# zengyf131/gswt_renderer

Measured on AMD Instinct MI355X. Metric: frames/sec @1920x1080, 32x32 Wang-tile grid, higher is better.
Workload: dtype f32

## Files before the change

### gswt_renderer_amd/csrc/gswt_api.hip

```cpp
#include "../../include/gswt_hip.h"
#include "gswt_device.h"

#include <dlfcn.h>

#include <algorithm>
#include <cstdarg>
#include <cstdio>
#include <cstring>
#include <string>
#include <unordered_map>
#include <utility>
#include <vector>

using namespace gswt;

namespace {

template <typename T>
struct DevBuf {
    T* p = nullptr;
    size_t cap = 0;
    DevBuf() = default;
    DevBuf(DevBuf&& o) noexcept : p(std::exchange(o.p, nullptr)), cap(std::exchange(o.cap, 0)) {}
    DevBuf& operator=(DevBuf&& o) noexcept { std::swap(p, o.p); std::swap(cap, o.cap); return *this; }
    ~DevBuf() { release(); }
    hipError_t ensure(size_t n)
    {
        if (n <= cap) return hipSuccess;
        size_t ncap = n + n / 4 + 1024;
        T* np = nullptr;
        static const bool log_alloc = getenv("GSWT_LOG_ALLOC") != nullptr;
        if (log_alloc) fprintf(stderr, "gswt alloc: %zu -> %zu bytes%s\n", cap * sizeof(T), ncap * sizeof(T), p ? " (grow: frees the old buffer)" : "");
        hipError_t e = hipMalloc(&np, ncap * sizeof(T));
        if (e != hipSuccess) return e;
        if (p) hipFree(p);
        p = np; cap = ncap;
        return hipSuccess;
    }
    hipError_t ensure_roomy(size_t n) { return n <= cap ? hipSuccess : ensure(2 * n); }
    void release() { if (p) hipFree(p); p = nullptr; cap = 0; }
};

using ListRef = gswt::SceneList;

static inline hipError_t null_stream_done() { return hipStreamSynchronize(nullptr); }

template <typename T>
struct HostBuf {
    T* p = nullptr;
    size_t cap = 0;
    HostBuf() = default;
    HostBuf(HostBuf&& o) noexcept : p(std::exchange(o.p, nullptr)), cap(std::exchange(o.cap, 0)) {}
    HostBuf& operator=(HostBuf&& o) noexcept { std::swap(p, o.p); std::swap(cap, o.cap); return *this; }
    ~HostBuf() { release(); }
    hipError_t ensure(size_t n)
    {
        if (n <= cap) return hipSuccess;
        const size_t ncap = n + n / 4 + 64;
        T* np = nullptr;
        hipError_t e = hipHostMalloc(reinterpret_cast<void**>(&np), ncap * sizeof(T), hipHostMallocDefault);
        if (e != hipSuccess) return e;
        if (p) hipHostFree(p);
        p = np; cap = ncap;
        return hipSuccess;
    }
    void release() { if (p) hipHostFree(p); p = nullptr; cap = 0; }
};

}

#ifndef GSWT_FRAME_SLOTS
#define GSWT_FRAME_SLOTS 5
#endif
constexpr int kFrameSlots = GSWT_FRAME_SLOTS;
constexpr const char* kStreamLayout = "c012p34s";

constexpr int kDrawSets = kFrameSlots + 5;
static_assert(kDrawSets <= kMergeSources, "MergeSources holds one pointer pair per draw set");
static_assert(sizeof(gswt_render_config) == 32 && offsetof(gswt_render_config, out_format) == 28, "gswt_render_config layout");
static_assert(GSWT_OUT_RGBA32F == kOutF32 && GSWT_OUT_RGBA8_UNORM == kOutRGBA8 && GSWT_OUT_BGRA8_UNORM == kOutBGRA8, "output formats");
template <typename T>
struct Ref { T* p = nullptr; };

struct DrawSet {
    HostBuf<uint8_t> h_blob;
    DevBuf<uint8_t> d_blob;
    size_t blob_bytes = 0;
    size_t off_draws = 0, off_xcd = 0, off_groups = 0, off_jobs = 0, off_remap = 0, off_segs = 0, off_blocks = 0, off_cblocks = 0, off_n64 = 0;
    template <typename T> T* hp(size_t off) { return reinterpret_cast<T*>(h_blob.p + off); }
    template <typename T> T* dp(size_t off) { return reinterpret_cast<T*>(d_blob.p + off); }
    hipError_t plan(size_t n_draws, size_t n_groups, size_t n_members, size_t total_entries)
    {
        size_t o = 0;
        auto take = [&o](size_t bytes) { const size_t at = o; o = (o + bytes + 255) & ~(size_t)255; return at; };
        const size_t n_blk = total_entries / 1024 + 2 * n_members + 2;
        off_draws = take((n_draws + 1) * sizeof(DrawDev)); off_xcd = take((n_draws + 1) * 4);
        off_groups = take((n_groups + 1) * sizeof(MergeGroup)); off_jobs = take((n_groups + 1) * sizeof(MergeCopy));
        off_remap = take((n_members + 1) * sizeof(uint2)); off_segs = take((2 * n_members + 1) * sizeof(MergeSeg));
        off_blocks = take(n_blk * sizeof(uint2)); off_cblocks = take(n_blk * sizeof(uint2)); off_n64 = take(64);
        blob_bytes = o;
        hipError_t e = o <= h_blob.cap ? hipSuccess : h_blob.ensure(2 * o);
        if (e != hipSuccess) return e;
        e = d_blob.ensure_roomy(o);
        if (e != hipSuccess) return e;
        draws.p = dp<DrawDev>(off_draws); xcd_first.p = dp<uint32_t>(off_xcd);
        return hipSuccess;
    }
    uint64_t per_xcd[8] = {};
    uint64_t longest = 0;
    Ref<DrawDev> draws;
    DevBuf<uint2> chunk_tab;
    DevBuf<uint2> chunk_tab_xcd;
    DevBuf<uint32_t> merged_list, merged_map;
    Ref<uint32_t> xcd_first;
    struct GroupDesc { uint32_t view, base, len, first, n; uint64_t hash; };
    std::vector<GroupDesc> g_desc;
    std::vector<gswt_merge_member> g_members;
    bool g_valid = false;
    uint32_t src_mask = 0;
    hipEvent_t ev_up = nullptr;
    bool ev_up_pending = false;
    bool built = false;
    size_t n_merged = 0;
    uint32_t n_launch = 0;
    uint32_t n_draws = 0, n_chunks = 0;
    uint64_t n_entries = 0;
    void release()
    {
        chunk_tab.release(); chunk_tab_xcd.release(); merged_list.release(); merged_map.release(); h_blob.release(); d_blob.release();
        draws.p = nullptr; xcd_first.p = nullptr;
        if (ev_up) hipEventDestroy(ev_up);
        ev_up = nullptr;
    }
};

struct FrameArgs {
    gswt_camera_uniforms cam;
    gswt_scene_uniforms su;
    gswt_render_config cfg;
    int width = 0, height = 0;
    const float4* d_bg = nullptr;
    const float* d_bgd = nullptr;
    float4* d_out = nullptr;
    float* d_out_depth = nullptr;
};

enum FrameEvent { kEvStart, kEvProjected, kEvEmitted, kEvSorted, kEvRanges, kEvEnd, kEvCompositeBegin, kEvCompositeEnd, kEvDone, kFrameEvents };

struct FrameSlot {
    hipStream_t stream = nullptr;
    hipEvent_t ev[kFrameEvents] = {};
    hipEvent_t ev_in = nullptr;
    hipEvent_t ev_gather = nullptr;
    bool gather_recorded = false;
    unsigned long long seq = 0;
    unsigned long long* hc = nullptr;
    unsigned long long* hc_dev = nullptr;
    bool pending = false;
    bool collected = false;
    int collected_rc = 0;
    gswt_timings collected_timings = {};
    FrameArgs args;
    int set = 0;
    uint32_t cap = 0;
    int n_tiles = 0;
    int timing_level = 0;
    DevBuf<uint2> rects;
    DevBuf<Rec> recs;
    DevBuf<uint4> live_tab;
    DevBuf<uint32_t> live_cnt;
    DevBuf<uint32_t> live_cid;
    DevBuf<uint32_t> cell_culled;
    DevBuf<uint32_t> block_sums, draw_culled, keys_a, keys_b, vals_a, vals_b, ghist;
    DevBuf<uint2> ranges;
    DevBuf<uint32_t> item_base;
    DevBuf<uint4> item_tab;
    DevBuf<uint32_t> aux_a, aux_b;
    bool strict_vs = false;
    uint32_t depth_passes = 0;
    bool depth_local = false;
    bool full_grid = false;
    uint32_t n_launch_eff = 0;
    DevBuf<float4> partials;
    DevBuf<float> partials_z;
    DevBuf<float4> col_f;
    DevBuf<float> depths;
    GraphRec grec;
    hipGraph_t graph = nullptr;
    hipGraphExec_t graph_exec = nullptr;
    hipGraphNode_t graph_nodes[kGraphMaxNodes] = {};
    GraphNodeRec graph_last[kGraphMaxNodes];
    uint32_t graph_n = 0;
    void release_graph()
    {
        if (graph_exec) hipGraphExecDestroy(graph_exec);
        if (graph) hipGraphDestroy(graph);
        graph_exec = nullptr; graph = nullptr; graph_n = 0;
    }
    void release_buffers()
    {
        rects.release(); recs.release(); cell_culled.release(); live_tab.release(); live_cid.release(); live_cnt.release(); block_sums.release(); draw_culled.release(); keys_a.release();
        keys_b.release(); vals_a.release(); vals_b.release(); ghist.release(); ranges.release(); item_base.release();
        aux_a.release(); aux_b.release(); partials.release(); partials_z.release(); item_tab.release(); col_f.release(); depths.release();
    }
};

struct gswt_ctx {
    int device = 0;
    FrameSlot slots[kFrameSlots];
    unsigned long long frame_seq = 0;
    hipStream_t stream = nullptr;
    bool own_stream = true;
    std::string err;
    DevBuf<uint4> tex;
    size_t n_splats = 0;
    float loc_lo[3] = {}, loc_hi[3] = {}, loc_max_trace = 0.0f;
    DevBuf<uint32_t> static_list;
    DevBuf<float> static_boxes;
    std::vector<ListRef> lists;
    size_t static_n = 0, boxes_n = 0;
    int n_lod = 0, n_tile = 0, n_view = 0;
    bool scene_ready = false;
    DevBuf<float> hmap;
    int hm_w = 0, hm_h = 0;
    float hm_min = 0.f, hm_max = 0.f, hm_du = 0.f, hm_dv = 0.f;
    DevBuf<float4> sky_faces;
    int sky_size = 0, sky_equi = 0;
    DevBuf<float4> proxy_tex;
    int proxy_size = 0, proxy_mips = 0, proxy_grid_dim = 2048;
    uint32_t proxy_mip_off[16] = {};
    DrawSet sets[kDrawSets];
    int cur_set = 0;
    int latest_set = 0;
    int pending_set = -1;
    hipStream_t set_stream = nullptr;
    std::vector<hipStream_t> pad_streams;
    int opt_defer_swap = 0;
    int opt_graph = 0;
    int opt_strict_vs = 1;
    int opt_composite = 0;
    int opt_no_chunk_cull = 0;
    unsigned long long stat_graph_launches = 0, stat_graph_rebuilds = 0, stat_graph_node_updates = 0;
    int pending_frames = 0;
    int merge_target = 0;
    DevBuf<int32_t> raw_depth;
    std::vector<uint32_t> raw_off;
    std::vector<uint32_t> raw_cnt, raw_merge_offset;

    int opt_no_merge_reuse = 0;
    unsigned long long stat_groups_built = 0, stat_groups_reused = 0, stat_groups_reused_deep = 0;
    DevBuf<uint32_t> mg_ws;
    bool draws_ready = false;
    uint32_t pair_cap = 0;
    uint32_t depth_passes = 3;
    uint32_t depth_passes_low_run = 0, depth_passes_low_max = 0;
    int opt_depth_sort = 0;
    int opt_item_order = 0;
    uint32_t live_hint = 0;
    uint32_t depth_max_tile_len = 0;
    unsigned long long stat_depth_local = 0, stat_depth_global = 0;
    int last_slot = 0;
    DevBuf<float4> bg_rgba, out_img;
    DevBuf<float> bg_depth, out_depth_img;
    DevBuf<Varyings> dbg;
    int opt_no_prefilter = 0;
    int opt_debug_varyings = 0;
    int opt_timing = 2;
    int opt_segment = 1536;
    int opt_fixed_pair_cap = 0;
    uint32_t last_n_tiles = 0;
    gswt_timings timings = {};
    void* comm = nullptr;
    int comm_rank = 0, comm_world = 0;
    std::vector<gswt_ctx*> group;
    int group_rank = 0;
    DevBuf<float4> gather_buf;
    hipEvent_t ev_push = nullptr;
    hipEvent_t ev_unshard = nullptr;
    bool unshard_pending = false;
};

namespace {

int fail(gswt_ctx* c, int code, const char* fmt, ...)
{
    char buf[512];
    va_list ap;
    va_start(ap, fmt);
    vsnprintf(buf, sizeof(buf), fmt, ap);
    va_end(ap);
    if (c) c->err = buf;
    return code;
}

hipError_t sync_all(gswt_ctx* c)
{
    hipError_t e = hipStreamSynchronize(c->stream);
    if (c->set_stream) { hipError_t e2 = hipStreamSynchronize(c->set_stream); if (e == hipSuccess) e = e2; }
    for (auto& sl : c->slots)
        if (sl.stream) { hipError_t e2 = hipStreamSynchronize(sl.stream); if (e == hipSuccess) e = e2; }
    return e;
}

#define GSWT_CATCH(NAME)                                                                   \
    catch (const std::bad_alloc&) { return GSWT_ERR_CAPACITY; }                             \
    catch (...) { return GSWT_ERR_HIP; }

#define HIP_TRY(c, expr)                                                                              \
    do {                                                                                              \
        hipError_t _e = (expr);                                                                       \
        if (_e != hipSuccess) return fail((c), GSWT_ERR_HIP, "%s: %s", #expr, hipGetErrorString(_e)); \
    } while (0)

void mat4_mul(const float* a, const float* b, float* out)
{
    for (int c = 0; c < 4; c++)
        for (int r = 0; r < 4; r++) {
            float acc = a[r] * b[4 * c];
            for (int k = 1; k < 4; k++) acc = acc + a[4 * k + r] * b[4 * c + k];
            out[4 * c + r] = acc;
        }
}

}

namespace {

struct Id128 { char b[GSWT_COMM_ID_BYTES]; };
struct RcclApi {
    void* lib = nullptr;
    int (*GetUniqueId)(void*) = nullptr;
    int (*CommInitRank)(void**, int,  Id128, int) = nullptr;
    int (*AllGather)(const void*, void*, size_t, int, void*, hipStream_t) = nullptr;
    int (*CommDestroy)(void*) = nullptr;
    const char* (*GetErrorString)(int) = nullptr;
    bool tried = false;
};
RcclApi g_rccl;

const char* rccl_load()
{
    if (g_rccl.lib) return nullptr;
    if (g_rccl.tried) return "librccl.so could not be loaded";
    g_rccl.tried = true;
    const char* names[] = {"librccl.so", "librccl.so.1", "/opt/rocm/lib/librccl.so.1"};
    for (const char* n : names) {
        g_rccl.lib = dlopen(n, RTLD_NOW | RTLD_GLOBAL);
        if (g_rccl.lib) break;
    }
    if (!g_rccl.lib) return "librccl.so could not be loaded";
    g_rccl.GetUniqueId = reinterpret_cast<int (*)(void*)>(dlsym(g_rccl.lib, "ncclGetUniqueId"));
    g_rccl.CommInitRank = reinterpret_cast<int (*)(void**, int, Id128, int)>(dlsym(g_rccl.lib, "ncclCommInitRank"));
    g_rccl.AllGather = reinterpret_cast<int (*)(const void*, void*, size_t, int, void*, hipStream_t)>(dlsym(g_rccl.lib, "ncclAllGather"));
    g_rccl.CommDestroy = reinterpret_cast<int (*)(void*)>(dlsym(g_rccl.lib, "ncclCommDestroy"));
    g_rccl.GetErrorString = reinterpret_cast<const char* (*)(int)>(dlsym(g_rccl.lib, "ncclGetErrorString"));
    if (!g_rccl.GetUniqueId || !g_rccl.CommInitRank || !g_rccl.AllGather || !g_rccl.CommDestroy) {
        dlclose(g_rccl.lib); g_rccl.lib = nullptr;
        return "librccl.so lacks ncclGetUniqueId / ncclCommInitRank / ncclAllGather / ncclCommDestroy";
    }
    return nullptr;
}

constexpr int kNcclFloat = 7;

struct ShardGeom { int world, mode, out_rows, out_w, fmt; size_t px, bytes; };
ShardGeom shard_geom(const FrameSlot& sl)
{
    ShardGeom g;
    const gswt_render_config& cfg = sl.args.cfg;
    g.world = cfg.shard_count <= 1 ? 1 : cfg.shard_count;
    g.mode = cfg.shard_mode;
    const bool cols = g.world > 1 && g.mode == GSWT_SHARD_COLUMNS;
    g.out_rows = g.world > 1 && !cols ? gswt_shard_rows_padded(sl.args.height, g.world) : sl.args.height;
    g.out_w = cols ? gswt_shard_cols_padded(sl.args.width, g.world) : sl.args.width;
    g.px = (size_t)g.out_rows * g.out_w;
    g.fmt = (int)cfg.out_format;
    g.bytes = g.px * out_pixel_bytes(g.fmt);
    return g;
}

}

static int finish_frame(gswt_ctx* c, FrameSlot& sl);

static hipError_t collect_pending(gswt_ctx* c)
{
    for (auto& sl : c->slots)
        if (sl.pending && !sl.collected) {
            sl.collected_rc = finish_frame(c, sl);
            sl.collected_timings = c->timings;
            sl.collected = true;
        }
    return sync_all(c);
}

static void invalidate_merge_sources(gswt_ctx* c)
{
    for (auto& ds : c->sets) { ds.g_valid = false; ds.g_desc.clear(); ds.g_members.clear(); ds.src_mask = 0; }
}

static void collect_set(gswt_ctx* c, int set, bool host_upload)
{
    for (auto& sl : c->slots)
        if (sl.pending && !sl.collected && sl.set == set) {
            sl.collected_rc = finish_frame(c, sl);
            sl.collected_timings = c->timings;
            sl.collected = true;
        }
    if (!host_upload) return;
    for (int k = 0; k < kDrawSets; k++) {
        DrawSet& o = c->sets[k];
        if (k != set && o.ev_up_pending && ((o.src_mask >> set) & 1u)) { (void)hipEventSynchronize(o.ev_up); o.ev_up_pending = false; }
    }
}

namespace gswt {
int ctx_device(const gswt_ctx* c) { return c->device; }
}

extern "C" {

int gswt_create(int device_id, gswt_ctx** out)
try {
    if (!out) return GSWT_ERR_BAD_ARG;
    *out = nullptr;
    int ndev = 0;
    if (hipGetDeviceCount(&ndev) != hipSuccess || ndev <= 0) return GSWT_ERR_HIP;
    if (device_id < 0 || device_id >= ndev) return GSWT_ERR_BAD_ARG;
    if (hipSetDevice(device_id) != hipSuccess) return GSWT_ERR_HIP;
    gswt_ctx* c = new (std::nothrow) gswt_ctx();
    if (!c) return GSWT_ERR_CAPACITY;
    c->device = device_id;
    const char* layout = getenv("GSWT_STREAM_LAYOUT");
    if (!layout || !*layout) layout = kStreamLayout;
    for (const char* q = layout; *q; q++) {
        hipStream_t* dst = nullptr;
        hipStream_t pad = nullptr;
        if (*q == 'c') dst = &c->stream;
        else if (*q == 's') dst = &c->set_stream;
        else if (*q >= '0' && *q < '0' + kFrameSlots) dst = &c->slots[*q - '0'].stream;
        else if (*q == 'p') dst = &pad;
        else continue;
        if (*dst) continue;
        if ((q[1] == '+' || q[1] == '-')) {
            int lo = 0, hi = 0;
            hipDeviceGetStreamPriorityRange(&lo, &hi);
            if (hipStreamCreateWithPriority(dst, hipStreamNonBlocking, q[1] == '+' ? hi : lo) != hipSuccess) { delete c; return GSWT_ERR_HIP; }
        } else
        if (hipStreamCreateWithFlags(dst, hipStreamNonBlocking) != hipSuccess) { delete c; return GSWT_ERR_HIP; }
        if (dst == &pad) c->pad_streams.push_back(pad);
    }
    if (!c->stream && hipStreamCreateWithFlags(&c->stream, hipStreamNonBlocking) != hipSuccess) { delete c; return GSWT_ERR_HIP; }
    if (!c->set_stream && hipStreamCreateWithFlags(&c->set_stream, hipStreamNonBlocking) != hipSuccess) { delete c; return GSWT_ERR_HIP; }
    for (auto& sl : c->slots) {
        if (hipEventCreateWithFlags(&sl.ev_in, hipEventDisableTiming) != hipSuccess) { delete c; return GSWT_ERR_HIP; }
        if (hipEventCreate(&sl.ev_gather) != hipSuccess) { delete c; return GSWT_ERR_HIP; }
        for (auto& e : sl.ev)
            if (hipEventCreate(&e) != hipSuccess) { delete c; return GSWT_ERR_HIP; }
        if (hipHostMalloc(reinterpret_cast<void**>(&sl.hc), 8 * sizeof(unsigned long long), hipHostMallocMapped) != hipSuccess) { delete c; return GSWT_ERR_HIP; }
        memset(sl.hc, 0, 8 * sizeof(unsigned long long));
        if (hipHostGetDevicePointer(reinterpret_cast<void**>(&sl.hc_dev), sl.hc, 0) != hipSuccess) sl.hc_dev = nullptr;
    }
    *out = c;
    return GSWT_OK;
} GSWT_CATCH("gswt_create")

void gswt_destroy(gswt_ctx* c)
{
    if (!c) return;
    hipSetDevice(c->device);
    sync_all(c);
    for (gswt_ctx* m : std::vector<gswt_ctx*>(c->group))
        if (m && m != c) m->group.clear();
    c->group.clear();
    if (c->comm && g_rccl.CommDestroy) g_rccl.CommDestroy(c->comm);
    if (c->ev_push) hipEventDestroy(c->ev_push);
    if (c->ev_unshard) hipEventDestroy(c->ev_unshard);
    c->gather_buf.release();
    c->tex.release(); c->static_list.release(); c->static_boxes.release(); c->hmap.release(); for (auto& ds : c->sets) ds.release();
    c->raw_depth.release(); 
    c->mg_ws.release(); c->sky_faces.release(); c->proxy_tex.release(); c->bg_rgba.release(); c->out_img.release(); c->bg_depth.release(); c->out_depth_img.release(); c->dbg.release();
    for (auto& sl : c->slots) {
        sl.release_graph();
        sl.release_buffers();
        for (auto& e : sl.ev) if (e) hipEventDestroy(e);
        if (sl.ev_in) hipEventDestroy(sl.ev_in);
        if (sl.ev_gather) hipEventDestroy(sl.ev_gather);
        if (sl.hc) hipHostFree(sl.hc);
        if (sl.stream) hipStreamDestroy(sl.stream);
    }
    if (c->own_stream && c->stream) hipStreamDestroy(c->stream);
    if (c->set_stream) hipStreamDestroy(c->set_stream);
    for (hipStream_t ps : c->pad_streams) hipStreamDestroy(ps);
    delete c;
}

const char* gswt_last_error(const gswt_ctx* c) { return c ? c->err.c_str() : "null ctx"; }

int gswt_set_stream(gswt_ctx* c, void* hip_stream)
try {
    if (!c) return GSWT_ERR_BAD_ARG;
    collect_pending(c);
    if (c->own_stream && c->stream) hipStreamDestroy(c->stream);
    if (hip_stream) { c->stream = (hipStream_t)hip_stream; c->own_stream = false; return GSWT_OK; }
    c->stream = nullptr; c->own_stream = true;
    hipSetDevice(c->device);
    HIP_TRY(c, hipStreamCreateWithFlags(&c->stream, hipStreamNonBlocking));
    return GSWT_OK;
} GSWT_CATCH("gswt_set_stream")

int gswt_set_option(gswt_ctx* c, int key, int value)
try {
    if (!c) return GSWT_ERR_BAD_ARG;
    switch (key) {
    case GSWT_OPT_NO_LOD_PREFILTER: c->opt_no_prefilter = value; c->draws_ready = false; return GSWT_OK;
    case GSWT_OPT_DEBUG_VARYINGS: c->opt_debug_varyings = value; return GSWT_OK;
    case GSWT_OPT_DEBUG_FLAGS:
        if (value != 0) return fail(c, GSWT_ERR_BAD_ARG, "GSWT_OPT_DEBUG_FLAGS is reserved: only 0 is accepted");
        return GSWT_OK;
    case GSWT_OPT_TIMING: c->opt_timing = value; return GSWT_OK;
    case GSWT_OPT_NO_MERGE_REUSE: c->opt_no_merge_reuse = value; return GSWT_OK;
    case GSWT_OPT_DEFER_SWAP: c->opt_defer_swap = value; return GSWT_OK;
    case GSWT_OPT_GRAPH: c->opt_graph = value; return GSWT_OK;
    case GSWT_OPT_STRICT_VS: c->opt_strict_vs = value != 0; return GSWT_OK;
    case GSWT_OPT_COMPOSITE:
        if (value < 0 || value > 2) return fail(c, GSWT_ERR_BAD_ARG, "unknown compositor variant %d", value);
        c->opt_composite = value; return GSWT_OK;
    case GSWT_OPT_NO_CHUNK_CULL: c->opt_no_chunk_cull = value != 0; return GSWT_OK;
    case GSWT_OPT_ITEM_ORDER: c->opt_item_order = value != 0; return GSWT_OK;
    case GSWT_OPT_DEPTH_SORT:
        if (value < 0 || value > 2) return fail(c, GSWT_ERR_BAD_ARG, "GSWT_OPT_DEPTH_SORT: 0 (auto), 1 (global passes) or 2 (tile-local)");
        c->opt_depth_sort = value; c->depth_max_tile_len = 0;
        return GSWT_OK;
    case GSWT_OPT_DEPTH_PASSES:
        if (value < 1 || value > 4) return fail(c, GSWT_ERR_BAD_ARG, "depth-sort passes must be 1..4");
        c->depth_passes = (uint32_t)value; c->depth_passes_low_run = 0;
        return GSWT_OK;
    case GSWT_OPT_PAIR_CAP:
        if (value < 0) return fail(c, GSWT_ERR_BAD_ARG, "pair capacity must be >= 0");
        c->opt_fixed_pair_cap = value > 0; if (value > 0) c->pair_cap = (uint32_t)value;
        return GSWT_OK;
    case GSWT_OPT_SEGMENT:
        if (value < 256 || value % 256) return fail(c, GSWT_ERR_BAD_ARG, "segment must be a positive multiple of 256");
        c->opt_segment = value; return GSWT_OK;
    default: return fail(c, GSWT_ERR_BAD_ARG, "unknown option %d", key);
    }
} GSWT_CATCH("gswt_set_option")

int gswt_upload_scene(gswt_ctx* c, const uint32_t* tex_data, size_t n_splats, const gswt_base_list* lists, int n_lod,
                      int n_tile, int n_view)
try {
    if (!c) return GSWT_ERR_BAD_ARG;
    if (!tex_data || n_splats == 0 || !lists || n_lod <= 0 || n_tile <= 0 || n_view <= 0)
        return fail(c, GSWT_ERR_BAD_ARG, "gswt_upload_scene: empty scene");
    if (n_lod > 16) return fail(c, GSWT_ERR_BAD_ARG, "gswt_upload_scene: n_lod %d > 16 (transition_dist_vec holds 16)", n_lod);
    if (n_splats > (size_t)kIdxMask) return fail(c, GSWT_ERR_CAPACITY, "gswt_upload_scene: %zu splats exceed 2^28", n_splats);
    hipSetDevice(c->device);
    HIP_TRY(c, collect_pending(c));
    c->scene_ready = false; c->draws_ready = false;
    invalidate_merge_sources(c);
    HIP_TRY(c, c->tex.ensure(2 * n_splats));
    HIP_TRY(c, hipMemcpy(c->tex.p, tex_data, n_splats * 32, hipMemcpyHostToDevice));
    c->n_splats = n_splats;
    {
        float lo[3] = {3.402823466e+38f, 3.402823466e+38f, 3.402823466e+38f}, hi[3] = {-3.402823466e+38f, -3.402823466e+38f, -3.402823466e+38f};
        float tr_max = 0.0f;
        bool odd = false;
        auto half_val = [](uint32_t h) -> float {
            const uint32_t e = (h >> 10) & 0x1Fu, fr = h & 0x3FFu;
            if (e == 31u) return 0.0f;
            const float m = e == 0u ? (float)fr * 2.98023223876953125e-08f : ldexpf(1.0f + (float)fr / 1024.0f, (int)e - 15);
            return (h & 0x8000u) ? -m : m;
        };
        for (size_t i = 0; i < n_splats; i++) {
            const uint32_t* r = tex_data + 8 * i;
            float p[3];
            memcpy(p, r, 12);
            for (int k = 0; k < 3; k++) {
                if (!(p[k] == p[k]) || p[k] > 3e38f || p[k] < -3e38f) { odd = true; continue; }
                lo[k] = std::min(lo[k], p[k]); hi[k] = std::max(hi[k], p[k]);
            }
            const double xx = half_val(r[4] & 0xFFFFu), xy = half_val(r[4] >> 16), xz = half_val(r[5] & 0xFFFFu);
            const double yy = half_val(r[5] >> 16), yz = half_val(r[6] & 0xFFFFu), zz = half_val(r[6] >> 16);
            const double tr_d = xx + yy + zz;
            const bool psd = xx >= 0.0 && yy >= 0.0 && zz >= 0.0 && xx * yy - xy * xy >= 0.0 && xx * zz - xz * xz >= 0.0 &&
                             yy * zz - yz * yz >= 0.0 && xx * (yy * zz - yz * yz) - xy * (xy * zz - yz * xz) + xz * (xy * yz - yy * xz) >= 0.0;
            const double fro = std::sqrt(xx * xx + yy * yy + zz * zz + 2.0 * (xy * xy + xz * xz + yz * yz));
            const float tr = psd ? (float)tr_d : (float)(0.5 * (tr_d + 1.7320508075688772 * fro) * (1.0 + 1e-6));
            if (tr == tr) tr_max = std::max(tr_max, tr);
        }
        if (odd || lo[0] > hi[0]) { for (int k = 0; k < 3; k++) { lo[k] = -3.402823466e+38f; hi[k] = 3.402823466e+38f; } }
        for (int k = 0; k < 3; k++) { c->loc_lo[k] = lo[k]; c->loc_hi[k] = hi[k]; }
        c->loc_max_trace = tr_max;
    }
    const size_t nl = (size_t)n_lod * n_tile * n_view;
    c->lists.assign(nl, ListRef{});
    std::vector<uint32_t> arena;
    std::vector<float> boxes;
    auto add_boxes = [&](uint32_t base, uint32_t count) -> uint32_t {
        const uint32_t first = (uint32_t)(boxes.size() / 6);
        for (uint32_t k = 0; (size_t)k * kChunk < count; k++) {
            const uint32_t hi_i = count - k * (uint32_t)kChunk, lo_i = hi_i > (uint32_t)kChunk ? hi_i - (uint32_t)kChunk : 0u;
            float lo[3] = {3.402823466e+38f, 3.402823466e+38f, 3.402823466e+38f}, hi[3] = {-3.402823466e+38f, -3.402823466e+38f, -3.402823466e+38f};
            bool odd = false;
            for (uint32_t j = lo_i; j < hi_i; j++) {
                float pq[3];
                memcpy(pq, tex_data + 8 * (size_t)(arena[base + j] & kIdxMask), 12);
                for (int a = 0; a < 3; a++) {
                    if (!(pq[a] == pq[a]) || pq[a] > 3e38f || pq[a] < -3e38f) odd = true;
                    lo[a] = std::min(lo[a], pq[a]); hi[a] = std::max(hi[a], pq[a]);
                }
            }
            for (int a = 0; a < 3; a++) boxes.push_back(odd ? -__builtin_inff() : lo[a]);
            for (int a = 0; a < 3; a++) boxes.push_back(odd ? __builtin_inff() : hi[a]);
        }
        return first;
    };
    size_t total = 0;
    for (size_t i = 0; i < nl; i++) total += lists[i].splat_count;
    arena.reserve(2 * total);
    for (size_t i = 0; i < nl; i++) {
        const gswt_base_list& L = lists[i];
        const uint32_t lod = (uint32_t)(i / ((size_t)n_tile * n_view));
        if (L.splat_count && (!L.gs_index || !L.gs_lod_id)) return fail(c, GSWT_ERR_BAD_ARG, "gswt_upload_scene: list %zu has null arrays", i);
        ListRef ref;
        ref.pair_base = (uint32_t)arena.size();
        ref.pair_count = L.splat_count;
        for (uint32_t j = 0; j < L.splat_count; j++) {
            if (L.gs_index[j] >= n_splats) return fail(c, GSWT_ERR_BAD_ARG, "gswt_upload_scene: list %zu entry %u out of range", i, j);
            if (L.gs_lod_id[j] > 15u) return fail(c, GSWT_ERR_BAD_ARG, "gswt_upload_scene: list %zu lod id out of range", i);
            arena.push_back(L.gs_index[j] | (L.gs_lod_id[j] << kLodShift));
        }
        ref.self_base = (uint32_t)arena.size();
        for (uint32_t j = 0; j < L.splat_count; j++)
            if (L.gs_lod_id[j] == lod) arena.push_back(L.gs_index[j] | (lod << kLodShift));
        ref.self_count = (uint32_t)arena.size() - ref.self_base;
        ref.pair_box = add_boxes(ref.pair_base, ref.pair_count);
        ref.self_box = add_boxes(ref.self_base, ref.self_count);
        c->lists[i] = ref;
    }
    if (arena.size() >= 0xFFFFFFFFull) return fail(c, GSWT_ERR_CAPACITY, "gswt_upload_scene: static lists exceed 2^32 entries");
    HIP_TRY(c, c->static_list.ensure(arena.size() + 1));
    HIP_TRY(c, hipMemcpy(c->static_list.p, arena.data(), arena.size() * 4, hipMemcpyHostToDevice));
    HIP_TRY(c, c->static_boxes.ensure(boxes.size() + 6));
    if (!boxes.empty()) HIP_TRY(c, hipMemcpy(c->static_boxes.p, boxes.data(), boxes.size() * 4, hipMemcpyHostToDevice));
    HIP_TRY(c, null_stream_done());
    c->static_n = arena.size(); c->boxes_n = boxes.size() / 6;
    c->n_lod = n_lod; c->n_tile = n_tile; c->n_view = n_view;
    c->scene_ready = true;
    return GSWT_OK;
} GSWT_CATCH("gswt_upload_scene")

int gswt_upload_scene_rows(gswt_ctx* c, const uint8_t* const* rows32, const uint32_t* counts, int n_lod, int n_tile, const float* presort_vp,
                           int n_view)
try {
    if (!c) return GSWT_ERR_BAD_ARG;
    if (!rows32 || !counts || !presort_vp || n_lod <= 0 || n_tile <= 0 || n_view <= 0)
        return fail(c, GSWT_ERR_BAD_ARG, "gswt_upload_scene_rows: empty scene");
    if (n_lod > 16) return fail(c, GSWT_ERR_BAD_ARG, "gswt_upload_scene_rows: n_lod %d > 16 (transition_dist_vec holds 16)", n_lod);
    if (n_view > kSceneMaxViews) return fail(c, GSWT_ERR_BAD_ARG, "gswt_upload_scene_rows: n_view %d > %d", n_view, kSceneMaxViews);
    const size_t n_lt = (size_t)n_lod * n_tile, nv = (size_t)n_view;
    if (n_lt > 65536) return fail(c, GSWT_ERR_CAPACITY, "gswt_upload_scene_rows: %zu lists per view exceed the 16 list bits of the sort key", n_lt);
    std::vector<uint32_t> moff(n_lt);
    size_t n_splats = 0;
    for (size_t i = 0; i < n_lt; i++) {
        if (counts[i] == 0) return fail(c, GSWT_ERR_BAD_ARG, "gswt_upload_scene_rows: tile scene %zu is empty", i);
        if (!rows32[i]) return fail(c, GSWT_ERR_BAD_ARG, "gswt_upload_scene_rows: tile scene %zu has null rows", i);
        moff[i] = (uint32_t)std::min(n_splats, (size_t)kIdxMask);
        n_splats += counts[i];
        if (n_splats > (size_t)kIdxMask) return fail(c, GSWT_ERR_CAPACITY, "gswt_upload_scene_rows: more than 2^28 splats");
    }
    auto cnt = [&](size_t l, size_t t) -> uint32_t { return counts[l * n_tile + t]; };
    auto list_len = [&](size_t l, size_t t) -> uint32_t { return cnt(l, t) + (l + 1 < (size_t)n_lod ? cnt(l + 1, t) : 0u); };
    const size_t nl = n_lt * nv;
    std::vector<ListRef> lists(nl);
    size_t arena_n = 0, boxes_n = 0;
    for (size_t l = 0; l < (size_t)n_lod; l++)
        for (size_t t = 0; t < (size_t)n_tile; t++)
            for (size_t v = 0; v < nv; v++) {
                ListRef& r = lists[(l * n_tile + t) * nv + v];
                r.pair_base = (uint32_t)arena_n; r.pair_count = list_len(l, t);
                r.self_base = (uint32_t)(arena_n + r.pair_count); r.self_count = cnt(l, t);
                arena_n += (size_t)r.pair_count + r.self_count;
                r.pair_box = (uint32_t)boxes_n; boxes_n += (r.pair_count + kChunk - 1) / kChunk;
                r.self_box = (uint32_t)boxes_n; boxes_n += (r.self_count + kChunk - 1) / kChunk;
                if (arena_n >= 0xFFFFFFFFull) return fail(c, GSWT_ERR_CAPACITY, "gswt_upload_scene_rows: static lists exceed 2^32 entries");
            }
    if (nv * n_splats >= 0xFFFFFFFFull) return fail(c, GSWT_ERR_CAPACITY, "gswt_upload_scene_rows: raw depth arena exceeds 2^32");
    size_t n_total = 0;
    for (size_t l = 0; l < (size_t)n_lod; l++) for (size_t t = 0; t < (size_t)n_tile; t++) n_total += list_len(l, t);
    std::vector<MergeSeg> segs;
    std::vector<MergeGroup> groups;
    std::vector<uint2> blocks;
    std::vector<size_t> seg_first(nv + 1), blk_first(nv + 1);
    for (size_t v = 0; v < nv; v++) {
        seg_first[v] = segs.size(); blk_first[v] = blocks.size();
        uint32_t build = 0;
        for (size_t l = 0; l < (size_t)n_lod; l++)
            for (size_t t = 0; t < (size_t)n_tile; t++) {
                const uint32_t g = (uint32_t)(l * n_tile + t);
                MergeGroup G;
                G.base = build; G.len = list_len(l, t); G.mn = 2147483647; G.mx = -2147483647 - 1;
                G.out_base = lists[(size_t)g * nv + v].pair_base; G._pad[0] = G._pad[1] = G._pad[2] = 0;
                groups.push_back(G);
                for (size_t q = l; q < (size_t)n_lod && q <= l + 1; q++) {
                    const size_t lt = q * n_tile + t;
                    MergeSeg sg;
                    sg.group = g; sg.src = (uint32_t)(nv * moff[lt] + v * counts[lt]); sg.len = counts[lt]; sg.start = build;
                    sg.gs_offset = moff[lt]; sg.map_index = 0; sg.lod = (uint32_t)q; sg._pad = 0;
                    for (uint32_t off = 0; off < sg.len; off += 1024u) blocks.push_back(make_uint2((uint32_t)(segs.size() - seg_first[v]), off));
                    segs.push_back(sg);
                    build += sg.len;
                }
            }
    }
    seg_first[nv] = segs.size(); blk_first[nv] = blocks.size();
    SceneViews vps;
    memset(&vps, 0, sizeof(vps));
    vps.n_view = (uint32_t)nv;
    memcpy(vps.vp, presort_vp, nv * 16 * sizeof(float));
    int gbits = 1;
    while ((1u << gbits) < n_lt) gbits++;

    hipSetDevice(c->device);
    HIP_TRY(c, collect_pending(c));
    c->scene_ready = false; c->draws_ready = false;
    invalidate_merge_sources(c);
    c->raw_cnt.clear(); c->raw_merge_offset.clear(); c->raw_off.clear();
    hipStream_t s = c->stream;
    const size_t radix_words = radix_ws_words((uint32_t)n_total, 16 + gbits);
    DevBuf<uint4> rows_d;
    DevBuf<uint32_t> tabs, sortbuf;
    DevBuf<int32_t> bounds_d;
    HIP_TRY(c, rows_d.ensure(2 * n_splats));
    const size_t seg_words = segs.size() * sizeof(MergeSeg) / 4, grp_words = groups.size() * sizeof(MergeGroup) / 4;
    const size_t blk_words = 2 * blocks.size(), list_words = nl * sizeof(ListRef) / 4;
    HIP_TRY(c, tabs.ensure(2 * n_lt + seg_words + grp_words + blk_words + list_words));
    HIP_TRY(c, sortbuf.ensure(4 * n_total + 16 + radix_words + 16));
    HIP_TRY(c, bounds_d.ensure(8));
    HIP_TRY(c, c->tex.ensure(2 * n_splats));
    HIP_TRY(c, c->raw_depth.ensure(nv * n_splats + 1));
    HIP_TRY(c, c->static_list.ensure(arena_n + 1));
    HIP_TRY(c, c->static_boxes.ensure(6 * boxes_n + 6));
    uint32_t* const d_moff = tabs.p;
    uint32_t* const d_cnt = d_moff + n_lt;
    MergeSeg* const d_segs = reinterpret_cast<MergeSeg*>(d_cnt + n_lt);
    MergeGroup* const d_groups = reinterpret_cast<MergeGroup*>(tabs.p + 2 * n_lt + seg_words);
    uint2* const d_blocks = reinterpret_cast<uint2*>(tabs.p + 2 * n_lt + seg_words + grp_words);
    ListRef* const d_lists = reinterpret_cast<ListRef*>(tabs.p + 2 * n_lt + seg_words + grp_words + blk_words);
    for (size_t i = 0; i < n_lt; i++)
        HIP_TRY(c, hipMemcpyAsync(rows_d.p + 2 * (size_t)moff[i], rows32[i], (size_t)counts[i] * 32, hipMemcpyHostToDevice, s));
    HIP_TRY(c, hipMemcpyAsync(d_moff, moff.data(), n_lt * 4, hipMemcpyHostToDevice, s));
    HIP_TRY(c, hipMemcpyAsync(d_cnt, counts, n_lt * 4, hipMemcpyHostToDevice, s));
    HIP_TRY(c, hipMemcpyAsync(d_segs, segs.data(), seg_words * 4, hipMemcpyHostToDevice, s));
    HIP_TRY(c, hipMemcpyAsync(d_groups, groups.data(), grp_words * 4, hipMemcpyHostToDevice, s));
    HIP_TRY(c, hipMemcpyAsync(d_blocks, blocks.data(), blk_words * 4, hipMemcpyHostToDevice, s));
    HIP_TRY(c, hipMemcpyAsync(d_lists, lists.data(), list_words * 4, hipMemcpyHostToDevice, s));
    const int32_t bounds_init[8] = {2147483647, 2147483647, 2147483647, -2147483647 - 1, -2147483647 - 1, -2147483647 - 1, 0, 0};
    HIP_TRY(c, hipMemcpyAsync(bounds_d.p, bounds_init, sizeof(bounds_init), hipMemcpyHostToDevice, s));
    launch_scene_tex(s, rows_d.p, (uint32_t)n_splats, c->tex.p, bounds_d.p);
    launch_scene_raw(s, rows_d.p, (uint32_t)n_splats, d_moff, d_cnt, (uint32_t)n_lt, vps, c->raw_depth.p);
    uint32_t* const ka = sortbuf.p;
    uint32_t* const va = ka + n_total;
    uint32_t* const kb = va + n_total;
    uint32_t* const vb = kb + n_total;
    uint32_t* const hdr = vb + n_total;
    uint32_t* const ws = hdr + 16;
    const unsigned long long n64[4] = {(unsigned long long)n_total, 0ull, 0ull, 0ull};
    HIP_TRY(c, hipMemcpyAsync(hdr, n64, sizeof(n64), hipMemcpyHostToDevice, s));
    for (size_t v = 0; v < nv; v++) {
        HIP_TRY(c, hipMemsetAsync(ws, 0, radix_words * 4, s));
        const int where = launch_scene_sort(s, d_segs + seg_first[v], d_blocks + blk_first[v], (uint32_t)(blk_first[v + 1] - blk_first[v]),
                                            d_groups + v * n_lt, c->raw_depth.p, (uint32_t)n_total, reinterpret_cast<const unsigned long long*>(hdr),
                                            ka, va, kb, vb, ws, gbits);
        launch_scene_scatter(s, d_segs + seg_first[v], (uint32_t)(seg_first[v + 1] - seg_first[v]), d_groups + v * n_lt, where ? kb : ka,
                             where ? vb : va, (uint32_t)n_total, c->static_list.p, (uint32_t)arena_n);
    }
    launch_scene_self(s, d_lists, (uint32_t)nl, (uint32_t)((size_t)n_tile * nv), c->static_list.p);
    launch_scene_boxes(s, d_lists, (uint32_t)nl, (uint32_t)boxes_n, c->static_list.p, c->tex.p, (uint32_t)n_splats, c->static_boxes.p);
    HIP_TRY(c, hipGetLastError());
    int32_t bounds[8];
    HIP_TRY(c, hipMemcpyAsync(bounds, bounds_d.p, sizeof(bounds), hipMemcpyDeviceToHost, s));
    HIP_TRY(c, hipStreamSynchronize(s));
    {
        auto ord2f = [](int32_t i) { const int32_t b = i >= 0 ? i : i ^ 0x7FFFFFFF; float f; memcpy(&f, &b, 4); return f; };
        float lo[3], hi[3];
        for (int k = 0; k < 3; k++) { lo[k] = ord2f(bounds[k]); hi[k] = ord2f(bounds[3 + k]); }
        if (bounds[6] || lo[0] > hi[0]) { for (int k = 0; k < 3; k++) { lo[k] = -3.402823466e+38f; hi[k] = 3.402823466e+38f; } }
        for (int k = 0; k < 3; k++) { c->loc_lo[k] = lo[k]; c->loc_hi[k] = hi[k]; }
        memcpy(&c->loc_max_trace, &bounds[7], 4);
    }
    c->n_splats = n_splats;
    c->lists = std::move(lists);
    c->static_n = arena_n; c->boxes_n = boxes_n;
    c->raw_cnt.assign(counts, counts + n_lt);
    c->raw_merge_offset = moff;
    c->raw_off.assign(n_lt * nv, 0);
    for (size_t i = 0; i < n_lt; i++) for (size_t v = 0; v < nv; v++) c->raw_off[i * nv + v] = (uint32_t)(nv * moff[i] + v * counts[i]);
    c->n_lod = n_lod; c->n_tile = n_tile; c->n_view = n_view;
    c->scene_ready = true;
    return GSWT_OK;
} GSWT_CATCH("gswt_upload_scene_rows")

int gswt_debug_read_scene(gswt_ctx* c, int what, void* out, size_t cap_bytes, size_t* n_bytes)
try {
    if (!c || !n_bytes) return GSWT_ERR_BAD_ARG;
    if (!c->scene_ready) return fail(c, GSWT_ERR_STATE, "gswt_debug_read_scene before a scene upload");
    const void* dev = nullptr;
    const void* hostp = nullptr;
    size_t bytes = 0;
    std::vector<uint32_t> tmp;
    switch (what) {
    case GSWT_SCENE_TEX: dev = c->tex.p; bytes = c->n_splats * 32; break;
    case GSWT_SCENE_RAW_DEPTH: {
        size_t total = 0;
        for (uint32_t k : c->raw_cnt) total += (size_t)k * c->n_view;
        dev = c->raw_depth.p; bytes = total * 4; break;
    }
    case GSWT_SCENE_RAW_TABLES:
        tmp = c->raw_off;
        tmp.insert(tmp.end(), c->raw_cnt.begin(), c->raw_cnt.end());
        tmp.insert(tmp.end(), c->raw_merge_offset.begin(), c->raw_merge_offset.end());
        hostp = tmp.data(); bytes = tmp.size() * 4; break;
    case GSWT_SCENE_STATIC_LIST: dev = c->static_list.p; bytes = c->static_n * 4; break;
    case GSWT_SCENE_STATIC_BOXES: dev = c->static_boxes.p; bytes = c->boxes_n * 24; break;
    case GSWT_SCENE_LISTS: hostp = c->lists.data(); bytes = c->lists.size() * sizeof(ListRef); break;
    case GSWT_SCENE_BOUNDS: {
        tmp.resize(7);
        memcpy(tmp.data(), c->loc_lo, 12); memcpy(tmp.data() + 3, c->loc_hi, 12); memcpy(tmp.data() + 6, &c->loc_max_trace, 4);
        hostp = tmp.data(); bytes = 28; break;
    }
    default: return fail(c, GSWT_ERR_BAD_ARG, "gswt_debug_read_scene: unknown item %d", what);
    }
    *n_bytes = bytes;
    if (!out) return GSWT_OK;
    if (cap_bytes < bytes) return fail(c, GSWT_ERR_CAPACITY, "gswt_debug_read_scene: buffer holds %zu bytes, need %zu", cap_bytes, bytes);
    if (hostp) { memcpy(out, hostp, bytes); return GSWT_OK; }
    hipSetDevice(c->device);
    HIP_TRY(c, sync_all(c));
    if (bytes) HIP_TRY(c, hipMemcpy(out, dev, bytes, hipMemcpyDeviceToHost));
    return GSWT_OK;
} GSWT_CATCH("gswt_debug_read_scene")

int gswt_configure(gswt_ctx* c, const float* height_map, int hm_w, int hm_h)
try {
    if (!c) return GSWT_ERR_BAD_ARG;
    hipSetDevice(c->device);
    HIP_TRY(c, collect_pending(c));
    if (!height_map || hm_w <= 0 || hm_h <= 0) { c->hm_w = c->hm_h = 0; return GSWT_OK; }
    HIP_TRY(c, c->hmap.ensure((size_t)hm_w * hm_h + 2));
    HIP_TRY(c, hipMemcpy(c->hmap.p, height_map, (size_t)hm_w * hm_h * 4, hipMemcpyHostToDevice));
    HIP_TRY(c, hipMemset(c->hmap.p + (size_t)hm_w * hm_h, 0, 8));
    {
        float mn = height_map[0], mx = height_map[0], du = 0.f, dv = 0.f;
        bool finite = true;
        for (int y = 0; y < hm_h; y++)
            for (int x = 0; x < hm_w; x++) {
                const float h = height_map[(size_t)y * hm_w + x];
                const float hr = height_map[(size_t)y * hm_w + (x + 1 == hm_w ? 0 : x + 1)], hd = height_map[(size_t)(y + 1 == hm_h ? 0 : y + 1) * hm_w + x];
                if (!(h == h) || h > 3e38f || h < -3e38f) finite = false;
                mn = std::min(mn, h); mx = std::max(mx, h);
                du = std::max(du, std::fabs(hr - h)); dv = std::max(dv, std::fabs(hd - h));
            }
        c->hm_min = mn; c->hm_max = mx; c->hm_du = du * (float)hm_w; c->hm_dv = dv * (float)hm_h;
        if (!finite) { c->hm_min = -3e38f; c->hm_max = 3e38f; c->hm_du = c->hm_dv = 3e38f; }
    }
    HIP_TRY(c, null_stream_done());
    c->hm_w = hm_w; c->hm_h = hm_h;
    return GSWT_OK;
} GSWT_CATCH("gswt_configure")

static void activate_pending(gswt_ctx* c, bool force)
{
    if (c->pending_set < 0) return;
    DrawSet& P = c->sets[c->pending_set];
    bool now = force;
    if (!now && c->opt_defer_swap >= 2) now = c->pending_frames-- <= 0;
    else if (!now) now = !P.ev_up || hipEventQuery(P.ev_up) == hipSuccess;
    if (now) { c->cur_set = c->pending_set; c->pending_set = -1; }
}
static int next_target(gswt_ctx* c)
{
    activate_pending(c, true);
    return c->draws_ready ? (c->latest_set + 1) % kDrawSets : c->cur_set;
}
static void publish_set(gswt_ctx* c, int target)
{
    const bool first = !c->draws_ready || target == c->cur_set;
    c->latest_set = target;
    if (c->opt_defer_swap && !first) { c->pending_set = target; c->pending_frames = c->opt_defer_swap - 1; }
    else { c->cur_set = target; c->pending_set = -1; }
}

static int set_draws_impl(gswt_ctx* c, const gswt_draw* draws, int n_draws, const uint32_t* merged_gs_index,
                          const uint32_t* merged_map_id, const uint32_t* merged_lod_id, size_t n_merged, bool device_merge)
{
    if (!c) return GSWT_ERR_BAD_ARG;
    if (!c->scene_ready) return fail(c, GSWT_ERR_STATE, "gswt_set_draws before gswt_upload_scene");
    if (n_draws < 0 || (n_draws > 0 && !draws)) return fail(c, GSWT_ERR_BAD_ARG, "gswt_set_draws: bad draw list");
    if (!device_merge && n_merged && (!merged_gs_index || !merged_map_id)) return fail(c, GSWT_ERR_BAD_ARG, "gswt_set_draws: merged arrays missing");
    if (n_merged >= 0xFFFFFFFFull) return fail(c, GSWT_ERR_CAPACITY, "gswt_set_draws: merged lists exceed 2^32 entries");
    hipSetDevice(c->device);
    const int target = device_merge ? c->merge_target : next_target(c);
    collect_set(c, target, !device_merge);
    DrawSet& D = c->sets[target];
    if (D.ev_up_pending) { HIP_TRY(c, hipEventSynchronize(D.ev_up)); D.ev_up_pending = false; }
    if (!D.ev_up) HIP_TRY(c, hipEventCreateWithFlags(&D.ev_up, hipEventDisableTiming));
    if (!device_merge) HIP_TRY(c, D.plan((size_t)n_draws, 0, 0, 0));
    DrawDev* const dd = D.hp<DrawDev>(D.off_draws);
    uint32_t* const h_xcd_first = D.hp<uint32_t>(D.off_xcd);
    uint64_t entries = 0;
    for (int i = 0; i < n_draws; i++) {
        const gswt_draw& g = draws[i];
        DrawDev& d = dd[i];
        memset(&d, 0, sizeof(d));
        d.single_draw = g.tile.single_draw;
        d.valid_lod_id = g.tile.valid_lod_id;
        d.changing = g.tile.changing;
        d.changing_to_lower = g.tile.changing_to_lower;
        d.tile_lod = g.tile.tile_id[0];
        d.tile_idx = g.tile.tile_id[1]; d.tile_view = g.tile.tile_id[2];
        d.single_lod_id = g.tile.single_lod_id;
        d.map_coord[0] = g.tile.map_coord[0]; d.map_coord[1] = g.tile.map_coord[1];
        d.off[0] = g.tile.offset[0]; d.off[1] = g.tile.offset[1]; d.off[2] = g.tile.offset[2];
        d.cull_enable = g.cull_enable;
        d.lod = g.lod;
        memcpy(d.corners, g.corners, sizeof(d.corners));
        if (g.merged) {
            if ((size_t)g.merged_offset + g.merged_count > n_merged)
                return fail(c, GSWT_ERR_BAD_ARG, "gswt_set_draws: draw %d merged range out of bounds", i);
            if (g.merged_has_lod && !merged_lod_id && !device_merge)
                return fail(c, GSWT_ERR_BAD_ARG, "gswt_set_draws: draw %d needs merged_lod_id", i);
            if (g.tile.single_draw != 1u) return fail(c, GSWT_ERR_BAD_ARG, "gswt_set_draws: merged draw %d without single_draw", i);
            d.merged = 1; d.list_base = g.merged_offset; d.count = g.merged_count; d.box_base = 0xFFFFFFFFu;
        } else {
            if (g.tile.single_draw == 1u) return fail(c, GSWT_ERR_BAD_ARG, "gswt_set_draws: single_draw on static draw %d", i);
            if ((int)g.base_lod >= c->n_lod || (int)g.base_tile >= c->n_tile || (int)g.base_view >= c->n_view)
                return fail(c, GSWT_ERR_BAD_ARG, "gswt_set_draws: draw %d base list (%u,%u,%u) out of range", i, g.base_lod,
                            g.base_tile, g.base_view);
            const ListRef& L = c->lists[((size_t)g.base_lod * c->n_tile + g.base_tile) * c->n_view + g.base_view];
            const bool prefilter = !c->opt_no_prefilter && g.tile.valid_lod_id >= 0 && (uint32_t)g.tile.valid_lod_id == g.base_lod;
            d.merged = 0;
            d.list_base = prefilter ? L.self_base : L.pair_base;
            d.count = prefilter ? L.self_count : L.pair_count;
            d.box_base = prefilter ? L.self_box : L.pair_box;
        }
        d.entry_base = (uint32_t)entries;
        entries += d.count;
    }
    if (entries >= 0xFFFFFF00ull) return fail(c, GSWT_ERR_CAPACITY, "gswt_set_draws: %llu list entries exceed 2^32", (unsigned long long)entries);
    uint64_t slot = 0, per_xcd[8] = {};
    for (int i = n_draws - 1; i >= 0; i--) {
        DrawDev& d = dd[i];
        d.slot_base = (uint32_t)slot;
        const uint32_t nch = (d.count + kChunk - 1) / kChunk;
        int x = 0;
        for (int q = 1; q < 8; q++) if (per_xcd[q] < per_xcd[x]) x = q;
        d.xcd = (uint32_t)x;
        h_xcd_first[i] = (uint32_t)per_xcd[x];
        per_xcd[x] += nch;
        slot += (uint64_t)nch * kChunk;
    }
    if (slot >= 0xFFFFFFFFull) return fail(c, GSWT_ERR_CAPACITY, "gswt_set_draws: slot space exceeds 2^32");
    const size_t n_chunks = (size_t)(slot / kChunk);
    size_t longest = 0;
    for (int x = 0; x < 8; x++) longest = std::max<size_t>(longest, (size_t)per_xcd[x]);
    if (longest * 8 >= 0xFFFFFFFFull) return fail(c, GSWT_ERR_CAPACITY, "gswt_set_draws: chunk table too large");
    HIP_TRY(c, D.chunk_tab.ensure_roomy(n_chunks + 1));
    HIP_TRY(c, D.chunk_tab_xcd.ensure_roomy(longest * 8 + 1));
    D.n_launch = (uint32_t)(longest * 8);
    for (int x = 0; x < 8; x++) D.per_xcd[x] = per_xcd[x];
    D.longest = longest;
    if (!device_merge) {
        hipStream_t s = c->set_stream;
        HIP_TRY(c, hipMemcpyAsync(D.d_blob.p, D.h_blob.p, D.blob_bytes, hipMemcpyHostToDevice, s));
        launch_chunk_tabs(s, D.draws.p, D.xcd_first.p, (uint32_t)n_draws, D.chunk_tab.p, D.chunk_tab_xcd.p, D.per_xcd, D.longest);
        HIP_TRY(c, hipGetLastError());
        HIP_TRY(c, hipEventRecord(D.ev_up, s));
        D.ev_up_pending = true; D.built = false;
    }
    HIP_TRY(c, D.merged_list.ensure_roomy(n_merged + 1));
    HIP_TRY(c, D.merged_map.ensure_roomy(n_merged + 1));
    D.n_merged = n_merged;
    if (n_merged && !device_merge) {
        std::vector<uint32_t> packed(n_merged);
        for (size_t k = 0; k < n_merged; k++) {
            if (merged_gs_index[k] >= c->n_splats) return fail(c, GSWT_ERR_BAD_ARG, "gswt_set_draws: merged gs_index[%zu] out of range", k);
            packed[k] = merged_gs_index[k];
        }
        for (int i = 0; i < n_draws; i++) {
            const gswt_draw& g = draws[i];
            if (g.merged && g.merged_has_lod)
                for (uint32_t k = 0; k < g.merged_count; k++) {
                    uint32_t l = merged_lod_id[g.merged_offset + k];
                    if (l > 15u) return fail(c, GSWT_ERR_BAD_ARG, "gswt_set_draws: merged lod id out of range");
                    packed[g.merged_offset + k] |= l << kLodShift;
                }
        }
        HIP_TRY(c, hipMemcpy(D.merged_list.p, packed.data(), n_merged * 4, hipMemcpyHostToDevice));
        HIP_TRY(c, hipMemcpy(D.merged_map.p, merged_map_id, n_merged * 4, hipMemcpyHostToDevice));
        HIP_TRY(c, null_stream_done());
    }
    D.n_draws = (uint32_t)n_draws;
    D.n_chunks = (uint32_t)n_chunks;
    D.g_valid = false;
    D.src_mask = 0;
    D.n_entries = entries;
    for (int k = 0; k < kDrawSets; k++) {
        DrawSet& o = c->sets[k];
        if (&o == &D) continue;
        const bool empty = !o.d_blob.p && !o.chunk_tab.p && !o.merged_list.p;
        bool used = k == c->cur_set || k == c->pending_set || k == c->latest_set || o.ev_up_pending;
        for (const FrameSlot& fs : c->slots) used = used || (fs.pending && fs.set == k);
        if (used && !empty) continue;
        if (o.g_valid) continue;
        if (o.h_blob.cap >= D.h_blob.cap && o.d_blob.cap >= D.d_blob.cap && o.chunk_tab.cap >= D.chunk_tab.cap &&
            o.chunk_tab_xcd.cap >= D.chunk_tab_xcd.cap && o.merged_list.cap >= D.merged_list.cap && o.merged_map.cap >= D.merged_map.cap) continue;
        HIP_TRY(c, o.h_blob.ensure(D.h_blob.cap)); HIP_TRY(c, o.d_blob.ensure(D.d_blob.cap));
        HIP_TRY(c, o.chunk_tab.ensure(D.chunk_tab.cap)); HIP_TRY(c, o.chunk_tab_xcd.ensure(D.chunk_tab_xcd.cap));
        {
            const uint32_t* const l0 = o.merged_list.p; const uint32_t* const m0 = o.merged_map.p;
            HIP_TRY(c, o.merged_list.ensure(D.merged_list.cap)); HIP_TRY(c, o.merged_map.ensure(D.merged_map.cap));
            if (o.merged_list.p != l0 || o.merged_map.p != m0) o.g_valid = false;
        }
    }
    if (!device_merge) { publish_set(c, target); c->draws_ready = true; }
    return GSWT_OK;
}

int gswt_set_draws(gswt_ctx* c, const gswt_draw* draws, int n_draws, const uint32_t* merged_gs_index,
                   const uint32_t* merged_map_id, const uint32_t* merged_lod_id, size_t n_merged)
try {
    return set_draws_impl(c, draws, n_draws, merged_gs_index, merged_map_id, merged_lod_id, n_merged, false);
} GSWT_CATCH("gswt_set_draws")

int gswt_upload_raw_depth(gswt_ctx* c, const int32_t* const* raw_depth, const uint32_t* counts, const uint32_t* merge_offset)
try {
    if (!c || !raw_depth || !counts || !merge_offset) return GSWT_ERR_BAD_ARG;
    if (!c->scene_ready) return fail(c, GSWT_ERR_STATE, "gswt_upload_raw_depth before gswt_upload_scene");
    hipSetDevice(c->device);
    HIP_TRY(c, sync_all(c));
    invalidate_merge_sources(c);
    const size_t nlt = (size_t)c->n_lod * c->n_tile, nv = (size_t)c->n_view;
    c->raw_cnt.assign(counts, counts + nlt);
    c->raw_merge_offset.assign(merge_offset, merge_offset + nlt);
    c->raw_off.assign(nlt * nv, 0);
    size_t total = 0;
    for (size_t i = 0; i < nlt; i++) for (size_t v = 0; v < nv; v++) { c->raw_off[i * nv + v] = (uint32_t)total; total += counts[i]; }
    if (total >= 0xFFFFFFFFull) return fail(c, GSWT_ERR_CAPACITY, "gswt_upload_raw_depth: raw depth arena exceeds 2^32");
    std::vector<int32_t> arena(total);
    for (size_t i = 0; i < nlt; i++)
        for (size_t v = 0; v < nv; v++) {
            if (counts[i] && !raw_depth[i * nv + v]) return fail(c, GSWT_ERR_BAD_ARG, "gswt_upload_raw_depth: null array");
            if (counts[i]) memcpy(arena.data() + c->raw_off[i * nv + v], raw_depth[i * nv + v], (size_t)counts[i] * 4);
        }
    HIP_TRY(c, c->raw_depth.ensure(total + 1));
    if (total) HIP_TRY(c, hipMemcpy(c->raw_depth.p, arena.data(), total * 4, hipMemcpyHostToDevice));
    HIP_TRY(c, null_stream_done());
    return GSWT_OK;
} GSWT_CATCH("gswt_upload_raw_depth")

int gswt_set_draws_merge_groups(gswt_ctx* c, const gswt_draw* draws, int n_draws, const gswt_merge_group* groups, int n_groups,
                                const gswt_merge_member* members, int n_members)
try {
    if (!c) return GSWT_ERR_BAD_ARG;
    if (n_groups < 0 || n_members < 0 || (n_groups && (!groups || !members))) return fail(c, GSWT_ERR_BAD_ARG, "gswt_set_draws_merge_groups: bad groups");
    if (n_groups && c->raw_cnt.empty()) return fail(c, GSWT_ERR_STATE, "gswt_set_draws_merge_groups before gswt_upload_raw_depth");
    if (n_groups > 32768) return fail(c, GSWT_ERR_CAPACITY, "gswt_set_draws_merge_groups: more than 32768 merged groups");
    hipSetDevice(c->device);
    const int target = next_target(c);
    c->merge_target = target;
    collect_set(c, target, false);
    DrawSet& D = c->sets[target];
    std::vector<int> sources;
    if (c->draws_ready && !c->opt_no_merge_reuse)
        for (int j = 0; j < kDrawSets - 1; j++) {
            const int k = ((c->latest_set - j) % kDrawSets + kDrawSets) % kDrawSets;
            if (k != target && c->sets[k].g_valid && c->sets[k].merged_list.p) sources.push_back(k);
        }
    if (D.ev_up_pending) { HIP_TRY(c, hipEventSynchronize(D.ev_up)); D.ev_up_pending = false; }
    {
        size_t total_upper = 0;
        for (int q = 0; q < n_members; q++) {
            const gswt_merge_member& M = members[q];
            if ((int)M.lod < c->n_lod && (int)M.tile < c->n_tile) total_upper += c->raw_cnt[(size_t)M.lod * c->n_tile + M.tile];
            if (M.other_lod >= 0 && M.other_lod < c->n_lod && (int)M.tile < c->n_tile) total_upper += c->raw_cnt[(size_t)M.other_lod * c->n_tile + M.tile];
        }
        HIP_TRY(c, D.plan((size_t)std::max(n_draws, 0), (size_t)n_groups, (size_t)n_members, total_upper));
    }
    MergeSeg* const segs = D.hp<MergeSeg>(D.off_segs);
    MergeGroup* const grp = D.hp<MergeGroup>(D.off_groups);
    MergeCopy* const jobs = D.hp<MergeCopy>(D.off_jobs);
    uint2* const h_remap = D.hp<uint2>(D.off_remap);
    std::unordered_multimap<uint64_t, std::pair<int, uint32_t>> prev_by_hash;
    for (int k : sources) for (uint32_t q = 0; q < c->sets[k].g_desc.size(); q++) prev_by_hash.emplace(c->sets[k].g_desc[q].hash, std::make_pair(k, q));
    std::vector<DrawSet::GroupDesc> desc((size_t)n_groups);
    size_t n_segs = 0, n_build = 0, n_jobs = 0, n_remap = 0;
    uint64_t total = 0, build_total = 0;
    const size_t nv = (size_t)c->n_view;
    for (int g = 0; g < n_groups; g++) {
        const gswt_merge_group& G = groups[g];
        if ((uint64_t)G.first_member + G.n_members > (uint64_t)n_members || (int)G.view_id >= c->n_view)
            return fail(c, GSWT_ERR_BAD_ARG, "gswt_set_draws_merge_groups: group %d out of range", g);
        uint64_t h = 1469598103934665603ull ^ G.view_id, len = 0;
        for (uint32_t m = 0; m < G.n_members; m++) {
            const gswt_merge_member& M = members[G.first_member + m];
            const int lods[2] = {(int)M.lod, M.other_lod};
            for (int k = 0; k < 2; k++) {
                if (lods[k] < 0) continue;
                if (lods[k] >= c->n_lod || (int)M.tile >= c->n_tile) return fail(c, GSWT_ERR_BAD_ARG, "gswt_set_draws_merge_groups: member tid out of range");
                len += c->raw_cnt[(size_t)lods[k] * c->n_tile + M.tile];
            }
            h = (h ^ (((uint64_t)M.lod << 40) | ((uint64_t)M.tile << 8) | (uint64_t)(uint8_t)(M.other_lod + 1))) * 1099511628211ull;
        }
        DrawSet::GroupDesc& d = desc[g];
        d.view = G.view_id; d.base = (uint32_t)total; d.len = (uint32_t)len; d.first = G.first_member; d.n = G.n_members; d.hash = h;
        int match = -1, match_set = -1, match_rank = 1 << 30;
        if (!sources.empty() && len) {
            auto range = prev_by_hash.equal_range(h);
            for (auto it = range.first; it != range.second; ++it) {
                const DrawSet& ps = c->sets[it->second.first];
                const DrawSet::GroupDesc& p = ps.g_desc[it->second.second];
                if (p.view != G.view_id || p.n != G.n_members || p.len != (uint32_t)len || G.n_members > 256u) continue;
                bool same = true;
                for (uint32_t m = 0; m < G.n_members && same; m++) {
                    const gswt_merge_member& a = members[G.first_member + m];
                    const gswt_merge_member& b = ps.g_members[p.first + m];
                    same = a.lod == b.lod && a.tile == b.tile && a.other_lod == b.other_lod;
                }
                if (!same) continue;
                int rank = 0;
                while (rank < (int)sources.size() && sources[rank] != it->second.first) rank++;
                if (rank < match_rank) { match_rank = rank; match = (int)it->second.second; match_set = it->second.first; }
            }
        }
        if (match >= 0) {
            const DrawSet& ps = c->sets[match_set];
            const DrawSet::GroupDesc& p = ps.g_desc[match];
            MergeCopy jb;
            jb.src = p.base; jb.dst = (uint32_t)total; jb.len = (uint32_t)len; jb.first_pair = (uint32_t)n_remap; jb.n_pairs = 0; jb.src_set = (uint32_t)match_set; jb._pad[0] = jb._pad[1] = 0;
            bool moved = false;
            for (uint32_t m = 0; m < G.n_members; m++) moved = moved || members[G.first_member + m].map_index != ps.g_members[p.first + m].map_index;
            if (moved) {
                for (uint32_t m = 0; m < G.n_members; m++)
                    h_remap[n_remap++] = make_uint2(ps.g_members[p.first + m].map_index, members[G.first_member + m].map_index);
                jb.n_pairs = G.n_members;
            }
            jobs[n_jobs++] = jb;
            if (match_rank > 0) c->stat_groups_reused_deep++;
        } else if (len) {
            MergeGroup& B = grp[n_build];
            B.base = (uint32_t)build_total; B.len = (uint32_t)len; B.mn = 2147483647; B.mx = -2147483647 - 1; B.out_base = (uint32_t)total; B._pad[0] = B._pad[1] = B._pad[2] = 0;
            for (uint32_t m = 0; m < G.n_members; m++) {
                const gswt_merge_member& M = members[G.first_member + m];
                const int lods[2] = {(int)M.lod, M.other_lod};
                for (int k = 0; k < 2; k++) {
                    if (lods[k] < 0) continue;
                    const size_t lt = (size_t)lods[k] * c->n_tile + M.tile;
                    MergeSeg sg;
                    sg.group = (uint32_t)n_build; sg.src = c->raw_off[lt * nv + G.view_id]; sg.len = c->raw_cnt[lt]; sg.start = (uint32_t)build_total;
                    sg.gs_offset = c->raw_merge_offset[lt]; sg.map_index = M.map_index; sg.lod = (uint32_t)lods[k]; sg._pad = 0;
                    if (sg.len) segs[n_segs++] = sg;
                    build_total += sg.len;
                }
            }
            n_build++;
        }
        total += len;
    }
    if (total >= 0xFFFFFFFFull) return fail(c, GSWT_ERR_CAPACITY, "gswt_set_draws_merge_groups: merged lists exceed 2^32 entries");
    for (int i = 0; i < n_draws; i++)
        if (draws[i].merged) {
            const uint32_t g = draws[i].merged_group;
            if ((int)g >= n_groups || draws[i].merged_offset != desc[g].base || draws[i].merged_count != desc[g].len)
                return fail(c, GSWT_ERR_BAD_ARG, "gswt_set_draws_merge_groups: draw %d does not match group %u (offset %u/%u count %u/%u)", i, g,
                            draws[i].merged_offset, (int)g < n_groups ? desc[g].base : 0u, draws[i].merged_count, (int)g < n_groups ? desc[g].len : 0u);
        }
    int rc = set_draws_impl(c, draws, n_draws, nullptr, nullptr, nullptr, (size_t)total, true);
    if (rc != GSWT_OK) return rc;
    MergeSources msrc;
    for (int k = 0; k < kMergeSources; k++) { msrc.list[k] = nullptr; msrc.map[k] = nullptr; }
    D.src_mask = 0;
    for (int k : sources) {
        if (!c->sets[k].g_valid) return fail(c, GSWT_ERR_STATE, "gswt_set_draws_merge_groups: a source set lost its lists");
        msrc.list[k] = c->sets[k].merged_list.p; msrc.map[k] = c->sets[k].merged_map.p;
    }
    for (size_t q = 0; q < n_jobs; q++) D.src_mask |= 1u << jobs[q].src_set;
    D.g_desc.swap(desc);
    D.g_members.assign(members, members + n_members);
    D.g_valid = false;
    c->stat_groups_built += n_build; c->stat_groups_reused += n_jobs;
    hipStream_t s = c->set_stream;
    uint2* const h_cblocks = D.hp<uint2>(D.off_cblocks);
    uint2* const h_blocks = D.hp<uint2>(D.off_blocks);
    size_t n_cb = 0, n_blocks = 0;
    for (size_t q = 0; q < n_jobs; q++)
        for (uint32_t off = 0; off < jobs[q].len; off += 1024u) h_cblocks[n_cb++] = make_uint2((uint32_t)q, off);
    for (size_t q = 0; q < n_segs; q++)
        for (uint32_t off = 0; off < segs[q].len; off += 1024u) h_blocks[n_blocks++] = make_uint2((uint32_t)q, off);
    const uint32_t n_total = (uint32_t)build_total;
    memset(D.hp<uint8_t>(D.off_n64), 0, 64);
    *D.hp<unsigned long long>(D.off_n64) = n_total;
    HIP_TRY(c, hipMemcpyAsync(D.d_blob.p, D.h_blob.p, D.blob_bytes, hipMemcpyHostToDevice, s));
    launch_chunk_tabs(s, D.draws.p, D.xcd_first.p, D.n_draws, D.chunk_tab.p, D.chunk_tab_xcd.p, D.per_xcd, D.longest);
    if (n_jobs)
        launch_merge_copy(s, D.dp<MergeCopy>(D.off_jobs), D.dp<uint2>(D.off_cblocks), (uint32_t)n_cb, D.dp<uint2>(D.off_remap), msrc,
                          D.merged_list.p, D.merged_map.p);
    if (n_build) {
        int gbits = 1;
        while ((1u << gbits) < n_build) gbits++;
        const size_t radix_words = radix_ws_words(n_total, 16 + gbits);
        HIP_TRY(c, c->mg_ws.ensure_roomy(4 * (size_t)n_total + radix_words + 16));
        uint32_t* w = c->mg_ws.p;
        uint32_t* radix = w + 4 * (size_t)n_total;
        HIP_TRY(c, hipMemsetAsync(radix, 0, (radix_words + 16) * 4, s));
        launch_merge_build(s, D.dp<MergeSeg>(D.off_segs), (uint32_t)n_segs, D.dp<uint2>(D.off_blocks), (uint32_t)n_blocks, D.dp<MergeGroup>(D.off_groups),
                           (uint32_t)n_build, c->raw_depth.p, n_total, D.dp<unsigned long long>(D.off_n64), w, w + n_total, w + 2 * (size_t)n_total,
                           w + 3 * (size_t)n_total, radix, gbits, D.merged_list.p, D.merged_map.p);
    }
    HIP_TRY(c, hipGetLastError());
    HIP_TRY(c, hipEventRecord(D.ev_up, s));
    D.ev_up_pending = true; D.built = false;
    D.g_valid = true;
    publish_set(c, target);
    c->draws_ready = true;
    return GSWT_OK;
} GSWT_CATCH("gswt_set_draws_merge_groups")

int gswt_debug_read_merged(gswt_ctx* c, uint32_t* packed_list, uint32_t* map_id, size_t capacity, size_t* n)
try {
    if (!c || !n) return GSWT_ERR_BAD_ARG;
    const DrawSet& D = c->sets[c->cur_set];
    *n = D.n_merged;
    if (!packed_list || !map_id) return GSWT_OK;
    if (capacity < D.n_merged) return fail(c, GSWT_ERR_CAPACITY, "buffer holds %zu entries, need %zu", capacity, D.n_merged);
    hipSetDevice(c->device);
    HIP_TRY(c, sync_all(c));
    if (D.n_merged) {
        HIP_TRY(c, hipMemcpy(packed_list, D.merged_list.p, D.n_merged * 4, hipMemcpyDeviceToHost));
        HIP_TRY(c, hipMemcpy(map_id, D.merged_map.p, D.n_merged * 4, hipMemcpyDeviceToHost));
    }
    return GSWT_OK;
} GSWT_CATCH("gswt_debug_read_merged")

int gswt_shard_rows_padded(int height, int shard_count)
try {
    int tiles_y = (height + kTile - 1) / kTile;
    int sc = shard_count <= 1 ? 1 : shard_count;
    return ((tiles_y + sc - 1) / sc) * kTile;
} GSWT_CATCH("gswt_shard_rows_padded")

int gswt_shard_cols_padded(int width, int shard_count)
try {
    int tiles_x = (width + kTile - 1) / kTile;
    int sc = shard_count <= 1 ? 1 : shard_count;
    return ((tiles_x + sc - 1) / sc) * kTile;
} GSWT_CATCH("gswt_shard_cols_padded")

int gswt_shard_rows(int height, int shard_index, int shard_count)
try {
    int sc = shard_count <= 1 ? 1 : shard_count;
    if (shard_index < 0 || shard_index >= sc) return 0;
    int rows = 0;
    for (int y = 0; y < height; y++) if (((y / kTile) % sc) == shard_index) rows++;
    return rows;
} GSWT_CATCH("gswt_shard_rows")

static int validate_frame(gswt_ctx* c, const gswt_camera_uniforms* cam, const gswt_scene_uniforms* su, const gswt_render_config* cfg,
                          int width, int height, const void* out_rgba)
{
    if (!cam || !su || !cfg || !out_rgba) return fail(c, GSWT_ERR_BAD_ARG, "gswt_render: null argument");
    if (!c->draws_ready) return fail(c, GSWT_ERR_STATE, "gswt_render before gswt_set_draws");
    if (width <= 0 || height <= 0 || width > 65535 * kTile || height > 65535 * kTile)
        return fail(c, GSWT_ERR_BAD_ARG, "gswt_render: bad target size %dx%d", width, height);
    if ((float)width != cam->viewport[0] || (float)height != cam->viewport[1])
        return fail(c, GSWT_ERR_BAD_ARG, "gswt_render: camera viewport (%g,%g) != target %dx%d", cam->viewport[0], cam->viewport[1], width, height);
    if (su->surface_type == 1u && (c->hm_w == 0 || c->hm_h == 0))
        return fail(c, GSWT_ERR_STATE, "gswt_render: surface_type HeightMap without gswt_configure height map");
    if (su->surface_type > 2u) return fail(c, GSWT_ERR_BAD_ARG, "gswt_render: unknown surface_type %u", su->surface_type);
    if (su->surface_type == 2u && (su->map_half_wh[0] == 0u || su->map_half_wh[1] == 0u))
        return fail(c, GSWT_ERR_BAD_ARG, "gswt_render: Sphere surface needs a non-empty map");
    if (su->draw_mode > 4u) return fail(c, GSWT_ERR_BAD_ARG, "gswt_render: unknown draw_mode %u", su->draw_mode);
    if (cfg->order_mode != GSWT_ORDER_REFERENCE && cfg->order_mode != GSWT_ORDER_DEPTH)
        return fail(c, GSWT_ERR_BAD_ARG, "gswt_render: unknown order mode %d", cfg->order_mode);
    const int sc = cfg->shard_count <= 1 ? 1 : cfg->shard_count;
    if (sc > 1 && (cfg->shard_index < 0 || cfg->shard_index >= sc)) return fail(c, GSWT_ERR_BAD_ARG, "gswt_render: bad shard index");
    if (cfg->shard_mode != GSWT_SHARD_ROWS && cfg->shard_mode != GSWT_SHARD_COLUMNS) return fail(c, GSWT_ERR_BAD_ARG, "gswt_render: unknown shard mode %d", cfg->shard_mode);
    if (cfg->out_format != GSWT_OUT_RGBA32F && cfg->out_format != GSWT_OUT_RGBA8_UNORM && cfg->out_format != GSWT_OUT_BGRA8_UNORM)
        return fail(c, GSWT_ERR_BAD_ARG, "gswt_render: unknown out_format %u", cfg->out_format);
    return GSWT_OK;
}

static int replay_graph(gswt_ctx* c, FrameSlot& sl)
{
    GraphRec& R = sl.grec;
    if (R.overflow || R.n == 0) return fail(c, GSWT_ERR_STATE, "gswt_render: frame graph record overflow");
    bool rebuild = !sl.graph_exec || sl.graph_n != R.n;
    for (uint32_t i = 0; !rebuild && i < R.n; i++) rebuild = sl.graph_last[i].fn != R.nodes[i].fn;
    void* ptrs[40];
    auto fill = [&](GraphNodeRec& nd, hipKernelNodeParams& kp) {
        memset(&kp, 0, sizeof(kp));
        for (uint32_t a = 0; a < nd.n_args; a++) ptrs[a] = nd.args + nd.offs[a];
        kp.func = const_cast<void*>(nd.fn);
        kp.gridDim = nd.grid; kp.blockDim = nd.block; kp.sharedMemBytes = 0;
        kp.kernelParams = ptrs; kp.extra = nullptr;
    };
    if (rebuild) {
        sl.release_graph();
        HIP_TRY(c, hipGraphCreate(&sl.graph, 0));
        for (uint32_t i = 0; i < R.n; i++) {
            hipKernelNodeParams kp;
            fill(R.nodes[i], kp);
            HIP_TRY(c, hipGraphAddKernelNode(&sl.graph_nodes[i], sl.graph, i ? &sl.graph_nodes[i - 1] : nullptr, i ? 1 : 0, &kp));
            sl.graph_last[i] = R.nodes[i];
        }
        HIP_TRY(c, hipGraphInstantiate(&sl.graph_exec, sl.graph, nullptr, nullptr, 0));
        sl.graph_n = R.n;
        c->stat_graph_rebuilds++;
    } else {
        for (uint32_t i = 0; i < R.n; i++) {
            if (sl.graph_last[i].same(R.nodes[i])) continue;
            hipKernelNodeParams kp;
            fill(R.nodes[i], kp);
            HIP_TRY(c, hipGraphExecKernelNodeSetParams(sl.graph_exec, sl.graph_nodes[i], &kp));
            sl.graph_last[i] = R.nodes[i];
            c->stat_graph_node_updates++;
        }
    }
    HIP_TRY(c, hipGraphLaunch(sl.graph_exec, sl.stream));
    c->stat_graph_launches++;
    return GSWT_OK;
}

static Frame make_frame(const gswt_ctx& c, const FrameArgs& a)
{
    const gswt_camera_uniforms* cam = &a.cam;
    const gswt_scene_uniforms* su = &a.su;
    const gswt_render_config* cfg = &a.cfg;
    const int width = a.width, height = a.height;
    const int sc = cfg->shard_count <= 1 ? 1 : cfg->shard_count;
    Frame f;
    memset(&f, 0, sizeof(f));
    memcpy(f.V, cam->view, 64);
    for (int cc = 0; cc < 4; cc++) {
        const float* P = cam->projection;
        f.GP[4 * cc + 0] = P[4 * cc + 0];
        f.GP[4 * cc + 1] = P[4 * cc + 1];
        f.GP[4 * cc + 2] = 0.5f * P[4 * cc + 2] + 0.5f * P[4 * cc + 3];
        f.GP[4 * cc + 3] = P[4 * cc + 3];
    }
    mat4_mul(cam->projection, cam->view, f.VP);
    f.focal[0] = cam->focal[0]; f.focal[1] = cam->focal[1];
    f.htan[0] = cam->htan_fov[0]; f.htan[1] = cam->htan_fov[1];
    f.cam_pos[0] = cam->cam_pos[0]; f.cam_pos[1] = cam->cam_pos[1]; f.cam_pos[2] = cam->cam_pos[2];
    f.W = (float)width; f.H = (float)height;
    f.splat_scale = su->splat_scale; f.tile_width = su->tile_width; f.clip_height = su->clip_height;
    f.point_cloud_radius = su->point_cloud_radius; f.transition_width_ratio = su->transition_width_ratio;
    f.sphere_radius = su->sphere_radius;
    f.use_clip = su->use_clip; f.surface_type = su->surface_type; f.num_lod = su->num_lod; f.draw_mode = su->draw_mode;
    f.map_half_wh[0] = su->map_half_wh[0]; f.map_half_wh[1] = su->map_half_wh[1];
    f.center_coord[0] = su->center_coord[0]; f.center_coord[1] = su->center_coord[1];
    memcpy(f.transition_dist, su->transition_dist_vec, 64);
    for (int k = 0; k < 3; k++) { f.height_map_scale[k] = su->height_map_scale[k]; f.scene_scale[k] = su->scene_scale[k]; }
    f.culling_dist = cfg->culling_dist; f.lod_enable_mask = cfg->lod_enable_mask; f.t_eps = cfg->transmittance_eps;
    f.has_depth = a.d_bgd ? 1 : 0;
    f.width = width; f.height = height;
    const int tiles_x_full = (width + kTile - 1) / kTile;
    const bool cols = sc > 1 && cfg->shard_mode == GSWT_SHARD_COLUMNS;
    f.tiles_x = tiles_x_full; f.tiles_y = (height + kTile - 1) / kTile;
    f.col0 = 0; f.col1 = tiles_x_full; f.out_w = width; f.out_x0 = 0; f.band_cull = 0;
    f.shard_index = sc > 1 && !cols ? cfg->shard_index : 0; f.shard_count = cols ? 1 : sc;
// ... 919 lines not shown
```

### gswt_renderer_amd/csrc/gswt_device.h

```cpp
#pragma once
#include <hip/hip_runtime.h>
#include <hip/hip_ext.h>
#include <hip/hip_fp16.h>
#include <stdint.h>
#include <string.h>
#include <type_traits>

namespace gswt {

constexpr int kTile = 16;
constexpr int kChunk = 256;
constexpr uint32_t kLodShift = 28;
constexpr uint32_t kIdxMask = (1u << kLodShift) - 1u;
constexpr int kOutF32 = 0, kOutRGBA8 = 1, kOutBGRA8 = 2;
inline size_t out_pixel_bytes(int out_format) { return out_format == kOutF32 ? 16u : 4u; }

struct DrawDev {
    uint32_t single_draw;
    int32_t valid_lod_id;
    uint32_t changing;
    int32_t changing_to_lower;
    uint32_t tile_lod;
    float off[3];
    uint32_t list_base;
    uint32_t count;
    uint32_t merged;
    uint32_t slot_base;
    uint32_t cull_enable;
    uint32_t lod;
    float corners[12];
    uint32_t entry_base;
    int32_t single_lod_id;
    uint32_t tile_idx;
    uint32_t tile_view;
    uint32_t map_coord[2];
    uint32_t box_base;
    uint32_t xcd;
};

struct Frame {
    float V[16];
    float GP[16];
    float VP[16];
    float focal[2];
    float htan[2];
    float cam_pos[3];
    float W, H;
    float splat_scale, tile_width, clip_height, point_cloud_radius, transition_width_ratio, sphere_radius;
    uint32_t use_clip, surface_type, num_lod, draw_mode;
    uint32_t map_half_wh[2];
    int32_t center_coord[2];
    float transition_dist[16];
    float height_map_scale[3];
    float scene_scale[3];
    float culling_dist;
    uint32_t lod_enable_mask;
    float t_eps;
    int32_t has_depth;
    int32_t width, height, tiles_x, tiles_y;
    int32_t shard_index, shard_count;
    int32_t col0, col1;
    int32_t out_w, out_x0;
    int32_t band_cull;
    float loc_lo[3], loc_hi[3];
    float loc_max_trace;
    float surf_zlo, surf_zhi;
    float surf_f2;
    int32_t hm_w, hm_h;
    uint32_t tiles_x_magic;
    uint32_t map_wh_y, map_wh_y_magic;
};

struct __attribute__((aligned(32))) Rec {
    float iux, iuy, ivx, ivy;
    float ndcx, ndcy, alpha, rgba8;
};

struct MergeSeg {
    uint32_t group, src, len, start, gs_offset, map_index, lod, _pad;
};
struct MergeGroup {
    uint32_t base, len;
    int32_t mn, mx;
    uint32_t out_base;
    uint32_t _pad[3];
};
struct MergeCopy {
    uint32_t src, dst, len;
    uint32_t first_pair, n_pairs;
    uint32_t src_set;
    uint32_t _pad[2];
};
struct SceneList { uint32_t pair_base, pair_count, self_base, self_count, pair_box, self_box; };
constexpr int kSceneMaxViews = 16;
struct SceneViews {
    uint32_t n_view;
    float vp[kSceneMaxViews][16];
};
constexpr int kMergeSources = 12;
struct MergeSources {
    const uint32_t* list[kMergeSources];
    const uint32_t* map[kMergeSources];
};

struct Varyings {
    int32_t visible;
    float ndc[2];
    float depth;
    float major[2];
    float minor[2];
    float rgba[4];
};

struct SkyArgs {
    float V[16];
    float p00, p11;
    int width, height, face_size, equirectangular;
};

struct SkyBakeArgs {
    float basis[6][9];
    int face_size, equi_w, equi_h;
};

struct ProxyMipArgs {
    int src_w, src_h, n;
    int u16;
    int pitch;
    int copy;
    int stride_v, stride_h;
    int splits, chunk;
    float maxv;
};
ProxyMipArgs plan_proxy_mip(int src_w, int src_h, int n, int u16, int pitch);
inline size_t proxy_mip_tmp_texels(const ProxyMipArgs& a) { return a.copy ? 0 : (size_t)a.n * a.src_w; }
inline size_t proxy_mip_part_texels(const ProxyMipArgs& a) { return a.copy || a.splits == 1 ? 0 : (size_t)a.splits * a.n * a.src_w; }
inline size_t proxy_mip_weights(const ProxyMipArgs& a, int axis) { return a.copy ? 0 : (size_t)a.n * (axis == 0 ? a.stride_v : a.stride_h); }

struct ProxyArgs {
    float height_offset, tile_width, width_scale, clip_height, brightness;
    uint32_t surface_type, use_clip, black_background;
    float V[16], GP[16];
    float p00, p11;
    float cam[3];
    uint32_t map_half_wh[2];
    float height_map_scale[3];
    int nx, ny;
    float cs, gx0, gy0;
    int hm_w, hm_h, tex_size, n_mips;
    uint32_t mip_off[16];
    int width, height;
};

struct GraphNodeRec {
    const void* fn = nullptr;
    dim3 grid, block;
    uint32_t n_args = 0, n_bytes = 0;
    uint16_t offs[40];
    alignas(16) unsigned char args[1280];
    template <typename T>
    void push(const T& v)
    {
        static_assert(alignof(T) <= 16, "kernel argument alignment");
        n_bytes = (n_bytes + (uint32_t)alignof(T) - 1u) & ~((uint32_t)alignof(T) - 1u);
        if (n_args >= 40u || n_bytes + sizeof(T) > sizeof(args)) { fn = nullptr; return; }
        memcpy(args + n_bytes, &v, sizeof(T));
        offs[n_args++] = (uint16_t)n_bytes;
        n_bytes += (uint32_t)sizeof(T);
    }
    bool same(const GraphNodeRec& o) const
    {
        return fn == o.fn && grid.x == o.grid.x && grid.y == o.grid.y && grid.z == o.grid.z && block.x == o.block.x && n_args == o.n_args &&
               n_bytes == o.n_bytes && memcmp(args, o.args, n_bytes) == 0;
    }
};
constexpr uint32_t kSuperStride = 16;
constexpr uint32_t kGraphMaxNodes = 32;
struct GraphRec {
    GraphNodeRec nodes[kGraphMaxNodes];
    uint32_t n = 0;
    bool overflow = false;
};
GraphRec*& graph_recorder();

template <typename... KA, typename... A>
inline void graph_record(GraphRec* rec, void (*k)(KA...), dim3 g, dim3 b, A&&... a)
{
    static_assert(sizeof...(KA) == sizeof...(A), "kernel argument count");
    if (rec->n >= kGraphMaxNodes) { rec->overflow = true; return; }
    GraphNodeRec& nd = rec->nodes[rec->n++];
    nd.fn = reinterpret_cast<const void*>(k);
    nd.grid = g; nd.block = b; nd.n_args = 0; nd.n_bytes = 0;
    memset(nd.args, 0, sizeof(nd.args));
    (nd.push(static_cast<typename std::decay<KA>::type>(a)), ...);
    if (!nd.fn) rec->overflow = true;
}
#define GSWT_LAUNCH(K, G, B, S, ...)                                                                     \
    do {                                                                                                 \
        if (GraphRec* rec_ = graph_recorder()) graph_record(rec_, K, G, B, __VA_ARGS__);                 \
        else hipLaunchKernelGGL(K, G, B, 0, S, __VA_ARGS__);                                             \
    } while (0)

bool kernel_events_enabled();
#define GSWT_LAUNCH_TIMED(K, G, B, S, E0, E1, ...)                                                       \
    do {                                                                                                 \
        if ((E0) && (E1) && !graph_recorder() && kernel_events_enabled())                                \
            hipExtLaunchKernelGGL(K, G, B, 0, S, E0, E1, 0, __VA_ARGS__);                                \
        else {                                                                                           \
            if (E0) hipEventRecord(E0, S);                                                               \
            GSWT_LAUNCH(K, G, B, S, __VA_ARGS__);                                                        \
            if (E1) hipEventRecord(E1, S);                                                               \
        }                                                                                                \
    } while (0)

struct FrameBufs {
    const DrawDev* draws;
    const uint2 *chunk_tab, *chunk_tab_xcd;
    const uint32_t *static_list, *merged_list, *merged_map;
    const uint4* tex;
    const float *hmap, *boxes;
    const float4* bg_rgba; const float* bg_depth; float4* out;
    float* out_depth;
    unsigned long long* host_counters;
    uint32_t n_chunks, n_cells, n_tiles, pair_cap, seg;
    uint2* rects; Rec* recs; float4* col_f; Varyings* dbg;
    float* depths;
    uint32_t *draw_culled, *cell_culled, *live_cnt, *live_cid, *block_sums; uint4* live_tab;
    unsigned long long* counters;
    uint32_t *krange, *super_sums, *radix_pair, *radix_depth;
    uint32_t *keys_a, *keys_b, *vals_a, *vals_b, *aux_a, *aux_b;
    uint2* ranges; uint32_t* long_tiles;
    uint32_t* item_base; uint4* item_tab; float4* partials;
    float* partials_z;
    uint32_t n_zero_head, n_zero_ranges, n_zero_depth;
};

void launch_chunk_tabs(hipStream_t s, const DrawDev* draws, const uint32_t* xcd_first, uint32_t n_draws, uint2* chunk_tab, uint2* chunk_tab_xcd,
                       const uint64_t per_xcd[8], uint64_t longest);
void launch_merge_build(hipStream_t s, const MergeSeg* segs, uint32_t n_segs, const uint2* blocks, uint32_t n_blocks, MergeGroup* groups, uint32_t n_groups,
                        const int32_t* raw, uint32_t n_total, const unsigned long long* n_total_dev, uint32_t* ka, uint32_t* va,
                        uint32_t* kb, uint32_t* vb, uint32_t* radix_ws, int group_bits, uint32_t* merged_list, uint32_t* merged_map);
int launch_scene_sort(hipStream_t s, const MergeSeg* segs, const uint2* blocks, uint32_t n_blocks, MergeGroup* groups, const int32_t* raw,
                      uint32_t n_total, const unsigned long long* n_total_dev, uint32_t* ka, uint32_t* va, uint32_t* kb, uint32_t* vb,
                      uint32_t* radix_ws, int group_bits);
void launch_scene_tex(hipStream_t s, const uint4* rows, uint32_t n, uint4* tex, int32_t* bounds);
void launch_scene_raw(hipStream_t s, const uint4* rows, uint32_t n, const uint32_t* moff, const uint32_t* cnt, uint32_t n_lt, const SceneViews& vps,
                      int32_t* raw);
void launch_scene_scatter(hipStream_t s, const MergeSeg* segs, uint32_t n_segs, const MergeGroup* groups, const uint32_t* sorted_keys,
                          const uint32_t* sorted_vals, uint32_t n_total, uint32_t* arena, uint32_t arena_n);
void launch_scene_self(hipStream_t s, const SceneList* lists, uint32_t n_lists, uint32_t lists_per_lod, uint32_t* arena);
void launch_scene_boxes(hipStream_t s, const SceneList* lists, uint32_t n_lists, uint32_t n_boxes, const uint32_t* arena, const uint4* tex,
                        uint32_t n_splats, float* boxes);
void launch_merge_copy(hipStream_t s, const MergeCopy* jobs, const uint2* blocks, uint32_t n_blocks, const uint2* remap, const MergeSources& src,
                       uint32_t* new_list, uint32_t* new_map);

void launch_cull(hipStream_t s, const Frame& f, const FrameBufs& b, bool chunk_cull);
void launch_project(hipStream_t s, const Frame& f, const FrameBufs& b, uint32_t n_launch, bool debug, bool strict);
void launch_emit(hipStream_t s, const Frame& f, const FrameBufs& b, uint32_t* keys, uint32_t* dkeys, uint32_t* krange, uint32_t n_launch);
void launch_composite(hipStream_t s, const Frame& f, const FrameBufs& b, const uint32_t* vals, int out_rows, int variant, const uint32_t* krange,
                      uint32_t depth_passes, bool report_max, bool heavy_first, hipEvent_t ev_begin, hipEvent_t ev_end, int out_format);
void launch_totals(hipStream_t s, uint32_t* super_sums, uint32_t n_super, unsigned long long* counters, uint32_t pair_cap);

size_t radix_ws_words(uint32_t n_cap, int key_bits);
size_t radix_ws_zero_words(uint32_t n_cap, int key_bits);
int launch_sort(hipStream_t s, uint32_t* keys_a, uint32_t* vals_a, uint32_t* keys_b, uint32_t* vals_b, uint32_t n_cap,
                const unsigned long long* n_ptr, int key_bits, uint32_t* ws, uint2* ranges = nullptr, const uint32_t* krange = nullptr,
                uint32_t* aux_a = nullptr, uint32_t* aux_b = nullptr);

void launch_tile_depth_sort(hipStream_t s, const uint2* ranges, uint32_t* vals, uint32_t* dkeys, uint32_t* vals_scratch, uint32_t* dkeys_scratch, int n_tiles,
                            uint32_t* long_list, unsigned long long* counters);
inline size_t tile_depth_list_words(size_t n_tiles) { return n_tiles + 1; }
uint32_t tile_depth_sort_cap();

void launch_unshard(hipStream_t s, const void* gathered, void* out, int width, int height, int shard_count, int rows_padded, int band_px,
                    int out_format);
void launch_skybox(hipStream_t s, const float* view16, float p00, float p11, int width, int height, int face_size, int equirect,
                   const float4* faces, float4* out);
void launch_skybox_bake(hipStream_t s, const SkyBakeArgs& a, const float4* equi, float4* faces);
void launch_proxy(hipStream_t s, const ProxyArgs& a, const float* hm, const float4* tex, float4* rgba, float* depth);
void launch_proxy_mip(hipStream_t s, const ProxyMipArgs& a, const uint8_t* src, int2* ranges, float* wv, float* wh, float4* tmp,
                      float4* part, float4* dst);
void launch_fill_f32(hipStream_t s, float* p, size_t n, float v);

}
```

### gswt_renderer_amd/csrc/gswt_kernels.hip

```cpp
#include "gswt_device.h"

namespace gswt {

__device__ __forceinline__ unsigned long long ballot64(bool p) { return __builtin_amdgcn_ballot_w64(p); }
__device__ __forceinline__ uint32_t lanes_below(unsigned long long m)
{
    return __builtin_amdgcn_mbcnt_hi((uint32_t)(m >> 32), __builtin_amdgcn_mbcnt_lo((uint32_t)m, 0u));
}

template <int CTRL, int ROW_MASK>
__device__ __forceinline__ uint32_t dpp_or_zero(uint32_t x)
{
    return (uint32_t)__builtin_amdgcn_update_dpp(0, (int)x, CTRL, ROW_MASK, 0xF, true);
}
__device__ __forceinline__ uint32_t wave_incl_scan(uint32_t v, uint32_t lane)
{
    (void)lane;
    v += dpp_or_zero<0x111, 0xF>(v);
    v += dpp_or_zero<0x112, 0xF>(v);
    v += dpp_or_zero<0x114, 0xF>(v);
    v += dpp_or_zero<0x118, 0xF>(v);
    v += dpp_or_zero<0x142, 0xA>(v);
    v += dpp_or_zero<0x143, 0xC>(v);
    return v;
// ... 43 lines not shown
        const int x = (int)fx;
        if ((w & (w - 1)) == 0) return x & (w - 1);
        int r = x - w * (int)floorf((float)x / (float)w);
        if (r < 0) r += w;
        if (r >= w) r -= w;
        return r;
    }
    return wrap_repeat_slow(fx, w);
}

__device__ __forceinline__ float sample_height(const float* __restrict__ hm, int w, int h, float u, float v)
{
    float x = u * (float)w - 0.5f;
    float y = v * (float)h - 0.5f;
    float fx0 = floorf(x), fy0 = floorf(y);
    float tx = x - fx0, ty = y - fy0;
    const int xa = wrap_repeat(fx0, w), ya = wrap_repeat(fy0, h);
    const int yb = ya + 1 == h ? 0 : ya + 1;
    const float* r0 = hm + (size_t)ya * w + xa;
    const float* r1 = hm + (size_t)yb * w + xa;
    typedef float hm_pair __attribute__((ext_vector_type(2), aligned(4)));
    hm_pair p0 = *reinterpret_cast<const hm_pair*>(r0), p1 = *reinterpret_cast<const hm_pair*>(r1);
    if (xa + 1 == w) { p0.y = hm[(size_t)ya * w]; p1.y = hm[(size_t)yb * w]; }
    float i00 = p0.x, i10 = p0.y;
    float i01 = p1.x, i11 = p1.y;
    float i0 = i00 * (1.0f - tx) + i10 * tx;
    float i1 = i01 * (1.0f - tx) + i11 * tx;
    return i0 * (1.0f - ty) + i1 * ty;
}

__device__ __forceinline__ void csincosf(float x, float& sn, float& cs)
{
    const float kf = rintf(x * 0.636619772367581343f);
    float r = fmaf(kf, -1.5703125f, x);
    r = fmaf(kf, -4.837512969970703125e-4f, r);
    r = fmaf(kf, -7.54978995489188216e-8f, r);
    const float z = r * r;
    float ps = fmaf(-1.9515295891e-4f, z, 8.3321608736e-3f);
    ps = fmaf(ps, z, -1.6666654611e-1f);
    const float s = fmaf(ps * z, r, r);
    float pc = fmaf(2.443315711809948e-5f, z, -1.388731625493765e-3f);
    pc = fmaf(pc, z, 4.166664568298827e-2f);
    const float c = fmaf(pc * z, z, fmaf(-0.5f, z, 1.0f));
    const int q = (int)kf & 3;
    float so = (q & 1) ? c : s, co = (q & 1) ? s : c;
    if (q == 2 || q == 3) so = -so;
    if (q == 1 || q == 2) co = -co;
    sn = so; cs = co;
}

__device__ __forceinline__ void sphere_point(float block_w, float bidx, float bidy, float bx, float by, float p[3])
{
    const float PI = 3.1415926535897932384626433832795f;
    float u, v;
    if (bidy == 0.0f) {
        if (by < bx) {
            if (bx - by == block_w) u = 0.0f;
            else u = (by / (block_w - (bx - by)) + bidx) / 5.0f;
            v = ((block_w - (bx - by)) / block_w) / 3.0f;
        } else {
            u = (bx / block_w + bidx) / 5.0f + ((by - bx) / block_w) * 0.1f;
            v = ((by - bx) / block_w) / 3.0f + (1.0f / 3.0f);
        }
    } else {
        if (by < bx) {
            u = (bx / block_w + bidx) / 5.0f + ((block_w - (bx - by)) / block_w) * 0.1f;
            v = ((block_w - (bx - by)) / block_w) / 3.0f + (1.0f / 3.0f);
        } else {
            if (by - bx == block_w) u = 0.0f;
            else u = (bx / (block_w - (by - bx)) + bidx) / 5.0f + 0.1f;
            v = ((by - bx) / block_w) / 3.0f + (2.0f / 3.0f);
        }
    }
    u = u + 0.5f * floorf(v);
    u = u * (2.0f * PI);
    v = (v - 0.5f) * PI;
    float su, cu, sv, cv;
    csincosf(u, su, cu);
    csincosf(v, sv, cv);
    p[0] = cv * cu; p[1] = cv * su; p[2] = sv;
}

__device__ __forceinline__ float dbg_rand(float cx, float cy)
{
    const float d = cx * 12.9898f + cy * 78.233f;
    float sn, cs;
    csincosf(d, sn, cs);
    const float v = sn * 43758.5453f;
    return v - floorf(v);
}

__device__ __forceinline__ void debug_draw_color(const Frame& f, const DrawDev& d, float vx, float vy, uint32_t lod_id, float t_ratio,
                                                 float& cr, float& cg, float& cb)
{
    const float tw = f.tile_width;
    if (f.draw_mode == 1u) {
        const float g = clampf(((cr + cg) + cb) / 0.6f, 0.0f, 1.0f);
        cr = cg = cb = g;
        const float margin = 0.05f * tw;
        const bool sphere = f.surface_type == 2u;
        if (d.single_draw == 1u) {
            cr = cr * dbg_rand(d.off[0], d.off[1]);
            cg = cg * dbg_rand(d.off[0] + 23.45f, d.off[1] + 23.45f);
            cb = cb * dbg_rand(d.off[0] + 67.89f, d.off[1] + 67.89f);
        } else if (vx < margin || vx > tw - margin) {
            const uint32_t bit = vx < margin ? d.tile_idx / 8u % 2u : d.tile_idx / 2u % 2u;
            if (vy < margin || vy > tw - margin) { cr = cg = cb = 0.5f; }
            else if (bit == 0u) { cr = 1.0f; cg = 0.0f; cb = 0.0f; }
            else { cr = 0.0f; cg = 1.0f; cb = 0.13f; }
        } else if (vy < margin || vy > tw - margin) {
            const uint32_t bit = vy < margin ? d.tile_idx % 2u : d.tile_idx / 4u % 2u;
            if (bit == 0u) {
                if (sphere) { cr = 1.0f; cg = 0.0f; cb = 0.0f; } else { cr = 1.0f; cg = 0.85f; cb = 0.0f; }
            } else {
                if (sphere) { cr = 0.0f; cg = 1.0f; cb = 0.13f; } else { cr = 0.0f; cg = 0.58f; cb = 1.0f; }
            }
        }
    } else if (f.draw_mode == 2u || f.draw_mode == 3u) {
        if (t_ratio > 0.0f && t_ratio < 1.0f) { cr = cg = cb = 0.0f; return; }
        if (f.draw_mode == 2u && d.changing == 1u) { cr = 0.0f; cg = 1.0f; cb = 0.0f; return; }
        uint32_t L = d.tile_lod;
        if (f.draw_mode == 3u) L = d.single_lod_id >= 0 ? (uint32_t)d.single_lod_id : lod_id;
        float cx = 0.0f, cy = 1.0f;
        if (L < 3u) cx = (3.0f - (float)L) / 3.0f;
        else cy = (6.0f - (float)L) / 3.0f;
        cr = 0.5f; cg = cx; cb = cy;
    } else if (f.draw_mode == 4u) {
        const uint32_t v = d.tile_view;
        float cx = 0.0f, cy = 0.0f;
        if (v < 4u) cx = (4.0f - (float)v) / 4.0f;
        if (v >= 4u) cy = (8.0f - (float)v) / 4.0f;
        if (v >= 8u) { cx = 1.0f; cy = 1.0f; }
        cr = 0.5f; cg = cx; cb = cy;
    }
}

__device__ __forceinline__ void tile_xy(const Frame& f, uint32_t tile, int& tx, int& ty)
{
    uint32_t q;
    if (f.tiles_x_magic != 0u && tile < 65536u) q = __umulhi(tile, f.tiles_x_magic);
    else q = tile / (uint32_t)f.tiles_x;
    tx = (int)(tile - q * (uint32_t)f.tiles_x); ty = (int)q;
}

__device__ __forceinline__ int owned_rows(int ty0, int ty1, int index, int count)
{
    if (count <= 1) return ty1 - ty0 + 1;
    int first = ty0 + ((index - ty0 % count) + count) % count;
    if (first > ty1) return 0;
    return (ty1 - first) / count + 1;
}

struct XcdLens { uint32_t len[8]; uint32_t longest; };
__global__ __launch_bounds__(256) void k_chunk_tabs(const DrawDev* __restrict__ draws, const uint32_t* __restrict__ xcd_first, uint32_t n_draws,
                                                    uint2* __restrict__ chunk_tab, uint2* __restrict__ chunk_tab_xcd, const XcdLens xl)
{
    const uint32_t d = blockIdx.x;
    if (d >= n_draws) {
        const uint32_t x = d - n_draws;
        for (uint32_t k = xl.len[x & 7u] + threadIdx.x; k < xl.longest; k += 256u) chunk_tab_xcd[(size_t)k * 8u + x] = make_uint2(0xFFFFFFFFu, 0xFFFFFFFFu);
        return;
    }
    const uint32_t nch = (draws[d].count + (uint32_t)kChunk - 1u) / (uint32_t)kChunk;
    const uint32_t c0 = draws[d].slot_base / (uint32_t)kChunk, x0 = xcd_first[d];
    for (uint32_t k = threadIdx.x; k < nch; k += 256u) {
        const uint2 e = make_uint2(d, k * (uint32_t)kChunk);
        chunk_tab[c0 + k] = e;
        chunk_tab_xcd[(size_t)(x0 + k) * 8u + (draws[d].xcd & 7u)] = e;
    }
}

__device__ __forceinline__ bool sphere_cell_box(const Frame& f, float bidx, float bidy, const float lo[3], const float hi[3], float blo[3], float bhi[3])
{
    const float xmax = ((float)f.map_half_wh[0] * 2.0f) * f.tile_width;
    const float block_w = xmax / 5.0f;
    const float ox = (float)(f.center_coord[0] - (int32_t)f.map_half_wh[0]) * f.tile_width + bidx * block_w;
    const float oy = (float)(f.center_coord[1] - (int32_t)f.map_half_wh[1]) * f.tile_width + bidy * block_w;
    const float bx0 = lo[0] - ox, bx1 = hi[0] - ox, by0 = lo[1] - oy, by1 = hi[1] - oy;
    if (!(block_w > 0.0f && bx0 >= 0.0f && bx1 <= block_w && by0 >= 0.0f && by1 <= block_w)) return false;
    constexpr int n = 3;
    const float R = fabsf(f.sphere_radius);
    const float zmax = fmaxf(fabsf(lo[2]), fabsf(hi[2]));
    const float rho = (R * 2.5f * ((bx1 - bx0) + (by1 - by0)) / (2.0f * (float)n * block_w) + zmax) * 1.02f + 1e-4f * R;
    if (!(rho == rho)) return false;
    for (int k = 0; k < 3; k++) { blo[k] = 3.402823466e+38f; bhi[k] = -3.402823466e+38f; }
    for (int j = 0; j < n; j++)
        for (int i = 0; i < n; i++) {
            float p[3];
            sphere_point(block_w, bidx, bidy, bx0 + (bx1 - bx0) * (((float)i + 0.5f) / (float)n), by0 + (by1 - by0) * (((float)j + 0.5f) / (float)n), p);
            for (int k = 0; k < 3; k++) { blo[k] = fminf(blo[k], p[k] * f.sphere_radius - rho); bhi[k] = fmaxf(bhi[k], p[k] * f.sphere_radius + rho); }
        }
    return blo[0] == blo[0] && bhi[0] == bhi[0] && blo[1] == blo[1] && bhi[1] == bhi[1] && blo[2] == blo[2] && bhi[2] == bhi[2];
}

__device__ __forceinline__ bool band_misses(const Frame& f, const float lo[3], const float hi[3], float bidx, float bidy)
{
    float blo[3], bhi[3];
    for (int k = 0; k < 3; k++) {
        const float a = lo[k] * f.scene_scale[k], b = hi[k] * f.scene_scale[k];
        blo[k] = fminf(a, b); bhi[k] = fmaxf(a, b);
    }
    if (f.surface_type == 1u) {
        const float zp = fmaxf(fabsf(blo[2]), fabsf(bhi[2])) * 1.0001f;
        blo[0] -= zp; bhi[0] += zp; blo[1] -= zp; bhi[1] += zp;
        blo[2] = f.surf_zlo - zp; bhi[2] = f.surf_zhi + zp;
    } else if (f.surface_type == 2u) {
        float slo[3], shi[3];
        if (!sphere_cell_box(f, bidx, bidy, blo, bhi, slo, shi)) return false;
        for (int k = 0; k < 3; k++) { blo[k] = slo[k]; bhi[k] = shi[k]; }
    }
    float xmin = 3.402823466e+38f, xmax = -3.402823466e+38f, wmin = 3.402823466e+38f;
    bool odd = false;
    for (int k = 0; k < 8; k++) {
        const float px = (k & 1) ? bhi[0] : blo[0];
        const float py = (k & 2) ? bhi[1] : blo[1];
        const float pz = (k & 4) ? bhi[2] : blo[2];
        const float cx = ((f.VP[0] * px + f.VP[4] * py) + f.VP[8] * pz) + f.VP[12];
        const float cw = ((f.VP[3] * px + f.VP[7] * py) + f.VP[11] * pz) + f.VP[15];
        wmin = fminf(wmin, cw);
        const float xp = (0.5f * (cx / cw) + 0.5f) * f.W;
        odd = odd || !(cw == cw) || !(xp == xp);
        xmin = fminf(xmin, xp); xmax = fmaxf(xmax, xp);
    }
    if (odd || !(wmin > 1e-6f && xmin == xmin && xmax == xmax)) return false;
    const float smax = fmaxf(fabsf(f.scene_scale[0]), fmaxf(fabsf(f.scene_scale[1]), fabsf(f.scene_scale[2])));
    const float hx = 1.3f * f.htan[0], hy = 1.3f * f.htan[1];
    const float jn2 = (f.focal[0] * f.focal[0] * (1.0f + hx * hx) + f.focal[1] * f.focal[1] * (1.0f + hy * hy)) / (wmin * wmin);
    const float lam = jn2 * smax * smax * fmaxf(f.loc_max_trace, 0.0f) * f.surf_f2;
    const float ss = fabsf(f.splat_scale);
    const float rad = fminf(2.0f * ss * sqrtf(lam), 1448.2f * ss) * 1.25f + 2.0f;
    if (!(rad == rad)) return false;
    return xmax + rad < (float)(f.col0 * kTile) || xmin - rad >= (float)(f.col1 * kTile);
}

__device__ __forceinline__ bool draw_is_culled(const Frame& f, const DrawDev& d)
{
    bool culled = false;
    if (d.cull_enable) {
        float mx = 3.402823466e+38f, my = 3.402823466e+38f, mz = -3.402823466e+38f;
        for (int ci = 0; ci < 4; ci++) {
            float px = d.corners[3 * ci], py = d.corners[3 * ci + 1], pz = d.corners[3 * ci + 2];
            float c4[4];
            for (int r = 0; r < 4; r++)
                c4[r] = ((f.VP[r] * px + f.VP[4 + r] * py) + f.VP[8 + r] * pz) + f.VP[12 + r] * 1.0f;
            float cx = c4[0] / c4[3], cy = c4[1] / c4[3], cz = c4[2] / c4[3];
            if (fabsf(cx) < mx) mx = fabsf(cx);
            if (fabsf(cy) < my) my = fabsf(cy);
            if (cz > mz) mz = cz;
        }
        float clip = f.culling_dist;
        if (mz < -clip || mx > clip || my > clip) culled = true;
    }
    if (!((f.lod_enable_mask >> (d.lod & 31u)) & 1u)) culled = true;
    if (!culled && f.band_cull && d.count && d.single_draw != 1u) {
        const float lo[3] = {f.loc_lo[0] + d.off[0], f.loc_lo[1] + d.off[1], f.loc_lo[2] + d.off[2]};
        const float hi[3] = {f.loc_hi[0] + d.off[0], f.loc_hi[1] + d.off[1], f.loc_hi[2] + d.off[2]};
        float bidx = 0.0f, bidy = 0.0f;
        if (f.surface_type == 2u) {
            bidx = (float)(5u * d.map_coord[0] / (f.map_half_wh[0] * 2u));
            bidy = (float)(2u * d.map_coord[1] / (f.map_half_wh[1] * 2u));
        }
        if (band_misses(f, lo, hi, bidx, bidy)) culled = true;
    }
    return culled;
}

__global__ __launch_bounds__(256) void k_cull(const Frame f, const DrawDev* __restrict__ draws, uint32_t* __restrict__ draw_culled,
                                              uint32_t* __restrict__ cell_culled, uint32_t n_cells,
                                              uint32_t* __restrict__ zero_a, uint32_t n_zero_a, uint32_t* __restrict__ zero_b, uint32_t n_zero_b,
                                              uint32_t* __restrict__ zero_c, uint32_t n_zero_c, uint32_t* __restrict__ zero_d, uint32_t n_zero_d,
                                              const uint2* __restrict__ chunk_tab, uint32_t n_chunks, const float* __restrict__ boxes, uint32_t chunk_cull,
                                              uint32_t* __restrict__ live_cnt, uint4* __restrict__ live_tab, uint32_t* __restrict__ live_cid)
{
    __shared__ uint32_t s_cnt[8], s_base[8];
    if (threadIdx.x < 8u) s_cnt[threadIdx.x] = 0u;
    const uint32_t gtid = blockIdx.x * 256u + threadIdx.x;
    for (uint32_t j = gtid; j < n_zero_a; j += gridDim.x * 256u) zero_a[j] = 0u;
    for (uint32_t j = gtid; j < n_zero_b; j += gridDim.x * 256u) zero_b[j] = 0u;
    for (uint32_t j = gtid; j < n_zero_c; j += gridDim.x * 256u) zero_c[j] = 0u;
    for (uint32_t j = gtid; j < n_zero_d; j += gridDim.x * 256u) zero_d[j] = 0u;
    if (f.band_cull) {
        const uint32_t map_wh_y = f.map_wh_y;
        for (uint32_t j = gtid; j < n_cells; j += gridDim.x * 256u) {
            const uint32_t mq = j / map_wh_y, mr = j % map_wh_y;
            const float ox = (float)((int32_t)(mq - f.map_half_wh[0]) + f.center_coord[0]) * f.tile_width;
            const float oy = (float)((int32_t)(mr - f.map_half_wh[1]) + f.center_coord[1]) * f.tile_width;
            const float lo[3] = {f.loc_lo[0] + ox, f.loc_lo[1] + oy, f.loc_lo[2]}, hi[3] = {f.loc_hi[0] + ox, f.loc_hi[1] + oy, f.loc_hi[2]};
            float bidx = 0.0f, bidy = 0.0f;
            if (f.surface_type == 2u) {
                bidx = (float)(5u * mq / (f.map_half_wh[0] * 2u));
                bidy = (float)(2u * mr / (f.map_half_wh[1] * 2u));
            }
            cell_culled[j] = band_misses(f, lo, hi, bidx, bidy) ? 1u : 0u;
        }
    }
    __syncthreads();
    const uint32_t c = blockIdx.x * 256u + threadIdx.x;
    bool live = false;
    uint4 e = make_uint4(0u, 0u, 0u, 0u);
    uint32_t x = 0, rank = 0;
    if (c < n_chunks) {
        const uint2 ct = chunk_tab[c];
        const DrawDev& d = draws[ct.x];
        const bool dc = draw_is_culled(f, d);
        if (ct.y == 0u) draw_culled[ct.x] = dc ? 1u : 0u;
        live = !dc && d.count != 0u;
        if (live && chunk_cull && d.merged == 0u && d.box_base != 0xFFFFFFFFu && f.surface_type <= 1u) {
            const float* b = boxes + 6u * (size_t)(d.box_base + (ct.y >> 8));
            float lo[3], hi[3];
#pragma unroll
            for (int k = 0; k < 3; k++) {
                const float a = (b[k] + d.off[k]) * f.scene_scale[k], z = (b[3 + k] + d.off[k]) * f.scene_scale[k];
                lo[k] = fminf(a, z); hi[k] = fmaxf(a, z);
            }
            if (f.surface_type == 1u) {
                const float zp = fmaxf(fabsf(lo[2]), fabsf(hi[2])) * 1.0001f + 1e-6f;
                lo[0] -= zp; hi[0] += zp; lo[1] -= zp; hi[1] += zp;
                lo[2] = f.surf_zlo - zp - 1e-4f * (fabsf(f.surf_zlo) + 1.0f); hi[2] = f.surf_zhi + zp + 1e-4f * (fabsf(f.surf_zhi) + 1.0f);
            }
            bool xp = true, xn = true, yp = true, yn = true, zn = true;
#pragma unroll
// ... 764 lines not shown
    constexpr int kSortItems = kSortBlock / kSortThreads, kSortWaves = kSortThreads / 64;
    uint32_t kmin = 0;
    if (krange) { uint32_t kmax; load_krange(krange, kmin, kmax); }
    const uint32_t n = clamped_count(n_ptr, n_cap);
    if (blockIdx.x * kSortBlock >= n) return;
#ifdef GSWT_TRACE
    const bool tr_on = threadIdx.x == 0 && blockIdx.x < 4096u;
    const uint32_t tr_item = kTraceItems / 2u + (shift ? 4096u : 0u) + blockIdx.x;
    GSWT_TR(0, GSWT_NOW())
#endif
    __shared__ uint32_t s_h[kSortWaves][256];
    __shared__ uint32_t s_g[256];
    __shared__ uint32_t s_w[4], s_w2[4];
    __shared__ uint32_t s_gs[2][256];
    __shared__ uint2 s_kv[kSortBlock];
    __shared__ uint32_t s_aux[AUX == 2 ? kSortBlock : 1];
    __shared__ uint16_t s_src[AUX == 1 ? kSortBlock : 1];
    const uint32_t w = threadIdx.x >> 6, lane = threadIdx.x & 63u;
    for (int k = 0; k < kSortWaves * 256 / kSortThreads; k++) (&s_h[0][0])[k * kSortThreads + threadIdx.x] = 0;
    __syncthreads();
    const uint32_t blk0 = blockIdx.x * kSortBlock;
    const uint32_t base = blk0 + w * (64 * kSortItems);
    uint32_t key[kSortItems], val[kSortItems], aux[AUX == 2 ? kSortItems : 1];
#pragma unroll
    for (int k = 0; k < kSortItems; k++) {
        const uint32_t i = min(base + (uint32_t)k * 64u + lane, n - 1u);
        key[k] = keys_in[i];
        val[k] = vals_in[i];
        if (AUX == 2) aux[AUX == 2 ? k : 0] = aux_in[i];
    }
    const uint32_t d = threadIdx.x & 255u;
    const bool dig = threadIdx.x < 256u;
    const uint32_t sb = blockIdx.x >> kSupShift;
    uint32_t pre = 0, g_tot = 0;
    if (dig) {
        uint32_t t[32];
#pragma unroll
        for (uint32_t u = 0; u < 32u; u++) {
            const uint32_t j = (sb << kSupShift) + u;
            t[u] = ghist[min(j, nblk - 1u) * 256u + d];
        }
        if (nsup <= kSupDirect && kSortThreads >= 512) {
        } else if (nsup <= kSupDirect) {
            uint32_t g[kSupDirect];
#pragma unroll
            for (uint32_t u = 0; u < kSupDirect; u++) g[u] = gsup[min(u, nsup - 1u) * 256u + d];
#pragma unroll
            for (uint32_t u = 0; u < kSupDirect; u++) { if (u < nsup) g_tot += g[u]; if (u < sb) pre += g[u]; }
        } else {
            g_tot = gtot[d];
            pre = gsup[(size_t)sb * 256u + d];
        }
#pragma unroll
        for (uint32_t u = 0; u < 32u; u++) if ((sb << kSupShift) + u < blockIdx.x) pre += t[u];
    } else if (nsup <= kSupDirect && kSortThreads >= 512 && threadIdx.x < 512u) {
        uint32_t g[kSupDirect], ge = 0, ga = 0;
#pragma unroll
        for (uint32_t u = 0; u < kSupDirect; u++) g[u] = gsup[min(u, nsup - 1u) * 256u + d];
#pragma unroll
        for (uint32_t u = 0; u < kSupDirect; u++) { if (u < nsup) ga += g[u]; if (u < sb) ge += g[u]; }
        s_gs[0][d] = ge; s_gs[1][d] = ga;
    }
#ifdef GSWT_TRACE
    { unsigned long long sink = key[0] + val[0] + pre; asm volatile("" :: "v"(sink)); }
    GSWT_TR(1, GSWT_NOW())
#endif
    constexpr bool kCachePeers = kSortItems <= 8;
    unsigned long long pm[kCachePeers ? kSortItems : 1];
#pragma unroll
    for (int k = 0; k < kSortItems; k++) {
        const bool valid = base + (uint32_t)k * 64u + lane < n;
        const uint32_t dgt = ((key[k] - kmin) >> shift) & mask;
        const unsigned long long peers = match_digit(dgt, valid, nbits);
        if (kCachePeers) pm[k] = peers;
        if (valid && lanes_below(peers) == 0u) atomicAdd(&s_h[w][dgt], (uint32_t)__popcll(peers));
    }
    GSWT_TR(2, GSWT_NOW())
    {
        const bool direct = nsup <= kSupDirect && kSortThreads >= 512;
        if (direct) {
            __syncthreads();
            if (dig) { pre += s_gs[0][d]; g_tot = s_gs[1][d]; }
        }
        uint32_t inc = wave_incl_scan(g_tot, lane);
        if (dig && lane == 63u) s_w[w] = inc;
        __syncthreads();
        uint32_t cnt[kSortWaves], blk_cnt = 0;
        if (dig) {
#pragma unroll
            for (int k = 0; k < kSortWaves; k++) { cnt[k] = s_h[k][d]; blk_cnt += cnt[k]; }
        }
        const uint32_t inc2 = wave_incl_scan(blk_cnt, lane);
        if (dig && lane == 63u) s_w2[w] = inc2;
        __syncthreads();
        if (dig) {
            uint32_t wb = 0, wb2 = 0;
            for (uint32_t i = 0; i < w; i++) { wb += s_w[i]; wb2 += s_w2[i]; }
            const uint32_t gbase = wb + inc - g_tot + pre;
            uint32_t lb = wb2 + inc2 - blk_cnt;
            s_g[d] = gbase - lb;
#pragma unroll
            for (int k = 0; k < kSortWaves; k++) { s_h[k][d] = lb; lb += cnt[k]; }
        }
    }
    __syncthreads();
    GSWT_TR(3, GSWT_NOW())
#pragma unroll
    for (int k = 0; k < kSortItems; k++) {
        uint32_t i = base + k * 64 + lane;
        bool valid = i < n;
        uint32_t dgt = valid ? (((key[k] - kmin) >> shift) & mask) : 0u;
        const unsigned long long peers = kCachePeers ? pm[kCachePeers ? k : 0] : match_digit(dgt, valid, nbits);
        const uint32_t rank = lanes_below(peers);
        uint32_t pos = 0;
        if (valid && rank == 0u) pos = atomicAdd(&s_h[w][dgt], (uint32_t)__popcll(peers));
        const int leader = valid ? (int)__ffsll((long long)peers) - 1 : (int)lane;
        pos = (uint32_t)__shfl((int)pos, leader, 64);
        if (valid) {
            s_kv[pos + rank] = make_uint2(key[k], val[k]);
            if (AUX == 2) s_aux[AUX == 2 ? pos + rank : 0u] = aux[AUX == 2 ? k : 0];
            if (AUX == 1) s_src[AUX == 1 ? pos + rank : 0u] = (uint16_t)(w * (64u * kSortItems) + (uint32_t)k * 64u + lane);
        }
    }
    __syncthreads();
    GSWT_TR(4, GSWT_NOW())
    const uint32_t n_blk = min((uint32_t)kSortBlock, n - blk0);
#pragma unroll
    for (int k = 0; k < kSortItems; k++) {
        const uint32_t i = (uint32_t)k * kSortThreads + threadIdx.x;
        if (i < n_blk) {
            const uint2 kv = s_kv[i];
            const uint32_t gp = s_g[((kv.x - kmin) >> shift) & mask] + i;
            vals_out[gp] = kv.y;
            if (AUX == 2) aux_out[gp] = s_aux[AUX == 2 ? i : 0u];
            if (AUX == 1) aux_out[gp] = aux_in[blk0 + s_src[AUX == 1 ? i : 0u]];
            if (!ranges) keys_out[gp] = kv.x;
            else {
                const uint32_t kp = s_kv[i == 0u ? 0u : i - 1u].x, kn = s_kv[min(i + 1u, n_blk - 1u)].x;
                if (i == 0u || kp != kv.x) atomicMax(&ranges[kv.x].x, ~gp);
                if (i == n_blk - 1u || kn != kv.x) atomicMax(&ranges[kv.x].y, gp + 1u);
            }
        }
    }
    GSWT_TR(5, GSWT_NOW())
}

__device__ __forceinline__ uint32_t mg_find_seg(const MergeSeg* __restrict__ segs, uint32_t n_segs, uint32_t e)
{
    uint32_t lo = 0, hi = n_segs;
    while (hi - lo > 1u) { const uint32_t mid = (lo + hi) >> 1; if (segs[mid].start <= e) lo = mid; else hi = mid; }
    return lo;
}

__global__ __launch_bounds__(256) void k_mg_minmax(const MergeSeg* __restrict__ segs, const uint2* __restrict__ blocks, const int32_t* __restrict__ raw,
                                                   MergeGroup* __restrict__ groups)
{
    __shared__ int32_t s_mn[4], s_mx[4];
    const uint2 b = blocks[blockIdx.x];
    const MergeSeg sg = segs[b.x];
    int32_t mn = 2147483647, mx = -2147483647 - 1;
#pragma unroll
    for (uint32_t k = 0; k < 4u; k++) {
        const uint32_t i = b.y + k * 256u + threadIdx.x;
        const int32_t d = raw[sg.src + min(i, sg.len - 1u)];
        mn = min(mn, d); mx = max(mx, d);
    }
    for (int off = 32; off > 0; off >>= 1) { mn = min(mn, __shfl_down(mn, off, 64)); mx = max(mx, __shfl_down(mx, off, 64)); }
    if ((threadIdx.x & 63u) == 0) { s_mn[threadIdx.x >> 6] = mn; s_mx[threadIdx.x >> 6] = mx; }
    __syncthreads();
    if (threadIdx.x == 0) {
        atomicMin(&groups[sg.group].mn, min(min(s_mn[0], s_mn[1]), min(s_mn[2], s_mn[3])));
        atomicMax(&groups[sg.group].mx, max(max(s_mx[0], s_mx[1]), max(s_mx[2], s_mx[3])));
    }
}

__global__ __launch_bounds__(256) void k_mg_keys(const MergeSeg* __restrict__ segs, const uint2* __restrict__ blocks, const int32_t* __restrict__ raw,
                                                 const MergeGroup* __restrict__ groups, uint32_t* __restrict__ keys, uint32_t* __restrict__ vals)
{
    const uint2 b = blocks[blockIdx.x];
    const MergeSeg sg = segs[b.x];
    const MergeGroup g = groups[sg.group];
    const float depth_inv = 65535.0f / (float)(int32_t)((uint32_t)g.mx - (uint32_t)g.mn);
#pragma unroll
    for (uint32_t k = 0; k < 4u; k++) {
        const uint32_t i = b.y + k * 256u + threadIdx.x;
        if (i >= sg.len) break;
        const int32_t d = raw[sg.src + i];
        const float v = floorf((float)(int32_t)((uint32_t)d - (uint32_t)g.mn) * depth_inv);
        int32_t bk;
        if (v != v) bk = 0;
        else if (v >= 2147483648.0f) bk = 2147483647;
        else if (v <= -2147483648.0f) bk = -2147483647 - 1;
        else bk = (int32_t)v;
        bk = min(max(bk, 0), 65535);
        const uint32_t e = sg.start + i;
        keys[e] = (sg.group << 16) | (uint32_t)bk;
        vals[e] = e;
    }
}

__global__ __launch_bounds__(256) void k_mg_final(const MergeSeg* __restrict__ segs, uint32_t n_segs, const MergeGroup* __restrict__ groups,
                                                  const uint32_t* __restrict__ sorted_keys, const uint32_t* __restrict__ sorted_vals,
                                                  uint32_t n_total, uint32_t* __restrict__ merged_list, uint32_t* __restrict__ merged_map)
{
    const uint32_t p = blockIdx.x * 256u + threadIdx.x;
    if (p >= n_total) return;
    const uint32_t g = sorted_keys[p] >> 16;
    const MergeGroup gr = groups[g];
    const uint32_t out = gr.out_base + (gr.len - 1u - (p - gr.base));
    const uint32_t e = sorted_vals[p];
    const MergeSeg sg = segs[mg_find_seg(segs, n_segs, e)];
    merged_list[out] = ((e - sg.start) + sg.gs_offset) | (sg.lod << kLodShift);
    merged_map[out] = sg.map_index;
}

__global__ __launch_bounds__(256) void k_mg_copy(const MergeCopy* __restrict__ jobs, const uint2* __restrict__ blocks, const uint2* __restrict__ remap,
                                                 const MergeSources src, uint32_t* __restrict__ new_list, uint32_t* __restrict__ new_map)
{
    __shared__ uint2 s_pairs[256];
    const uint2 b = blocks[blockIdx.x];
    const MergeCopy jb = jobs[b.x];
    const uint32_t* __restrict__ old_list = src.list[jb.src_set < (uint32_t)kMergeSources ? jb.src_set : 0u];
    const uint32_t* __restrict__ old_map = src.map[jb.src_set < (uint32_t)kMergeSources ? jb.src_set : 0u];
    const uint32_t np = min(jb.n_pairs, 256u);
    if (threadIdx.x < np) s_pairs[threadIdx.x] = remap[jb.first_pair + threadIdx.x];
    __syncthreads();
#pragma unroll
    for (uint32_t k = 0; k < 4u; k++) {
        const uint32_t i = b.y + k * 256u + threadIdx.x;
        if (i >= jb.len) break;
        new_list[jb.dst + i] = old_list[jb.src + i];
        uint32_t m = old_map[jb.src + i];
        for (uint32_t q = 0; q < np; q++) if (s_pairs[q].x == m) { m = s_pairs[q].y; break; }
        new_map[jb.dst + i] = m;
    }
}

constexpr uint32_t kTileSortCap = 16384u, kTileSortLongGrid = 256u;
template <bool WAVE>
__device__ __forceinline__ void tls_sync()
{
    if (WAVE) asm volatile("s_waitcnt lgkmcnt(0)" ::: "memory");
    else __syncthreads();
}
template <int THREADS, int ROUNDS, bool LONG, bool WAVE = false>
__device__ __forceinline__ void tile_depth_sort_one(uint32_t tile, const uint2* __restrict__ ranges, uint32_t* __restrict__ vals, const uint32_t* __restrict__ dkeys,
                                                    uint32_t* __restrict__ long_list, uint32_t* __restrict__ xl_list, unsigned long long* __restrict__ counters,
                                                    uint32_t n_lo, bool push, uint2* s_kv, uint32_t (*s_h)[256], uint32_t* s_w, uint32_t* s_mn, uint32_t* s_mx)
{
    constexpr uint32_t CAP = (uint32_t)(THREADS * ROUNDS);
    constexpr int NW = THREADS / 64;
    const uint2 rgv = ranges[__builtin_amdgcn_readfirstlane(tile)];
    const uint32_t rg_x = __builtin_amdgcn_readfirstlane(rgv.x), rg_y = __builtin_amdgcn_readfirstlane(rgv.y);
    if (rg_y == 0u) return;
    const uint32_t start = ~rg_x, n = rg_y - start;
    if (n <= max(n_lo, 1u)) return;
    if (n > CAP) {
        if ((WAVE ? (threadIdx.x & 63u) : threadIdx.x) == 0u && (LONG || push)) {
            if (LONG) counters[3] = 1ull;
            else {
                uint32_t* const lst = n > kTileSortCap ? xl_list : long_list;
                lst[1u + atomicAdd(&lst[0], 1u)] = tile;
            }
        }
        return;
    }
    static_assert(!WAVE || THREADS == 64, "wave-local mode is one wave");
    const uint32_t lane = threadIdx.x & 63u, w = WAVE ? 0u : __builtin_amdgcn_readfirstlane(threadIdx.x >> 6), tid = WAVE ? lane : threadIdx.x;
    const uint32_t rounds = (n + 63u) >> 6, rpw = (rounds + (uint32_t)NW - 1u) / (uint32_t)NW;
    const uint32_t base_w = w * rpw * 64u;
    uint32_t key[ROUNDS], val[ROUNDS];
    uint32_t mn = 0xFFFFFFFFu, mx = 0u;
#pragma unroll
    for (int k = 0; k < ROUNDS; k++) {
        key[k] = 0u; val[k] = 0u;
        if ((uint32_t)k >= rpw || base_w + (uint32_t)k * 64u >= n) continue;
        const uint32_t i = min(base_w + (uint32_t)k * 64u + lane, n - 1u);
        key[k] = dkeys[start + i];
        val[k] = vals[start + i];
        mn = min(mn, key[k]); mx = max(mx, key[k]);
    }
    mn = wave_min(mn); mx = wave_max(mx);
    if (lane == 0u) { s_mn[w] = mn; s_mx[w] = mx; }
    tls_sync<WAVE>();
#pragma unroll
    for (int q = 0; q < NW; q++) { mn = min(mn, s_mn[q]); mx = max(mx, s_mx[q]); }
    mn = __builtin_amdgcn_readfirstlane(mn); mx = __builtin_amdgcn_readfirstlane(mx);
    const uint32_t span = mx - mn;
    if (span == 0u) return;
    const uint32_t bits = 32u - (uint32_t)__clz((int)span), passes = (bits + 7u) >> 3, nb = (bits + passes - 1u) / passes, dmask = (1u << nb) - 1u;
#pragma unroll
    for (int k = 0; k < ROUNDS; k++) key[k] -= mn;
    for (uint32_t p = 0; p < passes; p++) {
        const uint32_t shift = nb * p;
        for (uint32_t q = tid; q < (uint32_t)NW * 256u; q += (uint32_t)THREADS) (&s_h[0][0])[q] = 0u;
        tls_sync<WAVE>();
        uint32_t pm[ROUNDS];
#pragma unroll
        for (int k = 0; k < ROUNDS; k++) {
            pm[k] = 0u;
            if ((uint32_t)k >= rpw || base_w + (uint32_t)k * 64u >= n) continue;
            const bool valid = base_w + (uint32_t)k * 64u + lane < n;
            const uint32_t dgt = (key[k] >> shift) & dmask;
            const unsigned long long peers = match_digit(dgt, valid, nb);
            const uint32_t rank = lanes_below(peers), cnt = (uint32_t)__popcll(peers);
            pm[k] = rank | (valid ? (uint32_t)(__ffsll((long long)peers) - 1) : lane) << 8 | cnt << 16;
            if (valid && rank == 0u) atomicAdd(&s_h[w][dgt], cnt);
        }
        tls_sync<WAVE>();
        constexpr int SCAN_T = THREADS < 256 ? THREADS : 256, DPT = 256 / SCAN_T;
        uint32_t cnt[DPT][NW], tot = 0, inc = 0;
        const bool dig = tid < (uint32_t)SCAN_T;
        const uint32_t d0 = (tid & (uint32_t)(SCAN_T - 1)) * (uint32_t)DPT;
        if (dig) {
#pragma unroll
            for (int j = 0; j < DPT; j++)
#pragma unroll
                for (int q = 0; q < NW; q++) { cnt[j][q] = s_h[q][d0 + (uint32_t)j]; tot += cnt[j][q]; }
            inc = wave_incl_scan(tot, lane);
            if (lane == 63u) s_w[w] = inc;
        }
        tls_sync<WAVE>();
        if (dig) {
            uint32_t b = inc - tot;
            for (uint32_t q = 0; q < w; q++) b += s_w[q];
#pragma unroll
            for (int j = 0; j < DPT; j++)
#pragma unroll
                for (int q = 0; q < NW; q++) { s_h[q][d0 + (uint32_t)j] = b; b += cnt[j][q]; }
        }
        tls_sync<WAVE>();
#pragma unroll
        for (int k = 0; k < ROUNDS; k++) {
            if ((uint32_t)k >= rpw || base_w + (uint32_t)k * 64u >= n) continue;
            const bool valid = base_w + (uint32_t)k * 64u + lane < n;
            const uint32_t dgt = (key[k] >> shift) & dmask;
            uint32_t pos = 0;
            if (valid && (pm[k] & 255u) == 0u) pos = atomicAdd(&s_h[w][dgt], pm[k] >> 16);
            pos = (uint32_t)__shfl((int)pos, (int)((pm[k] >> 8) & 255u), 64) + (pm[k] & 255u);
            if (valid) s_kv[pos] = make_uint2(key[k], val[k]);
        }
        tls_sync<WAVE>();
        if (p + 1u == passes) break;
#pragma unroll
        for (int k = 0; k < ROUNDS; k++) {
            const uint32_t i = base_w + (uint32_t)k * 64u + lane;
            if ((uint32_t)k < rpw && i < n) { const uint2 kv = s_kv[i]; key[k] = kv.x; val[k] = kv.y; }
        }
    }
    for (uint32_t i = tid; i < n; i += (uint32_t)THREADS) vals[start + i] = s_kv[i].y;
}

__device__ __forceinline__ void tile_depth_sort_xl(const uint2* __restrict__ ranges, uint32_t* vals_a, uint32_t* keys_a, uint32_t* vals_b,
                                                   uint32_t* keys_b, uint32_t n_tiles, const uint32_t* __restrict__ long_list,
                                                   uint32_t (*s_h)[256], uint32_t* s_w, uint32_t* s_mn, uint32_t* s_mx)
{
    constexpr uint32_t NW = 16u;
    const uint32_t* const xl_list = long_list + n_tiles + 1u;
    const uint32_t n_xl = min(xl_list[0], n_tiles);
    const uint32_t lane = threadIdx.x & 63u, w = __builtin_amdgcn_readfirstlane(threadIdx.x >> 6);
    for (uint32_t t = blockIdx.x; t < n_xl; t += gridDim.x) {
        const uint2 rgv = ranges[__builtin_amdgcn_readfirstlane(xl_list[1u + t])];
        const uint32_t start = ~(uint32_t)__builtin_amdgcn_readfirstlane(rgv.x), n = (uint32_t)__builtin_amdgcn_readfirstlane(rgv.y) - start;
        const uint32_t per = ((n + NW * 64u - 1u) / (NW * 64u)) * 64u;
        const uint32_t lo = min(w * per, n), hi = min(lo + per, n);
        uint32_t mn = 0xFFFFFFFFu, mx = 0u;
        for (uint32_t i = lo + lane; i < hi; i += 64u) { const uint32_t k = keys_a[start + i]; mn = min(mn, k); mx = max(mx, k); }
        mn = wave_min(mn); mx = wave_max(mx);
        if (lane == 0u) { s_mn[w] = mn; s_mx[w] = mx; }
        __syncthreads();
#pragma unroll
        for (uint32_t q = 0; q < NW; q++) { mn = min(mn, s_mn[q]); mx = max(mx, s_mx[q]); }
        mn = __builtin_amdgcn_readfirstlane(mn); mx = __builtin_amdgcn_readfirstlane(mx);
        const uint32_t span = mx - mn;
        uint32_t passes = 0, nb = 8u;
        if (span != 0u) { const uint32_t bits = 32u - (uint32_t)__clz((int)span); passes = (bits + 7u) >> 3; nb = (bits + passes - 1u) / passes; }
        const uint32_t dmask = (1u << nb) - 1u;
        uint32_t* src_k = keys_a; uint32_t* src_v = vals_a; uint32_t* dst_k = keys_b; uint32_t* dst_v = vals_b;
        for (uint32_t p = 0; p < passes; p++) {
            const uint32_t shift = nb * p;
            for (uint32_t q = threadIdx.x; q < NW * 256u; q += 1024u) (&s_h[0][0])[q] = 0u;
            __syncthreads();
            for (uint32_t r = lo; r < hi; r += 64u) {
                const bool valid = r + lane < hi;
                const uint32_t dgt = ((src_k[start + min(r + lane, hi - 1u)] - mn) >> shift) & dmask;
                const unsigned long long peers = match_digit(dgt, valid, nb);
                if (valid && lanes_below(peers) == 0u) atomicAdd(&s_h[w][dgt], (uint32_t)__popcll(peers));
// ... 559 lines not shown
    bool wave_live = true, counted_dead = false;
    if (tid < NBUF) {
        s_staged[tid] = 0u; s_done[tid] = 0u;
        comp_null_record<DEPTH || ZOUT, COLF>(s_q0, s_q1, s_q2, s_dep, tid * BS + B);
    }
    if (tid == 0) s_dead = 0u;
    const uint32_t n_pairs = rg.y - rg.x;
    const uint32_t nb = (n_pairs + B - 1u) / B;
    const uint32_t last_pair = rg.y - 1u;
    const uint32_t half = wave & 1u;
    uint32_t ks = wave >> 1, sb = wave >> 1, su = 0u;
    float4 ra = make_float4(0.f, 0.f, 0.f, 0.f), rb = ra, rd = ra;
    float rbw = 0.f;
    uint32_t slot_nxt = 0;
#define GSWT_DW_PAIR(KB) min(rg.x + (KB) * B + half * 64u + lane, last_pair)
#define GSWT_DW_LOAD(SLOT)                                                                           \
        {                                                                                           \
            const float4* rp = reinterpret_cast<const float4*>(recs + (SLOT));                      \
            ra = rp[0];                                                                             \
            rb = rp[1];                                                                             \
            if (DEPTH || ZOUT) rbw = depths[(SLOT)];                                                \
            if (COLF) rd = col_f[(SLOT)];                                                           \
        }
    if (n_pairs) {
        const uint32_t slot0 = vals[GSWT_DW_PAIR(ks)];
        GSWT_DW_LOAD(slot0)
        slot_nxt = vals[GSWT_DW_PAIR(ks + 2u)];
    }
    __syncthreads();
    uint32_t kb = 0u, ku = 0u;
    bool all_dead = false;
    for (uint32_t k = 0; k < nb && !all_dead; k++) {
        while (ks < nb && ks <= k + 2u) {
            const uint32_t need = 4u * su;
            if (lds_peek(&s_done[sb]) < need) {
                if (ks > k) break;
                while (lds_peek(&s_done[sb]) < need) {
                    if (EARLY && lds_peek(&s_dead) == 4u) { all_dead = true; break; }
                    __builtin_amdgcn_s_sleep(kDwSleep);
                }
                if (all_dead) break;
            }
            __builtin_amdgcn_fence(__ATOMIC_ACQUIRE, "workgroup");
            const uint32_t li = half * 64u + lane;
            if (ks * B + li < n_pairs) comp_stage<DEPTH || ZOUT, COLF>(hW, hHn, c0x, c0y, ra, rb, rbw, rd, s_q0, s_q1, s_q2, s_dep, s_bb, sb * BS + li, sb * B + li);
            __builtin_amdgcn_fence(__ATOMIC_RELEASE, "workgroup");
            if (lane == 0u) atomicAdd(&s_staged[sb], 1u);
            ks += 2u; sb += 2u; if (sb >= 3u) { sb -= 3u; su += 1u; }
            GSWT_DW_LOAD(slot_nxt)
            slot_nxt = vals[GSWT_DW_PAIR(ks + 2u)];
        }
        if (all_dead) break;
        {
            const uint32_t target = 2u * (ku + 1u);
            while (lds_peek(&s_staged[kb]) < target) {
                if (EARLY && lds_peek(&s_dead) == 4u) { all_dead = true; break; }
                __builtin_amdgcn_s_sleep(kDwSleep);
            }
            if (all_dead) break;
            __builtin_amdgcn_fence(__ATOMIC_ACQUIRE, "workgroup");
        }
        const uint32_t n = min(B, n_pairs - k * B);
        if (wave_live)
            composite_bin_walk<EARLY, DEPTH, COLF, ZOUT, B>(f, cl, n, s_q0 + kb * BS, s_q1 + kb * BS, s_q2 + (COLF ? kb * BS : 0u), s_bb + kb * B,
                                                            s_dep + ((DEPTH || ZOUT) ? kb * BS : 0u), wlist, dbuf, t_eps, T, ar, ag, ab, az, wave_live);
        __builtin_amdgcn_fence(__ATOMIC_RELEASE, "workgroup");
        if (lane == 0u) {
            atomicAdd(&s_done[kb], 1u);
            if (EARLY && !wave_live && !counted_dead) atomicAdd(&s_dead, 1u);
        }
        if (EARLY && !wave_live) counted_dead = true;
        kb += 1u; if (kb >= 3u) { kb = 0u; ku += 1u; }
        if (EARLY && lds_peek(&s_dead) == 4u) all_dead = true;
    }
#undef GSWT_DW_PAIR
#undef GSWT_DW_LOAD
    const float k255 = 1.0f / 255.0f;
    if (!COLF) { ar *= k255; ag *= k255; ab *= k255; }
    if (multi_seg) {
        const size_t pi = (size_t)(item_base[tile] + (it.y >> 1)) * 256u + tid;
        partials[pi] = make_float4(ar, ag, ab, T);
        if (ZOUT) partials_z[pi] = az;
        return;
    }
    uint32_t tid2 = threadIdx.x;
    asm volatile("" : "+v"(tid2));
    const int lxi2 = (int)(((tid2 & 63u) >> 4) * 4u + (tid2 & 3u)), lyi2 = (int)((tid2 >> 6) * 4u + ((tid2 & 15u) >> 2));
    const int px2 = bx + lxi2, py2 = by + lyi2;
    if (px2 < f.width && py2 < f.height)
        comp_final_pixel<OUTF, ZOUT>(f, bg_rgba, out, out_rows, px2, py2, tyl * kTile + lyi2, T, ar, ag, ab, bg_depth, out_depth, az);
}

template <int OUTF, bool ZOUT>
__global__ __launch_bounds__(256) void k_combine(const Frame f, const uint32_t* __restrict__ item_base,
                                                 const float4* __restrict__ partials, const float4* __restrict__ bg_rgba,
                                                 float4* __restrict__ out, int n_tiles, int out_rows,
                                                 const unsigned long long* __restrict__ counters, unsigned long long* __restrict__ host_counters,
                                                 const float* __restrict__ partials_z, const float* __restrict__ bg_depth, float* __restrict__ out_depth)
{
    const int tile = blockIdx.x;
    if (tile == 0 && threadIdx.x < 5u && host_counters) host_counters[threadIdx.x] = counters[threadIdx.x];
    const uint32_t i0 = item_base[tile], n_seg = item_base[tile + 1] - i0;
    if (n_seg == 1u) return;
    const auto [tyl, bx, by] = comp_tile(f, (uint32_t)tile);
    const uint32_t tid = threadIdx.x, wave = tid >> 6, lane = tid & 63u;
    const uint32_t grp = lane >> 4, gi = lane & 15u;
    const int lxi = (int)grp * 4 + (int)(gi & 3u);
    const int lyi = (int)wave * 4 + (int)(gi >> 2);
    const int px = bx + lxi, py = by + lyi;
    if (px >= f.width || py >= f.height) return;
    float T = 1.0f, ar = 0.0f, ag = 0.0f, ab = 0.0f, az = 0.0f;
    for (uint32_t s0 = 0; s0 < n_seg; s0 += 8u) {
        float4 p[8];
        float pz[8];
#pragma unroll
        for (uint32_t k = 0; k < 8u; k++) {
            const size_t pi = (size_t)(i0 + min(s0 + k, n_seg - 1u)) * 256u + tid;
            p[k] = partials[pi];
            if (ZOUT) pz[k] = partials_z[pi];
        }
#pragma unroll
        for (uint32_t k = 0; k < 8u; k++) {
            if (s0 + k < n_seg) {
                ar = fmaf(T, p[k].x, ar);
                ag = fmaf(T, p[k].y, ag);
                ab = fmaf(T, p[k].z, ab);
                if (ZOUT) az = fmaf(T, pz[k], az);
                T = T * p[k].w;
            }
        }
    }
    comp_final_pixel<OUTF, ZOUT>(f, bg_rgba, out, out_rows, px, py, tyl * kTile + lyi, T, ar, ag, ab, bg_depth, out_depth, az);
}

template <typename P>
__global__ void k_unshard(const P* __restrict__ gathered, P* __restrict__ out, int width, int height,
                          int shard_count, int rows_padded, int band_px)
{
    int x = blockIdx.x * blockDim.x + threadIdx.x;
    int y = blockIdx.y;
    if (x >= width || y >= height) return;
    size_t src;
    if (band_px > 0) {
        const int shard = x / band_px;
        src = ((size_t)shard * height + y) * band_px + (x - shard * band_px);
    } else {
        int ty = y >> 4;
        int shard = ty % shard_count, tyl = ty / shard_count;
        src = ((size_t)shard * rows_padded + (size_t)tyl * kTile + (y & 15)) * width + x;
    }
    out[(size_t)y * width + x] = gathered[src];
}

void launch_chunk_tabs(hipStream_t s, const DrawDev* draws, const uint32_t* xcd_first, uint32_t n_draws, uint2* chunk_tab, uint2* chunk_tab_xcd,
                       const uint64_t per_xcd[8], uint64_t longest)
{
    XcdLens xl;
    for (int x = 0; x < 8; x++) xl.len[x] = (uint32_t)per_xcd[x];
    xl.longest = (uint32_t)longest;
    if (n_draws) hipLaunchKernelGGL(k_chunk_tabs, dim3(n_draws + 8u), dim3(256), 0, s, draws, xcd_first, n_draws, chunk_tab, chunk_tab_xcd, xl);
}

GraphRec*& graph_recorder()
{
    static thread_local GraphRec* rec = nullptr;
    return rec;
}

bool kernel_events_enabled()
{
    static const bool on = !(getenv("GSWT_KERNEL_EVENTS") && atoi(getenv("GSWT_KERNEL_EVENTS")) == 0);
    return on;
}

void launch_cull(hipStream_t s, const Frame& f, const FrameBufs& b, bool chunk_cull)
{
    uint32_t grid = (b.n_chunks + 255u) / 256u;
    if (grid < 32) grid = 32;
    GSWT_LAUNCH(k_cull, dim3(grid), dim3(256), s, f, b.draws, b.draw_culled, b.cell_culled, b.n_cells, reinterpret_cast<uint32_t*>(b.counters), b.n_zero_head,
                reinterpret_cast<uint32_t*>(b.ranges), b.n_zero_ranges, b.block_sums, b.n_chunks, b.radix_depth, b.n_zero_depth,
                b.chunk_tab, b.n_chunks, b.boxes, chunk_cull && b.boxes ? 1u : 0u, b.live_cnt, b.live_tab, b.live_cid);
}

void launch_project(hipStream_t s, const Frame& f, const FrameBufs& b, uint32_t n_launch, bool debug, bool strict)
{
    if (b.n_chunks == 0) return;
    const uint32_t n_super = b.n_chunks / 256u + 1u;
    const bool full = f.surface_type == 2u || f.draw_mode != 0u;
#define GSWT_LAUNCH_PROJECT_S(D, F, S)                                                                                         \
    GSWT_LAUNCH((k_project<D, F, S>), dim3(n_launch), dim3(256), s, f, b.draws, b.chunk_tab_xcd, b.static_list, b.merged_list,   \
                b.merged_map, b.tex, b.hmap, b.draw_culled, b.cell_culled, b.live_cnt, b.live_tab, b.rects, b.recs, b.depths, b.block_sums, \
                b.super_sums, n_super, b.dbg, b.col_f)
#define GSWT_LAUNCH_PROJECT(D, F) do { if (strict) GSWT_LAUNCH_PROJECT_S(D, F, true); else GSWT_LAUNCH_PROJECT_S(D, F, false); } while (0)
    if (debug && full) { GSWT_LAUNCH_PROJECT(true, true); }
    else if (debug) { GSWT_LAUNCH_PROJECT(true, false); }
    else if (full) { GSWT_LAUNCH_PROJECT(false, true); }
    else { GSWT_LAUNCH_PROJECT(false, false); }
#undef GSWT_LAUNCH_PROJECT
#undef GSWT_LAUNCH_PROJECT_S
    GSWT_LAUNCH(k_totals, dim3(1), dim3(256), s, b.super_sums, n_super, b.counters, b.super_sums + 2u * kSuperStride * n_super, b.pair_cap, b.live_cnt, n_launch / 8u);
}

void launch_emit(hipStream_t s, const Frame& f, const FrameBufs& b, uint32_t* keys, uint32_t* dkeys, uint32_t* krange, uint32_t n_launch)
{
    const uint32_t n_chunks = b.n_chunks, pair_cap = b.pair_cap;
    if (n_chunks == 0) return;
    const uint32_t n_super = n_chunks / 256u + 1u;
    const uint32_t* const excl = b.super_sums + 2u * kSuperStride * n_super;
    const float* const no_f = nullptr; uint32_t* const no_u = nullptr;
    const uint32_t* const cnt2 = n_launch ? b.live_cnt + 8u * kSuperStride : nullptr;
    const uint32_t* const cid = n_launch ? b.live_cid : nullptr;
    const dim3 grid(n_launch ? ((n_launch / 8u + kEmitGroup - 1u) / kEmitGroup) * 8u : (n_chunks + kEmitGroup - 1u) / kEmitGroup);
#define GSWT_LAUNCH_EMIT(D, L)                                                                                                 \
    GSWT_LAUNCH((k_emit<D, L>), grid, dim3(256), s, f, b.rects, b.block_sums, excl, n_chunks, pair_cap, b.counters, keys, b.vals_a, \
                D ? b.depths : no_f, D ? dkeys : no_u, D ? krange : no_u, cnt2, cid)
    if (n_launch) { if (dkeys) GSWT_LAUNCH_EMIT(true, true); else GSWT_LAUNCH_EMIT(false, true); }
    else if (dkeys) GSWT_LAUNCH_EMIT(true, false);
    else GSWT_LAUNCH_EMIT(false, false);
#undef GSWT_LAUNCH_EMIT
}

size_t radix_ws_words(uint32_t n_cap, int key_bits)
{
    const uint32_t nblk = (n_cap + kSortBlock - 1) / kSortBlock, nsup = (nblk >> kSupShift) + 1;
    const int passes = (key_bits + 7) / 8;
    return (size_t)passes * ((size_t)256 * nblk + (size_t)256 * nsup + 256);
}
size_t radix_ws_zero_words(uint32_t n_cap, int key_bits)
{
    const uint32_t nblk = (n_cap + kSortBlock - 1) / kSortBlock, nsup = (nblk >> kSupShift) + 1;
    const int passes = (key_bits + 7) / 8;
    return (size_t)passes * ((size_t)256 * nsup + 256);
}

int launch_sort(hipStream_t s, uint32_t* keys_a, uint32_t* vals_a, uint32_t* keys_b, uint32_t* vals_b, uint32_t n_cap,
                const unsigned long long* n_ptr, int key_bits, uint32_t* ws, uint2* ranges, const uint32_t* krange, uint32_t* aux_a, uint32_t* aux_b)
{
    if (n_cap == 0) return 0;
    const uint32_t nblk = (n_cap + kSortBlock - 1) / kSortBlock, nsup = (nblk >> kSupShift) + 1;
    const int threads = n_cap <= kSortWideMax ? 512 : 256;
    int cur = 0;
    const int passes = (key_bits + 7) / 8;
    uint32_t* hist_rows = ws + (size_t)passes * ((size_t)256 * nsup + 256);
    for (int shift = 0; shift < key_bits; shift += 8) {
        uint32_t nbits = (uint32_t)((key_bits - shift) < 8 ? (key_bits - shift) : 8);
        uint32_t mask = (1u << nbits) - 1u;
        uint32_t* gsup = ws; uint32_t* gtot = gsup + (size_t)256 * nsup;
        ws = gtot + 256;
        uint32_t* ghist = hist_rows;
        hist_rows += (size_t)256 * nblk;
        uint32_t* ki = cur ? keys_b : keys_a; uint32_t* vi = cur ? vals_b : vals_a;
        uint32_t* ko = cur ? keys_a : keys_b; uint32_t* vo = cur ? vals_a : vals_b;
        const uint32_t* xi = cur ? aux_b : aux_a; uint32_t* xo = cur ? aux_a : aux_b;
#define GSWT_SORT_PASS(T)                                                                                                        \
        GSWT_LAUNCH(k_radix_hist<T>, dim3(nblk), dim3(T), s, ki, n_ptr, n_cap, (uint32_t)shift, mask, nbits, ghist, gsup, gtot, nblk, nsup, krange); \
        if (nsup > kSupDirect) GSWT_LAUNCH(k_radix_supscan, dim3(64), dim3(256), s, gsup, gtot, nsup);                          \
        if (aux_a && n_cap > (12u << 20)) GSWT_LAUNCH((k_radix_scatter<T, 2>), dim3(nblk), dim3(T), s, ki, vi, ko, vo, n_ptr, n_cap, (uint32_t)shift, mask, nbits, \
                           ghist, gsup, gtot, nblk, nsup, shift + 8 >= key_bits ? ranges : (uint2*)nullptr, krange, xi, xo);                  \
        else if (aux_a) GSWT_LAUNCH((k_radix_scatter<T, 1>), dim3(nblk), dim3(T), s, ki, vi, ko, vo, n_ptr, n_cap, (uint32_t)shift, mask, nbits,    \
                           ghist, gsup, gtot, nblk, nsup, shift + 8 >= key_bits ? ranges : (uint2*)nullptr, krange, xi, xo);                  \
        else GSWT_LAUNCH((k_radix_scatter<T, 0>), dim3(nblk), dim3(T), s, ki, vi, ko, vo, n_ptr, n_cap, (uint32_t)shift, mask, nbits,    \
                           ghist, gsup, gtot, nblk, nsup, shift + 8 >= key_bits ? ranges : (uint2*)nullptr, krange, xi, xo)
        if (threads == 512) { GSWT_SORT_PASS(512); }
        else { GSWT_SORT_PASS(256); }
#undef GSWT_SORT_PASS
        cur ^= 1;
    }
    return cur;
}

void launch_merge_build(hipStream_t s, const MergeSeg* segs, uint32_t n_segs, const uint2* blocks, uint32_t n_blocks, MergeGroup* groups, uint32_t n_groups,
                        const int32_t* raw, uint32_t n_total, const unsigned long long* n_total_dev, uint32_t* ka, uint32_t* va,
                        uint32_t* kb, uint32_t* vb, uint32_t* radix_ws, int group_bits, uint32_t* merged_list, uint32_t* merged_map)
{
    if (n_total == 0 || n_groups == 0 || n_blocks == 0) return;
    hipLaunchKernelGGL(k_mg_minmax, dim3(n_blocks), dim3(256), 0, s, segs, blocks, raw, groups);
    hipLaunchKernelGGL(k_mg_keys, dim3(n_blocks), dim3(256), 0, s, segs, blocks, raw, groups, ka, va);
    const int where = launch_sort(s, ka, va, kb, vb, n_total, n_total_dev, 16 + group_bits, radix_ws);
    hipLaunchKernelGGL(k_mg_final, dim3((n_total + 255) / 256), dim3(256), 0, s, segs, n_segs, groups, where ? kb : ka, where ? vb : va,
                       n_total, merged_list, merged_map);
}

int launch_scene_sort(hipStream_t s, const MergeSeg* segs, const uint2* blocks, uint32_t n_blocks, MergeGroup* groups, const int32_t* raw,
                      uint32_t n_total, const unsigned long long* n_total_dev, uint32_t* ka, uint32_t* va, uint32_t* kb, uint32_t* vb,
                      uint32_t* radix_ws, int group_bits)
{
    if (n_total == 0 || n_blocks == 0) return 0;
    hipLaunchKernelGGL(k_mg_minmax, dim3(n_blocks), dim3(256), 0, s, segs, blocks, raw, groups);
    hipLaunchKernelGGL(k_mg_keys, dim3(n_blocks), dim3(256), 0, s, segs, blocks, raw, groups, ka, va);
    return launch_sort(s, ka, va, kb, vb, n_total, n_total_dev, 16 + group_bits, radix_ws);
}

void launch_merge_copy(hipStream_t s, const MergeCopy* jobs, const uint2* blocks, uint32_t n_blocks, const uint2* remap, const MergeSources& src,
                       uint32_t* new_list, uint32_t* new_map)
{
    if (n_blocks) hipLaunchKernelGGL(k_mg_copy, dim3(n_blocks), dim3(256), 0, s, jobs, blocks, remap, src, new_list, new_map);
}

void launch_tile_depth_sort(hipStream_t s, const uint2* ranges, uint32_t* vals, uint32_t* dkeys, uint32_t* vals_scratch, uint32_t* dkeys_scratch, int n_tiles,
                            uint32_t* long_list, unsigned long long* counters)
{
    if (n_tiles <= 0) return;
    const uint32_t nt = (uint32_t)n_tiles;
    GSWT_LAUNCH((k_tile_depth_sort<64, 8, false>), dim3(nt), dim3(64), s, ranges, vals, dkeys, nt, long_list, counters, 0u, 0u, vals_scratch, dkeys_scratch);
    GSWT_LAUNCH((k_tile_depth_sort<256, 16, false>), dim3(nt), dim3(256), s, ranges, vals, dkeys, nt, long_list, counters, 512u, 1u, vals_scratch, dkeys_scratch);
    GSWT_LAUNCH((k_tile_depth_sort<1024, 16, true>), dim3(kTileSortLongGrid), dim3(1024), s, ranges, vals, dkeys, nt, long_list, counters, 4096u, 0u,
                vals_scratch, dkeys_scratch);
}
uint32_t tile_depth_sort_cap() { return kTileSortCap; }

template <typename Fn>
static void with_composite_edc(const Frame& f, Fn&& fn)
{
    const bool early = f.t_eps > 0.0f, depth = f.has_depth != 0, colf = f.draw_mode != 0u;
    using T = std::true_type;
    using F = std::false_type;
    if (colf) { if (depth) fn(F{}, T{}, T{}); else fn(F{}, F{}, T{}); }
    else if (early && depth) fn(T{}, T{}, F{});
    else if (early) fn(T{}, F{}, F{});
    else if (depth) fn(F{}, T{}, F{});
    else fn(F{}, F{}, F{});
}

template <int OUTF, bool ZOUT>
static void launch_composite_t(hipStream_t s, const Frame& f, const FrameBufs& b, const uint32_t* vals, int out_rows, int variant, const uint32_t* krange,
                               uint32_t depth_passes, bool report_max, bool heavy_first, hipEvent_t ev_begin, hipEvent_t ev_end)
{
    const int n_tiles = (int)b.n_tiles;
    const uint32_t seg = b.seg;
    if (n_tiles == 0) {
        if (ev_begin) hipEventRecord(ev_begin, s);
        if (ev_end) hipEventRecord(ev_end, s);
        return;
    }
    const uint32_t max_items = (uint32_t)n_tiles + b.pair_cap / seg + 1u;
    if (heavy_first)
        GSWT_LAUNCH(k_items<true>, dim3((n_tiles + 8191) / 8192), dim3(1024), s, b.ranges, n_tiles, seg, b.item_base, b.item_tab, max_items, krange, depth_passes, b.counters,
                    report_max ? 1u : 0u);
    else
        GSWT_LAUNCH(k_items<false>, dim3((n_tiles + 8191) / 8192), dim3(1024), s, b.ranges, n_tiles, seg, b.item_base, b.item_tab, max_items, krange, depth_passes, b.counters,
                    report_max ? 1u : 0u);
    with_composite_edc(f, [&](auto E, auto D, auto C) {
        if (variant == 1)
            GSWT_LAUNCH_TIMED((k_composite_dw<E, D, C, OUTF, ZOUT>), dim3(max_items), dim3(256), s, ev_begin, ev_end, f, b.item_base, b.item_tab, vals, b.recs,
                              b.depths, b.col_f, b.bg_rgba, b.bg_depth, b.out, b.partials, n_tiles, out_rows, b.out_depth, b.partials_z);
        else
            GSWT_LAUNCH_TIMED((k_composite<E, D, C, OUTF, ZOUT>), dim3(max_items), dim3(256), s, ev_begin, ev_end, f, b.ranges, b.item_base, b.item_tab, seg, vals,
                              b.recs, b.depths, b.col_f, b.bg_rgba, b.bg_depth, b.out, b.partials, n_tiles, out_rows, b.out_depth, b.partials_z);
    });
    GSWT_LAUNCH((k_combine<OUTF, ZOUT>), dim3(n_tiles), dim3(256), s, f, b.item_base, b.partials, b.bg_rgba, b.out, n_tiles, out_rows,
                (const unsigned long long*)b.counters, b.host_counters, (const float*)b.partials_z, b.bg_depth, b.out_depth);
}

template <int OUTF>
static void launch_composite_z(hipStream_t s, const Frame& f, const FrameBufs& b, const uint32_t* vals, int out_rows, int variant, const uint32_t* krange,
                               uint32_t depth_passes, bool report_max, bool heavy_first, hipEvent_t ev_begin, hipEvent_t ev_end)
{
    if (b.out_depth) launch_composite_t<OUTF, true>(s, f, b, vals, out_rows, variant, krange, depth_passes, report_max, heavy_first, ev_begin, ev_end);
    else launch_composite_t<OUTF, false>(s, f, b, vals, out_rows, variant, krange, depth_passes, report_max, heavy_first, ev_begin, ev_end);
}

void launch_composite(hipStream_t s, const Frame& f, const FrameBufs& b, const uint32_t* vals, int out_rows, int variant, const uint32_t* krange,
                      uint32_t depth_passes, bool report_max, bool heavy_first, hipEvent_t ev_begin, hipEvent_t ev_end, int out_format)
{
    if (out_format == kOutRGBA8) launch_composite_z<kOutRGBA8>(s, f, b, vals, out_rows, variant, krange, depth_passes, report_max, heavy_first, ev_begin, ev_end);
    else if (out_format == kOutBGRA8) launch_composite_z<kOutBGRA8>(s, f, b, vals, out_rows, variant, krange, depth_passes, report_max, heavy_first, ev_begin, ev_end);
    else launch_composite_z<kOutF32>(s, f, b, vals, out_rows, variant, krange, depth_passes, report_max, heavy_first, ev_begin, ev_end);
}

void launch_totals(hipStream_t s, uint32_t* super_sums, uint32_t n_super, unsigned long long* counters, uint32_t pair_cap)
{
    hipLaunchKernelGGL(k_totals, dim3(1), dim3(256), 0, s, super_sums, n_super, counters, super_sums + 2u * kSuperStride * n_super, pair_cap, (uint32_t*)nullptr, 0xFFFFFFFFu);
}

void launch_unshard(hipStream_t s, const void* gathered, void* out, int width, int height, int shard_count, int rows_padded, int band_px,
                    int out_format)
{
    const dim3 grid((width + 255) / 256, height);
    if (out_format == kOutF32)
        hipLaunchKernelGGL(k_unshard<float4>, grid, dim3(256), 0, s, static_cast<const float4*>(gathered), static_cast<float4*>(out), width, height,
                           shard_count, rows_padded, band_px);
    else
        hipLaunchKernelGGL(k_unshard<uint32_t>, grid, dim3(256), 0, s, static_cast<const uint32_t*>(gathered), static_cast<uint32_t*>(out), width,
                           height, shard_count, rows_padded, band_px);
}

}
#ifdef GSWT_TRACE
extern "C" __attribute__((visibility("default"))) int gswt_debug_trace(unsigned long long* out, unsigned n_items)
{
    hipDeviceSynchronize();
    if (n_items > gswt::kTraceItems) n_items = gswt::kTraceItems;
    return (int)hipMemcpyFromSymbol(out, HIP_SYMBOL(gswt::g_trace), (size_t)n_items * 64);
}
#endif
#ifdef GSWT_STATS
extern "C" __attribute__((visibility("default"))) int gswt_debug_stats(unsigned long long* out)
{
    hipDeviceSynchronize();
    return (int)hipMemcpyFromSymbol(out, HIP_SYMBOL(gswt::g_stats), 64);
}
#endif
```

Before: 5544.

## Fuse per-event prep kernels and replace global merge radix sort with segmented sort

Merges chunk-table building, merge-copy and min/max reduction into one k_event_pre launch with role-based workgroup dispatch. The chunk-table role now packs four draws per workgroup. When every group spans at most a bounded number of 1024-entry blocks, the global radix sort over the merged depth keys is replaced by a two-pass, per-group segmented 8-bit radix sort (hist plus scatter kernels). The aim is to cut launch count, the radix workspace memset and global sort passes in the per-event scene update. The cost is more complex device code and a size-dependent fallback path.

```diff
diff --git a/gswt_renderer_amd/csrc/gswt_api.hip b/gswt_renderer_amd/csrc/gswt_api.hip
--- a/gswt_renderer_amd/csrc/gswt_api.hip
+++ b/gswt_renderer_amd/csrc/gswt_api.hip
@@ -86,7 +86,7 @@
     HostBuf<uint8_t> h_blob;
     DevBuf<uint8_t> d_blob;
     size_t blob_bytes = 0;
-    size_t off_draws = 0, off_xcd = 0, off_groups = 0, off_jobs = 0, off_remap = 0, off_segs = 0, off_blocks = 0, off_cblocks = 0, off_n64 = 0;
+    size_t off_draws = 0, off_xcd = 0, off_groups = 0, off_jobs = 0, off_remap = 0, off_segs = 0, off_blocks = 0, off_cblocks = 0, off_gblocks = 0, off_n64 = 0;
     template <typename T> T* hp(size_t off) { return reinterpret_cast<T*>(h_blob.p + off); }
     template <typename T> T* dp(size_t off) { return reinterpret_cast<T*>(d_blob.p + off); }
     hipError_t plan(size_t n_draws, size_t n_groups, size_t n_members, size_t total_entries)
@@ -97,7 +97,8 @@
         off_draws = take((n_draws + 1) * sizeof(DrawDev)); off_xcd = take((n_draws + 1) * 4);
         off_groups = take((n_groups + 1) * sizeof(MergeGroup)); off_jobs = take((n_groups + 1) * sizeof(MergeCopy));
         off_remap = take((n_members + 1) * sizeof(uint2)); off_segs = take((2 * n_members + 1) * sizeof(MergeSeg));
-        off_blocks = take(n_blk * sizeof(uint2)); off_cblocks = take(n_blk * sizeof(uint2)); off_n64 = take(64);
+        off_blocks = take(n_blk * sizeof(uint2)); off_cblocks = take(n_blk * sizeof(uint2)); off_gblocks = take(n_blk * sizeof(uint2));
+        off_n64 = take(64);
         blob_bytes = o;
         hipError_t e = o <= h_blob.cap ? hipSuccess : h_blob.ensure(2 * o);
         if (e != hipSuccess) return e;
@@ -247,6 +248,7 @@
     std::vector<uint32_t> raw_off;
     std::vector<uint32_t> raw_cnt, raw_merge_offset;
 
+    uint32_t mg_seg_max_blocks = kMgSegMaxBlocks;
     int opt_no_merge_reuse = 0;
     unsigned long long stat_groups_built = 0, stat_groups_reused = 0, stat_groups_reused_deep = 0;
     DevBuf<uint32_t> mg_ws;
@@ -431,6 +433,7 @@
     gswt_ctx* c = new (std::nothrow) gswt_ctx();
     if (!c) return GSWT_ERR_CAPACITY;
     c->device = device_id;
+    if (const char* mb = getenv("GSWT_MERGE_SEG_MAX_BLOCKS")) c->mg_seg_max_blocks = (uint32_t)std::min<long>(std::max<long>(atol(mb), 0), (long)kMgSegMaxBlocks);
     const char* layout = getenv("GSWT_STREAM_LAYOUT");
     if (!layout || !*layout) layout = kStreamLayout;
     for (const char* q = layout; *q; q++) {
@@ -701,7 +704,7 @@
                 const uint32_t g = (uint32_t)(l * n_tile + t);
                 MergeGroup G;
                 G.base = build; G.len = list_len(l, t); G.mn = 2147483647; G.mx = -2147483647 - 1;
-                G.out_base = lists[(size_t)g * nv + v].pair_base; G._pad[0] = G._pad[1] = G._pad[2] = 0;
+                G.out_base = lists[(size_t)g * nv + v].pair_base; G.blk0 = G.n_blk0 = G.blk1 = 0;
                 groups.push_back(G);
                 for (size_t q = l; q < (size_t)n_lod && q <= l + 1; q++) {
                     const size_t lt = q * n_tile + t;
@@ -974,7 +977,10 @@
     if (!device_merge) {
         hipStream_t s = c->set_stream;
         HIP_TRY(c, hipMemcpyAsync(D.d_blob.p, D.h_blob.p, D.blob_bytes, hipMemcpyHostToDevice, s));
-        launch_chunk_tabs(s, D.draws.p, D.xcd_first.p, (uint32_t)n_draws, D.chunk_tab.p, D.chunk_tab_xcd.p, D.per_xcd, D.longest);
+        EventPreArgs pre = {};
+        pre.draws = D.draws.p; pre.xcd_first = D.xcd_first.p; pre.n_draws = (uint32_t)n_draws; pre.chunk_tab = D.chunk_tab.p; pre.chunk_tab_xcd = D.chunk_tab_xcd.p;
+        pre.per_xcd = D.per_xcd; pre.longest = D.longest;
+        launch_event_pre(s, pre);
         HIP_TRY(c, hipGetLastError());
         HIP_TRY(c, hipEventRecord(D.ev_up, s));
         D.ev_up_pending = true; D.built = false;
@@ -1150,7 +1156,7 @@
             if (match_rank > 0) c->stat_groups_reused_deep++;
         } else if (len) {
             MergeGroup& B = grp[n_build];
-            B.base = (uint32_t)build_total; B.len = (uint32_t)len; B.mn = 2147483647; B.mx = -2147483647 - 1; B.out_base = (uint32_t)total; B._pad[0] = B._pad[1] = B._pad[2] = 0;
+            B.base = (uint32_t)build_total; B.len = (uint32_t)len; B.mn = 2147483647; B.mx = -2147483647 - 1; B.out_base = (uint32_t)total; B.blk0 = B.n_blk0 = B.blk1 = 0;
             for (uint32_t m = 0; m < G.n_members; m++) {
                 const gswt_merge_member& M = members[G.first_member + m];
                 const int lods[2] = {(int)M.lod, M.other_lod};
@@ -1193,30 +1199,50 @@
     hipStream_t s = c->set_stream;
     uint2* const h_cblocks = D.hp<uint2>(D.off_cblocks);
     uint2* const h_blocks = D.hp<uint2>(D.off_blocks);
-    size_t n_cb = 0, n_blocks = 0;
+    uint2* const h_gblocks = D.hp<uint2>(D.off_gblocks);
+    size_t n_cb = 0, n_blocks = 0, n_gb = 0;
+    uint32_t longest_group = 0;
     for (size_t q = 0; q < n_jobs; q++)
         for (uint32_t off = 0; off < jobs[q].len; off += 1024u) h_cblocks[n_cb++] = make_uint2((uint32_t)q, off);
-    for (size_t q = 0; q < n_segs; q++)
-        for (uint32_t off = 0; off < segs[q].len; off += 1024u) h_blocks[n_blocks++] = make_uint2((uint32_t)q, off);
+    for (size_t q = 0; q < n_segs; q++) {
+        MergeGroup& B = grp[segs[q].group];
+        if (!B.n_blk0) B.blk0 = (uint32_t)n_blocks;
+        for (uint32_t off = 0; off < segs[q].len; off += 1024u) { h_blocks[n_blocks++] = make_uint2((uint32_t)q, off); B.n_blk0++; }
+        longest_group = std::max(longest_group, B.n_blk0);
+    }
+    for (size_t g = 0; g < n_build; g++) {
+        grp[g].blk1 = (uint32_t)n_gb;
+        for (uint32_t off = 0; off < grp[g].len; off += 1024u) h_gblocks[n_gb++] = make_uint2((uint32_t)g, off);
+    }
     const uint32_t n_total = (uint32_t)build_total;
     memset(D.hp<uint8_t>(D.off_n64), 0, 64);
     *D.hp<unsigned long long>(D.off_n64) = n_total;
+    const bool seg_sort = longest_group <= c->mg_seg_max_blocks;
+    int gbits = 1;
+    while ((1u << gbits) < n_build) gbits++;
+    if (n_build) {
+        const size_t words = seg_sort ? merge_seg_ws_words(n_total, (uint32_t)n_blocks, (uint32_t)n_gb) : 4 * (size_t)n_total + radix_ws_words(n_total, 16 + gbits) + 16;
+        HIP_TRY(c, c->mg_ws.ensure_roomy(words));
+    }
     HIP_TRY(c, hipMemcpyAsync(D.d_blob.p, D.h_blob.p, D.blob_bytes, hipMemcpyHostToDevice, s));
-    launch_chunk_tabs(s, D.draws.p, D.xcd_first.p, D.n_draws, D.chunk_tab.p, D.chunk_tab_xcd.p, D.per_xcd, D.longest);
-    if (n_jobs)
-        launch_merge_copy(s, D.dp<MergeCopy>(D.off_jobs), D.dp<uint2>(D.off_cblocks), (uint32_t)n_cb, D.dp<uint2>(D.off_remap), msrc,
-                          D.merged_list.p, D.merged_map.p);
-    if (n_build) {
-        int gbits = 1;
-        while ((1u << gbits) < n_build) gbits++;
-        const size_t radix_words = radix_ws_words(n_total, 16 + gbits);
-        HIP_TRY(c, c->mg_ws.ensure_roomy(4 * (size_t)n_total + radix_words + 16));
+    EventPreArgs pre = {};
+    pre.draws = D.draws.p; pre.xcd_first = D.xcd_first.p; pre.n_draws = D.n_draws; pre.chunk_tab = D.chunk_tab.p; pre.chunk_tab_xcd = D.chunk_tab_xcd.p;
+    pre.per_xcd = D.per_xcd; pre.longest = D.longest;
+    pre.jobs = D.dp<MergeCopy>(D.off_jobs); pre.cblocks = D.dp<uint2>(D.off_cblocks); pre.n_cblocks = (uint32_t)n_cb; pre.remap = D.dp<uint2>(D.off_remap); pre.src = &msrc;
+    pre.segs = D.dp<MergeSeg>(D.off_segs); pre.blocks = D.dp<uint2>(D.off_blocks); pre.n_blocks = n_build ? (uint32_t)n_blocks : 0u; pre.raw = c->raw_depth.p;
+    pre.groups = D.dp<MergeGroup>(D.off_groups);
+    pre.merged_list = D.merged_list.p; pre.merged_map = D.merged_map.p;
+    launch_event_pre(s, pre);
+    if (n_build && seg_sort) {
+        launch_merge_build_seg(s, pre.segs, (uint32_t)n_segs, pre.blocks, (uint32_t)n_blocks, D.dp<uint2>(D.off_gblocks), (uint32_t)n_gb, pre.groups,
+                               c->raw_depth.p, n_total, c->mg_ws.p, D.merged_list.p, D.merged_map.p);
+    } else if (n_build) {
         uint32_t* w = c->mg_ws.p;
         uint32_t* radix = w + 4 * (size_t)n_total;
-        HIP_TRY(c, hipMemsetAsync(radix, 0, (radix_words + 16) * 4, s));
-        launch_merge_build(s, D.dp<MergeSeg>(D.off_segs), (uint32_t)n_segs, D.dp<uint2>(D.off_blocks), (uint32_t)n_blocks, D.dp<MergeGroup>(D.off_groups),
-                           (uint32_t)n_build, c->raw_depth.p, n_total, D.dp<unsigned long long>(D.off_n64), w, w + n_total, w + 2 * (size_t)n_total,
-                           w + 3 * (size_t)n_total, radix, gbits, D.merged_list.p, D.merged_map.p);
+        HIP_TRY(c, hipMemsetAsync(radix, 0, (radix_ws_words(n_total, 16 + gbits) + 16) * 4, s));
+        launch_merge_build_global(s, pre.segs, (uint32_t)n_segs, pre.blocks, (uint32_t)n_blocks, pre.groups, (uint32_t)n_build, c->raw_depth.p, n_total,
+                                  D.dp<unsigned long long>(D.off_n64), w, w + n_total, w + 2 * (size_t)n_total, w + 3 * (size_t)n_total, radix, gbits,
+                                  D.merged_list.p, D.merged_map.p);
     }
     HIP_TRY(c, hipGetLastError());
     HIP_TRY(c, hipEventRecord(D.ev_up, s));
diff --git a/gswt_renderer_amd/csrc/gswt_device.h b/gswt_renderer_amd/csrc/gswt_device.h
--- a/gswt_renderer_amd/csrc/gswt_device.h
+++ b/gswt_renderer_amd/csrc/gswt_device.h
@@ -83,7 +83,8 @@
     uint32_t base, len;
     int32_t mn, mx;
     uint32_t out_base;
-    uint32_t _pad[3];
+    uint32_t blk0, n_blk0;
+    uint32_t blk1;
 };
 struct MergeCopy {
     uint32_t src, dst, len;
@@ -235,11 +236,21 @@
     uint32_t n_zero_head, n_zero_ranges, n_zero_depth;
 };
 
-void launch_chunk_tabs(hipStream_t s, const DrawDev* draws, const uint32_t* xcd_first, uint32_t n_draws, uint2* chunk_tab, uint2* chunk_tab_xcd,
-                       const uint64_t per_xcd[8], uint64_t longest);
-void launch_merge_build(hipStream_t s, const MergeSeg* segs, uint32_t n_segs, const uint2* blocks, uint32_t n_blocks, MergeGroup* groups, uint32_t n_groups,
-                        const int32_t* raw, uint32_t n_total, const unsigned long long* n_total_dev, uint32_t* ka, uint32_t* va,
-                        uint32_t* kb, uint32_t* vb, uint32_t* radix_ws, int group_bits, uint32_t* merged_list, uint32_t* merged_map);
+struct EventPreArgs {
+    const DrawDev* draws; const uint32_t* xcd_first; uint32_t n_draws; uint2* chunk_tab; uint2* chunk_tab_xcd; const uint64_t* per_xcd; uint64_t longest;
+    const MergeCopy* jobs; const uint2* cblocks; uint32_t n_cblocks; const uint2* remap; const MergeSources* src;
+    const MergeSeg* segs; const uint2* blocks; uint32_t n_blocks; const int32_t* raw; MergeGroup* groups;
+    uint32_t* merged_list; uint32_t* merged_map;
+};
+void launch_event_pre(hipStream_t s, const EventPreArgs& a);
+constexpr uint32_t kMgSegMaxBlocks = 512;
+size_t merge_seg_ws_words(uint32_t n_total, uint32_t n_blocks, uint32_t n_gblocks);
+void launch_merge_build_seg(hipStream_t s, const MergeSeg* segs, uint32_t n_segs, const uint2* blocks, uint32_t n_blocks, const uint2* gblocks,
+                            uint32_t n_gblocks, const MergeGroup* groups, const int32_t* raw, uint32_t n_total, uint32_t* ws,
+                            uint32_t* merged_list, uint32_t* merged_map);
+void launch_merge_build_global(hipStream_t s, const MergeSeg* segs, uint32_t n_segs, const uint2* blocks, uint32_t n_blocks, MergeGroup* groups, uint32_t n_groups,
+                               const int32_t* raw, uint32_t n_total, const unsigned long long* n_total_dev, uint32_t* ka, uint32_t* va,
+                               uint32_t* kb, uint32_t* vb, uint32_t* radix_ws, int group_bits, uint32_t* merged_list, uint32_t* merged_map);
 int launch_scene_sort(hipStream_t s, const MergeSeg* segs, const uint2* blocks, uint32_t n_blocks, MergeGroup* groups, const int32_t* raw,
                       uint32_t n_total, const unsigned long long* n_total_dev, uint32_t* ka, uint32_t* va, uint32_t* kb, uint32_t* vb,
                       uint32_t* radix_ws, int group_bits);
@@ -251,8 +262,6 @@
 void launch_scene_self(hipStream_t s, const SceneList* lists, uint32_t n_lists, uint32_t lists_per_lod, uint32_t* arena);
 void launch_scene_boxes(hipStream_t s, const SceneList* lists, uint32_t n_lists, uint32_t n_boxes, const uint32_t* arena, const uint4* tex,
                         uint32_t n_splats, float* boxes);
-void launch_merge_copy(hipStream_t s, const MergeCopy* jobs, const uint2* blocks, uint32_t n_blocks, const uint2* remap, const MergeSources& src,
-                       uint32_t* new_list, uint32_t* new_map);
 
 void launch_cull(hipStream_t s, const Frame& f, const FrameBufs& b, bool chunk_cull);
 void launch_project(hipStream_t s, const Frame& f, const FrameBufs& b, uint32_t n_launch, bool debug, bool strict);
diff --git a/gswt_renderer_amd/csrc/gswt_kernels.hip b/gswt_renderer_amd/csrc/gswt_kernels.hip
--- a/gswt_renderer_amd/csrc/gswt_kernels.hip
+++ b/gswt_renderer_amd/csrc/gswt_kernels.hip
@@ -219,21 +219,24 @@
 }
 
 struct XcdLens { uint32_t len[8]; uint32_t longest; };
-__global__ __launch_bounds__(256) void k_chunk_tabs(const DrawDev* __restrict__ draws, const uint32_t* __restrict__ xcd_first, uint32_t n_draws,
-                                                    uint2* __restrict__ chunk_tab, uint2* __restrict__ chunk_tab_xcd, const XcdLens xl)
-{
-    const uint32_t d = blockIdx.x;
-    if (d >= n_draws) {
-        const uint32_t x = d - n_draws;
+__host__ __device__ __forceinline__ uint32_t chunk_tabs_workgroups(uint32_t n_draws) { return n_draws ? (n_draws + 3u) / 4u + 8u : 0u; }
+__device__ __forceinline__ void chunk_tabs_role(uint32_t wg, const DrawDev* __restrict__ draws, const uint32_t* __restrict__ xcd_first, uint32_t n_draws,
+                                                uint2* __restrict__ chunk_tab, uint2* __restrict__ chunk_tab_xcd, const XcdLens& xl)
+{
+    const uint32_t n_dw = (n_draws + 3u) / 4u;
+    if (wg >= n_dw) {
+        const uint32_t x = wg - n_dw;
         for (uint32_t k = xl.len[x & 7u] + threadIdx.x; k < xl.longest; k += 256u) chunk_tab_xcd[(size_t)k * 8u + x] = make_uint2(0xFFFFFFFFu, 0xFFFFFFFFu);
         return;
     }
+    const uint32_t d = wg * 4u + (threadIdx.x >> 6);
+    if (d >= n_draws) return;
     const uint32_t nch = (draws[d].count + (uint32_t)kChunk - 1u) / (uint32_t)kChunk;
-    const uint32_t c0 = draws[d].slot_base / (uint32_t)kChunk, x0 = xcd_first[d];
-    for (uint32_t k = threadIdx.x; k < nch; k += 256u) {
+    const uint32_t c0 = draws[d].slot_base / (uint32_t)kChunk, x0 = xcd_first[d], xcd = draws[d].xcd & 7u;
+    for (uint32_t k = threadIdx.x & 63u; k < nch; k += 64u) {
         const uint2 e = make_uint2(d, k * (uint32_t)kChunk);
         chunk_tab[c0 + k] = e;
-        chunk_tab_xcd[(size_t)(x0 + k) * 8u + (draws[d].xcd & 7u)] = e;
+        chunk_tab_xcd[(size_t)(x0 + k) * 8u + xcd] = e;
     }
 }
 
@@ -1304,11 +1307,12 @@
     return lo;
 }
 
-__global__ __launch_bounds__(256) void k_mg_minmax(const MergeSeg* __restrict__ segs, const uint2* __restrict__ blocks, const int32_t* __restrict__ raw,
-                                                   MergeGroup* __restrict__ groups)
+constexpr uint32_t kMgBlock = 1024;
+__device__ __forceinline__ void mg_minmax_block(uint32_t blk, const MergeSeg* __restrict__ segs, const uint2* __restrict__ blocks, const int32_t* __restrict__ raw,
+                                                MergeGroup* __restrict__ groups)
 {
     __shared__ int32_t s_mn[4], s_mx[4];
-    const uint2 b = blocks[blockIdx.x];
+    const uint2 b = blocks[blk];
     const MergeSeg sg = segs[b.x];
     int32_t mn = 2147483647, mx = -2147483647 - 1;
 #pragma unroll
@@ -1326,29 +1330,47 @@
     }
 }
 
+__global__ __launch_bounds__(256) void k_mg_minmax(const MergeSeg* __restrict__ segs, const uint2* __restrict__ blocks, const int32_t* __restrict__ raw,
+                                                   MergeGroup* __restrict__ groups)
+{
+    mg_minmax_block(blockIdx.x, segs, blocks, raw, groups);
+}
+
+__device__ __forceinline__ float mg_depth_inv(const MergeGroup& g) { return 65535.0f / (float)(int32_t)((uint32_t)g.mx - (uint32_t)g.mn); }
+__device__ __forceinline__ uint32_t mg_bucket(int32_t d, int32_t mn, float depth_inv)
+{
+    const float v = floorf((float)(int32_t)((uint32_t)d - (uint32_t)mn) * depth_inv);
+    int32_t bk;
+    if (v != v) bk = 0;
+    else if (v >= 2147483648.0f) bk = 2147483647;
+    else if (v <= -2147483648.0f) bk = -2147483647 - 1;
+    else bk = (int32_t)v;
+    return (uint32_t)min(max(bk, 0), 65535);
+}
+
 __global__ __launch_bounds__(256) void k_mg_keys(const MergeSeg* __restrict__ segs, const uint2* __restrict__ blocks, const int32_t* __restrict__ raw,
                                                  const MergeGroup* __restrict__ groups, uint32_t* __restrict__ keys, uint32_t* __restrict__ vals)
 {
     const uint2 b = blocks[blockIdx.x];
     const MergeSeg sg = segs[b.x];
     const MergeGroup g = groups[sg.group];
-    const float depth_inv = 65535.0f / (float)(int32_t)((uint32_t)g.mx - (uint32_t)g.mn);
+    const float depth_inv = mg_depth_inv(g);
 #pragma unroll
     for (uint32_t k = 0; k < 4u; k++) {
         const uint32_t i = b.y + k * 256u + threadIdx.x;
         if (i >= sg.len) break;
-        const int32_t d = raw[sg.src + i];
-        const float v = floorf((float)(int32_t)((uint32_t)d - (uint32_t)g.mn) * depth_inv);
-        int32_t bk;
-        if (v != v) bk = 0;
-        else if (v >= 2147483648.0f) bk = 2147483647;
-        else if (v <= -2147483648.0f) bk = -2147483647 - 1;
-        else bk = (int32_t)v;
-        bk = min(max(bk, 0), 65535);
         const uint32_t e = sg.start + i;
-        keys[e] = (sg.group << 16) | (uint32_t)bk;
+        keys[e] = (sg.group << 16) | mg_bucket(raw[sg.src + i], g.mn, depth_inv);
         vals[e] = e;
     }
+}
+
+__device__ __forceinline__ void mg_write_entry(const MergeSeg* __restrict__ segs, uint32_t n_segs, uint32_t e, uint32_t out,
+                                               uint32_t* __restrict__ merged_list, uint32_t* __restrict__ merged_map)
+{
+    const MergeSeg sg = segs[mg_find_seg(segs, n_segs, e)];
+    merged_list[out] = ((e - sg.start) + sg.gs_offset) | (sg.lod << kLodShift);
+    merged_map[out] = sg.map_index;
 }
 
 __global__ __launch_bounds__(256) void k_mg_final(const MergeSeg* __restrict__ segs, uint32_t n_segs, const MergeGroup* __restrict__ groups,
@@ -1359,18 +1381,14 @@
     if (p >= n_total) return;
     const uint32_t g = sorted_keys[p] >> 16;
     const MergeGroup gr = groups[g];
-    const uint32_t out = gr.out_base + (gr.len - 1u - (p - gr.base));
-    const uint32_t e = sorted_vals[p];
-    const MergeSeg sg = segs[mg_find_seg(segs, n_segs, e)];
-    merged_list[out] = ((e - sg.start) + sg.gs_offset) | (sg.lod << kLodShift);
-    merged_map[out] = sg.map_index;
-}
-
-__global__ __launch_bounds__(256) void k_mg_copy(const MergeCopy* __restrict__ jobs, const uint2* __restrict__ blocks, const uint2* __restrict__ remap,
-                                                 const MergeSources src, uint32_t* __restrict__ new_list, uint32_t* __restrict__ new_map)
+    mg_write_entry(segs, n_segs, sorted_vals[p], gr.out_base + (gr.len - 1u - (p - gr.base)), merged_list, merged_map);
+}
+
+__device__ __forceinline__ void mg_copy_block(uint32_t blk, const MergeCopy* __restrict__ jobs, const uint2* __restrict__ blocks, const uint2* __restrict__ remap,
+                                              const MergeSources& src, uint32_t* __restrict__ new_list, uint32_t* __restrict__ new_map)
 {
     __shared__ uint2 s_pairs[256];
-    const uint2 b = blocks[blockIdx.x];
+    const uint2 b = blocks[blk];
     const MergeCopy jb = jobs[b.x];
     const uint32_t* __restrict__ old_list = src.list[jb.src_set < (uint32_t)kMergeSources ? jb.src_set : 0u];
     const uint32_t* __restrict__ old_map = src.map[jb.src_set < (uint32_t)kMergeSources ? jb.src_set : 0u];
@@ -1385,6 +1403,134 @@
         uint32_t m = old_map[jb.src + i];
         for (uint32_t q = 0; q < np; q++) if (s_pairs[q].x == m) { m = s_pairs[q].y; break; }
         new_map[jb.dst + i] = m;
+    }
+}
+
+struct EventPre {
+    const DrawDev* draws; const uint32_t* xcd_first; uint32_t n_draws; uint2* chunk_tab; uint2* chunk_tab_xcd; XcdLens xl;
+    const MergeCopy* jobs; const uint2* cblocks; uint32_t n_cblocks; const uint2* remap; MergeSources src;
+    const MergeSeg* segs; const uint2* blocks; uint32_t n_blocks; const int32_t* raw; MergeGroup* groups;
+    uint32_t* merged_list; uint32_t* merged_map;
+};
+__global__ __launch_bounds__(256) void k_event_pre(const EventPre e)
+{
+    uint32_t wg = blockIdx.x;
+    const uint32_t n_tab = chunk_tabs_workgroups(e.n_draws);
+    if (wg < n_tab) { chunk_tabs_role(wg, e.draws, e.xcd_first, e.n_draws, e.chunk_tab, e.chunk_tab_xcd, e.xl); return; }
+    wg -= n_tab;
+    if (wg < e.n_cblocks) { mg_copy_block(wg, e.jobs, e.cblocks, e.remap, e.src, e.merged_list, e.merged_map); return; }
+    wg -= e.n_cblocks;
+    if (wg < e.n_blocks) mg_minmax_block(wg, e.segs, e.blocks, e.raw, e.groups);
+}
+
+template <int PASS>
+struct MgsBlock { MergeGroup g; uint32_t first, n, row0, n_rows; float depth_inv; uint32_t src, start; };
+template <int PASS>
+__device__ __forceinline__ MgsBlock<PASS> mgs_block(uint32_t blk, const MergeSeg* __restrict__ segs, const uint2* __restrict__ blocks, const MergeGroup* __restrict__ groups)
+{
+    MgsBlock<PASS> B;
+    const uint2 b = blocks[blk];
+    if (PASS == 0) {
+        const MergeSeg sg = segs[b.x];
+        B.g = groups[sg.group];
+        B.first = b.y; B.n = min(sg.len - b.y, kMgBlock); B.src = sg.src; B.start = sg.start;
+        B.row0 = B.g.blk0; B.n_rows = B.g.n_blk0;
+        B.depth_inv = mg_depth_inv(B.g);
+    } else {
+        B.g = groups[b.x];
+        B.first = b.y; B.n = min(B.g.len - b.y, kMgBlock); B.src = 0; B.start = 0;
+        B.row0 = B.g.blk1; B.n_rows = (B.g.len + kMgBlock - 1u) / kMgBlock;
+        B.depth_inv = 0.0f;
+    }
+    return B;
+}
+template <int PASS>
+__device__ __forceinline__ uint32_t mgs_bucket(const MgsBlock<PASS>& B, uint32_t i, const int32_t* __restrict__ raw, const uint32_t* __restrict__ keys_mid)
+{
+    if (PASS == 0) return mg_bucket(raw[B.src + B.first + i], B.g.mn, B.depth_inv);
+    return keys_mid[B.g.base + B.first + i];
+}
+
+template <int PASS>
+__global__ __launch_bounds__(256) void k_mgs_hist(const MergeSeg* __restrict__ segs, const uint2* __restrict__ blocks, const MergeGroup* __restrict__ groups,
+                                                  const int32_t* __restrict__ raw, const uint32_t* __restrict__ keys_mid, uint32_t* __restrict__ rows)
+{
+    __shared__ uint32_t s_h[256];
+    s_h[threadIdx.x] = 0u;
+    const MgsBlock<PASS> B = mgs_block<PASS>(blockIdx.x, segs, blocks, groups);
+    __syncthreads();
+#pragma unroll
+    for (uint32_t k = 0; k < 4u; k++) {
+        const uint32_t i = k * 256u + threadIdx.x;
+        if (i < B.n) atomicAdd(&s_h[(mgs_bucket<PASS>(B, i, raw, keys_mid) >> (8 * PASS)) & 255u], 1u);
+    }
+    __syncthreads();
+    rows[(size_t)blockIdx.x * 256u + threadIdx.x] = s_h[threadIdx.x];
+}
+
+template <int PASS>
+__global__ __launch_bounds__(256) void k_mgs_scatter(const MergeSeg* __restrict__ segs, uint32_t n_segs, const uint2* __restrict__ blocks,
+                                                     const MergeGroup* __restrict__ groups, const int32_t* __restrict__ raw, const uint32_t* __restrict__ rows,
+                                                     uint32_t* __restrict__ keys_mid, uint32_t* __restrict__ vals_mid,
+                                                     uint32_t* __restrict__ merged_list, uint32_t* __restrict__ merged_map)
+{
+    __shared__ uint32_t s_cnt[16][256];
+    __shared__ uint32_t s_base[256];
+    __shared__ uint32_t s_wsum[4];
+    const uint32_t t = threadIdx.x, lane = t & 63u, w = t >> 6;
+    const MgsBlock<PASS> B = mgs_block<PASS>(blockIdx.x, segs, blocks, groups);
+#pragma unroll
+    for (uint32_t r = 0; r < 16u; r++) s_cnt[r][t] = 0u;
+    uint32_t total = 0, before = 0;
+    for (uint32_t r = 0; r < B.n_rows; r++) {
+        const uint32_t v = rows[(size_t)(B.row0 + r) * 256u + t];
+        total += v;
+        if (B.row0 + r < blockIdx.x) before += v;
+    }
+    uint32_t incl = total;
+    for (int off = 1; off < 64; off <<= 1) { const uint32_t o = __shfl_up(incl, off, 64); if ((int)lane >= off) incl += o; }
+    if (lane == 63u) s_wsum[w] = incl;
+    __syncthreads();
+    uint32_t wbase = 0;
+    for (uint32_t q = 0; q < w; q++) wbase += s_wsum[q];
+    s_base[t] = wbase + incl - total + before;
+    uint32_t bucket[4], rank[4];
+#pragma unroll
+    for (uint32_t k = 0; k < 4u; k++) {
+        const uint32_t i = k * 256u + t;
+        const bool valid = i < B.n;
+        bucket[k] = valid ? mgs_bucket<PASS>(B, i, raw, keys_mid) : 0u;
+        const uint32_t digit = (bucket[k] >> (8 * PASS)) & 255u;
+        unsigned long long peers = __ballot(valid);
+#pragma unroll
+        for (int bit = 0; bit < 8; bit++) {
+            const bool one = (digit >> bit) & 1u;
+            const unsigned long long m = __ballot(one);
+            peers &= one ? m : ~m;
+        }
+        rank[k] = (uint32_t)__popcll(peers & ((1ull << lane) - 1ull));
+        if (valid && (peers >> lane) == 1ull) s_cnt[k * 4u + w][digit] = (uint32_t)__popcll(peers);
+    }
+    __syncthreads();
+    {
+        uint32_t run = 0;
+#pragma unroll
+        for (uint32_t r = 0; r < 16u; r++) { const uint32_t c = s_cnt[r][t]; s_cnt[r][t] = run; run += c; }
+    }
+    __syncthreads();
+#pragma unroll
+    for (uint32_t k = 0; k < 4u; k++) {
+        const uint32_t i = k * 256u + t;
+        if (i >= B.n) break;
+        const uint32_t digit = (bucket[k] >> (8 * PASS)) & 255u;
+        const uint32_t pos = s_base[digit] + s_cnt[k * 4u + w][digit] + rank[k];
+        if (pos >= B.g.len) continue;
+        if (PASS == 0) {
+            keys_mid[B.g.base + pos] = bucket[k];
+            vals_mid[B.g.base + pos] = B.start + B.first + i;
+        } else {
+            mg_write_entry(segs, n_segs, vals_mid[B.g.base + B.first + i], B.g.out_base + (B.g.len - 1u - pos), merged_list, merged_map);
+        }
     }
 }
 
@@ -2250,13 +2396,19 @@
     out[(size_t)y * width + x] = gathered[src];
 }
 
-void launch_chunk_tabs(hipStream_t s, const DrawDev* draws, const uint32_t* xcd_first, uint32_t n_draws, uint2* chunk_tab, uint2* chunk_tab_xcd,
-                       const uint64_t per_xcd[8], uint64_t longest)
-{
-    XcdLens xl;
-    for (int x = 0; x < 8; x++) xl.len[x] = (uint32_t)per_xcd[x];
-    xl.longest = (uint32_t)longest;
-    if (n_draws) hipLaunchKernelGGL(k_chunk_tabs, dim3(n_draws + 8u), dim3(256), 0, s, draws, xcd_first, n_draws, chunk_tab, chunk_tab_xcd, xl);
+void launch_event_pre(hipStream_t s, const EventPreArgs& a)
+{
+    EventPre e;
+    e.draws = a.draws; e.xcd_first = a.xcd_first; e.n_draws = a.n_draws; e.chunk_tab = a.chunk_tab; e.chunk_tab_xcd = a.chunk_tab_xcd;
+    for (int x = 0; x < 8; x++) e.xl.len[x] = (uint32_t)a.per_xcd[x];
+    e.xl.longest = (uint32_t)a.longest;
+    e.jobs = a.jobs; e.cblocks = a.cblocks; e.n_cblocks = a.n_cblocks; e.remap = a.remap;
+    if (a.src) e.src = *a.src;
+    else for (int k = 0; k < kMergeSources; k++) { e.src.list[k] = nullptr; e.src.map[k] = nullptr; }
+    e.segs = a.segs; e.blocks = a.blocks; e.n_blocks = a.n_blocks; e.raw = a.raw; e.groups = a.groups;
+    e.merged_list = a.merged_list; e.merged_map = a.merged_map;
+    const uint32_t grid = chunk_tabs_workgroups(a.n_draws) + a.n_cblocks + a.n_blocks;
+    if (grid) hipLaunchKernelGGL(k_event_pre, dim3(grid), dim3(256), 0, s, e);
 }
 
 GraphRec*& graph_recorder()
@@ -2367,12 +2519,29 @@
     return cur;
 }
 
-void launch_merge_build(hipStream_t s, const MergeSeg* segs, uint32_t n_segs, const uint2* blocks, uint32_t n_blocks, MergeGroup* groups, uint32_t n_groups,
-                        const int32_t* raw, uint32_t n_total, const unsigned long long* n_total_dev, uint32_t* ka, uint32_t* va,
-                        uint32_t* kb, uint32_t* vb, uint32_t* radix_ws, int group_bits, uint32_t* merged_list, uint32_t* merged_map)
+size_t merge_seg_ws_words(uint32_t n_total, uint32_t n_blocks, uint32_t n_gblocks)
+{
+    return 2 * (size_t)n_total + (size_t)256 * ((size_t)n_blocks + n_gblocks);
+}
+
+void launch_merge_build_seg(hipStream_t s, const MergeSeg* segs, uint32_t n_segs, const uint2* blocks, uint32_t n_blocks, const uint2* gblocks,
+                            uint32_t n_gblocks, const MergeGroup* groups, const int32_t* raw, uint32_t n_total, uint32_t* ws,
+                            uint32_t* merged_list, uint32_t* merged_map)
+{
+    if (n_total == 0 || n_blocks == 0 || n_gblocks == 0) return;
+    uint32_t* const keys_mid = ws; uint32_t* const vals_mid = ws + n_total;
+    uint32_t* const rows0 = ws + 2 * (size_t)n_total; uint32_t* const rows1 = rows0 + (size_t)256 * n_blocks;
+    hipLaunchKernelGGL(k_mgs_hist<0>, dim3(n_blocks), dim3(256), 0, s, segs, blocks, groups, raw, keys_mid, rows0);
+    hipLaunchKernelGGL(k_mgs_scatter<0>, dim3(n_blocks), dim3(256), 0, s, segs, n_segs, blocks, groups, raw, rows0, keys_mid, vals_mid, merged_list, merged_map);
+    hipLaunchKernelGGL(k_mgs_hist<1>, dim3(n_gblocks), dim3(256), 0, s, segs, gblocks, groups, raw, keys_mid, rows1);
+    hipLaunchKernelGGL(k_mgs_scatter<1>, dim3(n_gblocks), dim3(256), 0, s, segs, n_segs, gblocks, groups, raw, rows1, keys_mid, vals_mid, merged_list, merged_map);
+}
+
+void launch_merge_build_global(hipStream_t s, const MergeSeg* segs, uint32_t n_segs, const uint2* blocks, uint32_t n_blocks, MergeGroup* groups, uint32_t n_groups,
+                               const int32_t* raw, uint32_t n_total, const unsigned long long* n_total_dev, uint32_t* ka, uint32_t* va,
+                               uint32_t* kb, uint32_t* vb, uint32_t* radix_ws, int group_bits, uint32_t* merged_list, uint32_t* merged_map)
 {
     if (n_total == 0 || n_groups == 0 || n_blocks == 0) return;
-    hipLaunchKernelGGL(k_mg_minmax, dim3(n_blocks), dim3(256), 0, s, segs, blocks, raw, groups);
     hipLaunchKernelGGL(k_mg_keys, dim3(n_blocks), dim3(256), 0, s, segs, blocks, raw, groups, ka, va);
     const int where = launch_sort(s, ka, va, kb, vb, n_total, n_total_dev, 16 + group_bits, radix_ws);
     hipLaunchKernelGGL(k_mg_final, dim3((n_total + 255) / 256), dim3(256), 0, s, segs, n_segs, groups, where ? kb : ka, where ? vb : va,
@@ -2387,12 +2556,6 @@
     hipLaunchKernelGGL(k_mg_minmax, dim3(n_blocks), dim3(256), 0, s, segs, blocks, raw, groups);
     hipLaunchKernelGGL(k_mg_keys, dim3(n_blocks), dim3(256), 0, s, segs, blocks, raw, groups, ka, va);
     return launch_sort(s, ka, va, kb, vb, n_total, n_total_dev, 16 + group_bits, radix_ws);
-}
-
-void launch_merge_copy(hipStream_t s, const MergeCopy* jobs, const uint2* blocks, uint32_t n_blocks, const uint2* remap, const MergeSources& src,
-                       uint32_t* new_list, uint32_t* new_map)
-{
-    if (n_blocks) hipLaunchKernelGGL(k_mg_copy, dim3(n_blocks), dim3(256), 0, s, jobs, blocks, remap, src, new_list, new_map);
 }
 
 void launch_tile_depth_sort(hipStream_t s, const uint2* ranges, uint32_t* vals, uint32_t* dkeys, uint32_t* vals_scratch, uint32_t* dkeys_scratch, int n_tiles,
```

Result: no change. 5504 (median of 3 runs) (-0.7%).
